# i2Nav-WHU/IC-GVINS

Measured on NVIDIA H100. Metric: frames/sec (KLT+BA) 1280x560 300-feat 10-KF window, higher is better.
Workload: dtype u8/int32 fixed point + f32 (KLT), f64 (BA)

## Files before the change

ic_gvins_b200/csrc/ba.cu:

```cuda
#include <cooperative_groups.h>
#include <dlfcn.h>
#include <unistd.h>
#include <math.h>
#include <nccl.h>
#include <stdlib.h>
#include <string.h>

#include <algorithm>
#include <string>
#include <thread>
#include <vector>

#include "ba_math.cuh"
#include "common.cuh"
#include "geom_core.cuh"

namespace icg {
using namespace bam;
namespace cg = cooperative_groups;

constexpr int BA_SPLIT_W = 4;
constexpr int BA_CHOL_NB = 8;
constexpr int BA_MARG_MAXB = 72;
constexpr int BA_MAX_NODES = 32;

struct BaCaps {
    int NW, K, L, F, G, R;
    int NCV, N, NS, NCA, RJ, LP, NVB;
    int GQ;
};

struct WinDims {
    int K, L, F, n_imu, n_gnss, marg_r, marg_nb;
    int ext_const, td_const, reproj_huber, gnss_huber, has_imu_error, has_pose_prior, has_mix_prior;
    double reproj_sinv;
};

struct LmState {
    double radius, decrease_factor, x_cost, x_norm, cand_cost, model_cost_change, step_norm, gmax, initial_cost, cost_cam;
    int iter, n_success, n_invalid, done, need_lin, last_success, first, step_valid, fresh_lin, max_iter, chol_ok;
};

struct ShardDev {
    int split;
    int PK, BS, RV;
    double *peer[8];
    size_t off_inbox, off_bcast, off_scal, off_flagA, off_flagB, off_flagC;
    double *redv;
    int *err;
    double *slm;
    int *slm_cnt;
};

struct BaDev {
    ShardDev S;
    WinDims *dims;
    LmState *st;
    double *pose, *mix, *ext, *rho;
    double *pose_c, *mix_c, *ext_c, *rho_c;
    double *pose_0, *mix_0, *ext_0, *rho_0;
    uint8_t *f_active_0;
    double *gnss_std_0;
    uint8_t *f_active;
    int *lm_off;
    int *lm_perm;
    int *vb_lm0;
    int *ref_nrun;
    int *f_meta_s;
    double *f_const_s;
    int *vis_ord;
    int *part_off, *pair_ro, *npairs;
    double *gpart;
    int *vis_cnt;
    double *Mp;
    double *AW;
    double *costf;
    double *hl, *gl, *scale_l, *scale_c;
    double *Hc, *gc;
    double *Hs;
    double *visv;
    double *imu_blob, *imu_U;
    int *gnss_node;
    double *gnss_blh, *gnss_std, *lever;
    double *pose_prior, *pose_prior_sinfo, *mix_prior, *mix_prior_std;
    int *marg_type, *marg_node;
    double *marg_x0, *marg_H0, *marg_b0, *marg_c0;
    double *cost_part;
    double *red;
    double *redmax;
    double *red2;
    int rank, world;
    double *step_c, *step_l;
    double *Sglobal;
    unsigned long long *clk;
};

__device__ __forceinline__ int col_pose(int k) { return 6 * k; }
__device__ __forceinline__ int col_ext(int K) { return 6 * K; }
__device__ __forceinline__ int col_td(int K) { return 6 * K + 6; }
__device__ __forceinline__ int col_mix(int K, int k) { return 6 * K + 7 + 9 * k; }

__device__ __forceinline__ int jc_off(int a) { return a < 18 ? (a / 6) * 12 + (a % 6) : 36 + 2 * (a - 18); }
__device__ __forceinline__ int jc_row1(int a) { return a < 18 ? 6 : 1; }
__device__ __forceinline__ int tri20(int la, int lb) {
    return la * 20 - la * (la - 1) / 2 + (lb - la);
}
__device__ __forceinline__ void dmma884(double &c0, double &c1, double a, double b) {
    asm volatile("mma.sync.aligned.m8n8k4.row.col.f64.f64.f64.f64 {%0,%1}, {%2}, {%3}, {%0,%1};" : "+d"(c0), "+d"(c1) : "d"(a), "d"(b));
}
constexpr int LV_LD = 45;
constexpr size_t LV_SMEM = sizeof(double) * (128 * LV_LD + (BA_MAX_NODES + 1) * NODE_FRAME_LD);
__global__ void __launch_bounds__(128, 4) ba_lin_vis(BaCaps C, BaDev D) {
    extern __shared__ double lv_sm[];
    __shared__ int s_ord[128], s_gbeg[BA_MAX_NODES], s_gend[BA_MAX_NODES], s_last, s_p0, s_np;
    double (*s_rec)[LV_LD] = (double (*)[LV_LD]) lv_sm;
    double (*s_frame)[NODE_FRAME_LD] = (double (*)[NODE_FRAME_LD]) (lv_sm + 128 * LV_LD);
    const int w = blockIdx.y;
    const LmState &st = D.st[w];
    if (st.done || !st.need_lin) return;
    const int *vb = D.vb_lm0 + (size_t) w * C.NVB;
    if ((int) blockIdx.x >= vb[C.NVB - 1]) return;
    const WinDims dm = D.dims[w];
    const int tid = threadIdx.x;
    const int *off = D.lm_off + (size_t) w * (C.L + 1);
    const int pA = vb[blockIdx.x], pB = vb[blockIdx.x + 1];
    const int s0 = off[pA], nslot = off[pB] - s0;
    if (tid <= dm.K) node_frame(tid < dm.K ? D.pose + ((size_t) w * C.K + tid) * 7 : D.ext + (size_t) w * 8, s_frame[tid]);
    if (tid < BA_MAX_NODES) s_gbeg[tid] = s_gend[tid] = 0;
    if (tid == 0) s_np = 0;
    __syncthreads();
    if (tid < nslot) {
        const int q = s0 + tid;
        double r[2], Ji[12], Jj[12], Je[12], Jr[2], Jt[2], cost = 0;
        const int4 meta = ((const int4 *) D.f_meta_s)[(size_t) w * C.F + q];
        const int i = meta.y, j = meta.z, f = meta.w;
        if (D.f_active[(size_t) w * C.F + f] != 0) {
            const double *ext = D.ext + (size_t) w * 8;
            reproj_eval_frames(s_frame[i], s_frame[j], s_frame[dm.K], D.rho[(size_t) w * C.L + meta.x], ext[7],
                               D.f_const_s + ((size_t) w * C.F + q) * 14, dm.reproj_sinv, true, r, Ji, Jj, Je, Jr, Jt);
            if (dm.ext_const)
                for (int k = 0; k < 12; k++) Je[k] = 0;
            if (dm.td_const) Jt[0] = Jt[1] = 0;
            double sq = r[0] * r[0] + r[1] * r[1], sc = 1.0;
            if (dm.reproj_huber)
                huber(sq, cost, sc);
            else
                cost = 0.5 * sq;
            if (sc != 1.0) {
                for (int k = 0; k < 12; k++) Ji[k] *= sc, Jj[k] *= sc, Je[k] *= sc;
                Jr[0] *= sc, Jr[1] *= sc, Jt[0] *= sc, Jt[1] *= sc, r[0] *= sc, r[1] *= sc;
            }
        } else {
            for (int k = 0; k < 12; k++) Ji[k] = Jj[k] = Je[k] = 0;
            Jr[0] = Jr[1] = Jt[0] = Jt[1] = r[0] = r[1] = 0;
        }
        D.costf[(size_t) w * C.F + f] = cost;
        double *sr = s_rec[tid];
#pragma unroll
        for (int k = 0; k < 12; k++) sr[k] = Ji[k], sr[12 + k] = Jj[k], sr[24 + k] = Je[k];
        sr[36] = Jt[0], sr[37] = Jt[1], sr[38] = r[0], sr[39] = r[1];
        sr[40] = Jr[0], sr[41] = Jr[1], sr[42] = (double) j, sr[43] = (double) i;
    }
    __syncthreads();
    const int lane = tid & 31, warp = tid >> 5;
    if (nslot > 0) {
        if (tid < nslot) {
            const int *ord = D.vis_ord + (size_t) w * C.F + s0;
            const int v = ord[tid], ob = (int) s_rec[v & 255][42];
            s_ord[tid] = v;
            if (tid == 0 || (int) s_rec[ord[tid - 1] & 255][42] != ob) s_gbeg[ob] = tid;
            if (tid == nslot - 1 || (int) s_rec[ord[tid + 1] & 255][42] != ob) s_gend[ob] = tid + 1;
        }
        __syncthreads();
        const int kk = lane & 3, g = lane >> 2;
        int o[3];
#pragma unroll
        for (int t = 0; t < 3; t++) {
            const int a = 8 * t + g;
            o[t] = a < 20 ? jc_off(a) + (kk & 1) * jc_row1(a) : -1;
        }
        for (int ob = warp; ob < dm.K; ob += 4) {
            const int beg = s_gbeg[ob], end = s_gend[ob];
            if (beg == end) continue;
            double c00[2] = {0, 0}, c01[2] = {0, 0}, c02[2] = {0, 0}, c11[2] = {0, 0}, c12[2] = {0, 0}, c22[2] = {0, 0};
            constexpr int UNR = 2;
            for (int base = beg; base < end; base += 2 * UNR) {
                double x[UNR][3];
#pragma unroll
                for (int u = 0; u < UNR; u++) {
                    const int q = base + 2 * u + (kk >> 1);
                    const bool ok = q < end;
                    const double *rec = s_rec[ok ? s_ord[q] & 255 : 0];
#pragma unroll
                    for (int t = 0; t < 3; t++) x[u][t] = (ok && o[t] >= 0) ? rec[o[t]] : 0.0;
                }
#pragma unroll
                for (int u = 0; u < UNR; u++) {
                    dmma884(c00[0], c00[1], x[u][0], x[u][0]);
                    dmma884(c01[0], c01[1], x[u][0], x[u][1]);
                    dmma884(c02[0], c02[1], x[u][0], x[u][2]);
                    dmma884(c11[0], c11[1], x[u][1], x[u][1]);
                    dmma884(c12[0], c12[1], x[u][1], x[u][2]);
                    dmma884(c22[0], c22[1], x[u][2], x[u][2]);
                }
            }
            double *pp = D.gpart + ((size_t) w * C.GQ + (s_ord[beg] >> 8)) * 210;
            auto put = [&](int ti, int tj, const double *c) {
#pragma unroll
                for (int e = 0; e < 2; e++) {
                    const int la = 8 * ti + g, lb = 8 * tj + 2 * kk + e;
                    if (la <= lb && lb < 20) pp[tri20(la, lb)] = c[e];
                }
            };
            put(0, 0, c00), put(0, 1, c01), put(0, 2, c02), put(1, 1, c11), put(1, 2, c12), put(2, 2, c22);
        }
        __threadfence();
    }
    const int *perm = D.lm_perm + (size_t) w * C.L;
    const int K = dm.K, NCV = 6 * K + 7, NCA = 4 * ((NCV + 1 + 3) / 4);
    const int grp = tid >> 3, sl = tid & 7;
    int o0[3], o1[3];
#pragma unroll
    for (int t = 0; t < 3; t++) {
        const int c = sl + 8 * t;
        o0[t] = c < 19 ? jc_off(c) : 38, o1[t] = c < 19 ? o0[t] + jc_row1(c) : 39;
    }
    for (int pl = pA + grp; pl < pB; pl += 16) {
        const int l = perm[pl], f0 = off[pl] - s0, nf = off[pl + 1] - off[pl];
        double *row = D.AW + ((size_t) w * C.LP + l) * C.NCA;
        for (int c = sl; c < NCA; c += 8) row[c] = 0.0;
        __syncwarp(0xffu << (tid & 24));
        double acc[3] = {0, 0, 0};
        for (int q = 0; q < nf; q++) {
            const double *rec = s_rec[f0 + q];
            const double r0 = rec[40], r1 = rec[41];
            const int ob = (int) rec[42];
#pragma unroll
            for (int t = 0; t < 3; t++) {
                const int c = sl + 8 * t;
                if (c == 20) {
                    acc[t] += r0 * r0 + r1 * r1;
                } else if (c < 20) {
                    const double v = rec[o0[t]] * r0 + rec[o1[t]] * r1;
                    if (c >= 6 && c < 12)
                        row[col_pose(ob) + c - 6] = v;
                    else
                        acc[t] += v;
                }
            }
        }
        const int ref = nf > 0 ? (int) s_rec[f0][43] : 0;
#pragma unroll
        for (int t = 0; t < 3; t++) {
            const int c = sl + 8 * t;
            if (nf > 0) {
                if (c < 6) row[col_pose(ref) + c] = acc[t];
                else if (c >= 12 && c < 18) row[col_ext(K) + c - 12] = acc[t];
                else if (c == 18) row[col_td(K)] = acc[t];
            }
            if (c == 19) {
                row[NCV] = acc[t];
                D.gl[(size_t) w * C.L + l] = acc[t];
            } else if (c == 20) {
                D.hl[(size_t) w * C.L + l] = acc[t];
                if (st.first) D.scale_l[(size_t) w * C.L + l] = 1.0 / (1.0 + sqrt(acc[t]));
            }
        }
    }
    if (nslot == 0) return;
    const int rn = (int) s_rec[0][43];
    __syncthreads();
    if (tid == 0) s_last = atomicAdd(D.vis_cnt + (size_t) w * C.K + rn, 1) == D.ref_nrun[(size_t) w * C.K + rn] - 1;
    __syncthreads();
    if (!s_last) return;
    __threadfence();
    if (tid == 0) D.vis_cnt[(size_t) w * C.K + rn] = 0;
    const int PM = C.K * (C.K - 1), P = D.npairs[w];
    const int *pro = D.pair_ro + (size_t) w * PM, *poff = D.part_off + (size_t) w * (PM + 1);
    for (int p = tid; p < P; p += 128)
        if ((pro[p] >> 8) == rn) {
            atomicAdd(&s_np, 1);
            if (p == 0 || (pro[p - 1] >> 8) != rn) s_p0 = p;
        }
    __syncthreads();
    const double *part = D.gpart + (size_t) w * C.GQ * 210;
    double *Mp = D.Mp + (size_t) w * PM * 210;
    for (int p = s_p0 + warp; p < s_p0 + s_np; p += 4) {
        const int k0 = poff[p], k1 = poff[p + 1];
        double acc[7];
#pragma unroll
        for (int j = 0; j < 7; j++) acc[j] = lane + 32 * j < 210 ? __ldcg(part + (size_t) k0 * 210 + lane + 32 * j) : 0.0;
        for (int k = k0 + 1; k < k1; k++) {
            double v[7];
#pragma unroll
            for (int j = 0; j < 7; j++) v[j] = lane + 32 * j < 210 ? __ldcg(part + (size_t) k * 210 + lane + 32 * j) : 0.0;
#pragma unroll
            for (int j = 0; j < 7; j++) acc[j] += v[j];
        }
#pragma unroll
        for (int j = 0; j < 7; j++)
            if (lane + 32 * j < 210) Mp[(size_t) p * 210 + lane + 32 * j] = acc[j];
    }
}


__device__ __forceinline__ void gram2_slots(const BaCaps &C, const BaDev &D, int w, int K, short *s_slot) {
    const int PM = C.K * (C.K - 1), P = D.npairs[w];
    const int *pro = D.pair_ro + (size_t) w * PM;
    for (int e = threadIdx.x; e < K * K; e += blockDim.x) s_slot[e] = -1;
    __syncthreads();
    for (int p = threadIdx.x; p < P; p += blockDim.x) s_slot[(pro[p] >> 8) * K + (pro[p] & 255)] = (short) p;
    __syncthreads();
}
__device__ __forceinline__ double gram2_entry(const BaCaps &C, const BaDev &D, int w, int K, const short *s_slot, int A, int B) {
    const int PM = C.K * (C.K - 1), P = D.npairs[w];
    const double *Mp = D.Mp + (size_t) w * PM * 210;
    const int bA = A < 6 * K ? A / 6 : K, bB = B < 6 * K ? B / 6 : K;
    const int a = A - 6 * bA, b = B - 6 * bB;
    const int ga = 12 + a, gb = 12 + b;
    double sum = 0;
    if (bA == K) {
        const int idx = tri20(ga, gb);
        double s4[4] = {0, 0, 0, 0};
        int p = 0;
        for (; p + 16 <= P; p += 16) {
            double v[16];
#pragma unroll
            for (int u = 0; u < 16; u++) v[u] = Mp[(size_t) (p + u) * 210 + idx];
#pragma unroll
            for (int u = 0; u < 16; u++) s4[u & 3] += v[u];
        }
        for (; p < P; p++) s4[p & 3] += Mp[(size_t) p * 210 + idx];
        sum = (s4[0] + s4[1]) + (s4[2] + s4[3]);
    } else if (bB == K || bB == bA) {
        const int i1 = tri20(a, bB == K ? gb : b), i2 = tri20(6 + a, bB == K ? gb : 6 + b);
        for (int o0 = 0; o0 < K; o0 += 8) {
            double v1[8], v2[8];
#pragma unroll
            for (int u = 0; u < 8; u++) {
                const int o = o0 + u;
                const int p1 = o < K ? s_slot[bA * K + o] : -1, p2 = o < K ? s_slot[o * K + bA] : -1;
                v1[u] = p1 >= 0 ? Mp[(size_t) p1 * 210 + i1] : 0.0;
                v2[u] = p2 >= 0 ? Mp[(size_t) p2 * 210 + i2] : 0.0;
            }
#pragma unroll
            for (int u = 0; u < 8; u++) sum += v1[u], sum += v2[u];
        }
    } else {
        const int p1 = s_slot[bA * K + bB], p2 = s_slot[bB * K + bA];
        if (p1 >= 0) sum += Mp[(size_t) p1 * 210 + tri20(a, 6 + b)];
        if (p2 >= 0) sum += Mp[(size_t) p2 * 210 + tri20(b, 6 + a)];
    }
    return sum;
}

__device__ __forceinline__ double block_sum(double v, double *s_red);
__device__ __forceinline__ double block_max(double v, double *s_red);
__device__ __forceinline__ double *x_inbox(const BaDev &D, int peer, int w, int from);
__device__ __forceinline__ int tri_idx(int A, int B, int ncv);

__device__ __forceinline__ void schur_store(const BaCaps &C, const BaDev &D, int w, int K, const short *s_slot, int A, int B, double cw) {
    const int NCV = 6 * K + 7;
    const bool nccl = !D.S.split && D.world > 1;
    if (A == NCV && !nccl) return;
    const size_t e = (size_t) w * C.NS * C.NS + (size_t) B * C.NS + A;
    const double hc = !D.S.split && !nccl && B < NCV ? D.Hc[e] : 0.0;
    const double cj = gram2_entry(C, D, w, K, s_slot, A, B);
    if (D.S.split) {
        double *P = x_inbox(D, w % D.world, w, D.rank);
        const int TRI = NCV * (NCV + 1) / 2;
        if (B < NCV) {
            P[tri_idx(A, B, NCV)] = cj - cw;
            if (A == B) P[TRI + A] = cj;
        } else {
            P[TRI + NCV + A] = cj;
            P[TRI + 2 * NCV + A] = cw;
        }
    } else if (nccl) {
        const size_t NN = (size_t) C.NCA * C.NCA;
        double *R = D.red + (size_t) w * (2 * NN + 8);
        R[(size_t) A * C.NCA + B] = R[(size_t) B * C.NCA + A] = cj;
        R[NN + (size_t) A * C.NCA + B] = R[NN + (size_t) B * C.NCA + A] = cw;
    } else {
        double *V = D.visv + (size_t) w * 3 * C.NCV;
        if (B < NCV) {
            D.Hs[e] = hc + (cj - cw);
            if (A == B) V[A] = cj;
        } else {
            V[NCV + A] = cj, V[2 * NCV + A] = cw;
        }
    }
}

__device__ __forceinline__ void schur_scalars(const BaCaps &C, const BaDev &D, int w, const WinDims &dm, double *s_red) {
    const int tid = threadIdx.x;
    double c = 0, q = 0, gm = 0;
    for (int f = tid; f < dm.F; f += 256) c += D.costf[(size_t) w * C.F + f];
    for (int l = tid; l < dm.L; l += 256) {
        const double r = D.rho[(size_t) w * C.L + l];
        q += r * r;
        gm = fmax(gm, fabs(D.gl[(size_t) w * C.L + l]));
    }
    c = block_sum(c, s_red);
    q = block_sum(q, s_red);
    gm = block_max(gm, s_red);
    if (tid != 0) return;
    if (D.S.split) {
        const int NCV = 6 * dm.K + 7, TRI = NCV * (NCV + 1) / 2;
        double *P = x_inbox(D, w % D.world, w, D.rank);
        P[TRI + 3 * NCV] = c, P[TRI + 3 * NCV + 1] = q, P[TRI + 3 * NCV + 2] = gm;
    } else {
        const size_t NN = (size_t) C.NCA * C.NCA;
        double *R = D.red + (size_t) w * (2 * NN + 8);
        R[2 * NN] = c, R[2 * NN + 1] = q;
        for (int k = 2; k < 8; k++) R[2 * NN + k] = 0;
        D.redmax[w] = gm;
    }
}

constexpr int SCHUR_RCH = 80;
constexpr int SCHUR_PASS = 16;
__global__ void __cluster_dims__(BA_SPLIT_W, 1, 1) __launch_bounds__(256) ba_schur_dmma(BaCaps C, BaDev D, int ld) {
    extern __shared__ double sA[];
    __shared__ short s_slot[32 * 32];
    __shared__ double s_red[40];
    cg::cluster_group cluster = cg::this_cluster();
    const int w = blockIdx.y, split = blockIdx.x;
    const LmState &st = D.st[w];
    if (st.done) return;
    const WinDims dm = D.dims[w];
    const int NCV = 6 * dm.K + 7, NCA = 4 * ((NCV + 1 + 3) / 4);
    const int T2 = (NCA + 15) / 16, nsuper = T2 * (T2 + 1) / 2;
    const int tid = threadIdx.x, lane = tid & 31, warp = tid >> 5, g = lane >> 2, kk = lane & 3;
    double *sphi = sA + (size_t) SCHUR_RCH * ld;
    const double *A = D.AW + (size_t) w * C.LP * C.NCA;
    const double radius = st.radius;
    const int nsteps = (dm.L + 3) / 4;
    const int r_beg = 4 * (int) ((long long) nsteps * split / BA_SPLIT_W), r_end = min(dm.L, 4 * (int) ((long long) nsteps * (split + 1) / BA_SPLIT_W));
    const int npass = (nsuper + SCHUR_PASS - 1) / SCHUR_PASS;
    gram2_slots(C, D, w, dm.K, s_slot);
    for (int pass = 0; pass < npass; pass++) {
        if (pass > 0) cluster.barrier_wait();
        int si[2], sj[2];
        bool on[2];
#pragma unroll
        for (int h2 = 0; h2 < 2; h2++) {
            const int su = (2 * pass + h2) * 8 + warp;
            on[h2] = su < nsuper;
            int a = 0, e = on[h2] ? su : 0;
            while (e >= T2 - a) e -= T2 - a, a++;
            si[h2] = a, sj[h2] = a + e;
        }
        double acc[2][4][2];
#pragma unroll
        for (int h2 = 0; h2 < 2; h2++)
#pragma unroll
            for (int q = 0; q < 4; q++) acc[h2][q][0] = acc[h2][q][1] = 0;
        for (int r0 = r_beg; r0 < r_end; r0 += SCHUR_RCH) {
            const int nr = min(SCHUR_RCH, r_end - r0), nr4 = (nr + 3) & ~3;
            __syncthreads();
            for (int rb = warp; rb < nr4; rb += 8 * 4) {
                double v[4][3];
#pragma unroll
                for (int u = 0; u < 4; u++) {
                    const int rr = rb + 8 * u;
#pragma unroll
                    for (int cchunk = 0; cchunk < 3; cchunk++) {
                        const int c = lane + 32 * cchunk;
                        v[u][cchunk] = (rr < nr && c < NCA) ? A[(size_t) (r0 + rr) * C.NCA + c] : 0.0;
                    }
                }
#pragma unroll
                for (int u = 0; u < 4; u++) {
                    const int rr = rb + 8 * u;
#pragma unroll
                    for (int cchunk = 0; cchunk < 3; cchunk++) {
                        const int c = lane + 32 * cchunk;
                        if (rr < nr4 && c < ld) sA[(size_t) rr * ld + c] = v[u][cchunk];
                    }
                }
                for (int c = lane + 96; c < ld; c += 32)
                    for (int u = 0; u < 4; u++) {
                        const int rr = rb + 8 * u;
                        if (rr < nr4) sA[(size_t) rr * ld + c] = (rr < nr && c < NCA) ? A[(size_t) (r0 + rr) * C.NCA + c] : 0.0;
                    }
            }
            for (int rr = tid; rr < nr4; rr += 256) {
                double ph = 0;
                if (rr < nr) {
                    const int l = r0 + rr;
                    const double sl = D.scale_l[(size_t) w * C.L + l], hs = sl * sl * D.hl[(size_t) w * C.L + l];
                    ph = sl * sl / (hs + fmin(fmax(hs, 1e-6), 1e32) / radius);
                }
                sphi[rr] = ph;
            }
            __syncthreads();
            for (int ks = 0; ks < nr4 / 4; ks++) {
                const double *row = sA + (size_t) (4 * ks + kk) * ld;
                const double ph = sphi[4 * ks + kk];
#pragma unroll
                for (int h2 = 0; h2 < 2; h2++) {
                    if (!on[h2]) continue;
                    const double xb0 = row[16 * sj[h2] + g], xb1 = row[16 * sj[h2] + 8 + g];
                    const double a0 = row[16 * si[h2] + g] * ph, a1 = row[16 * si[h2] + 8 + g] * ph;
                    dmma884(acc[h2][0][0], acc[h2][0][1], a0, xb0);
                    dmma884(acc[h2][1][0], acc[h2][1][1], a0, xb1);
                    dmma884(acc[h2][2][0], acc[h2][2][1], a1, xb0);
                    dmma884(acc[h2][3][0], acc[h2][3][1], a1, xb1);
                }
            }
        }
        __syncthreads();
#pragma unroll
        for (int h2 = 0; h2 < 2; h2++) {
            if (!on[h2]) continue;
#pragma unroll
            for (int q = 0; q < 4; q++)
#pragma unroll
                for (int e = 0; e < 2; e++) sA[(h2 * 8 + warp) * 256 + 64 * q + 32 * e + lane] = acc[h2][q][e];
        }
        cluster.sync();
        const int nslot = min(SCHUR_PASS, nsuper - SCHUR_PASS * pass);
        double cw[SCHUR_PASS / BA_SPLIT_W];
#pragma unroll
        for (int j = 0; j < SCHUR_PASS / BA_SPLIT_W; j++) {
            const int sl = split + BA_SPLIT_W * j;
            double p[BA_SPLIT_W];
#pragma unroll
            for (int k = 0; k < BA_SPLIT_W; k++) p[k] = sl < nslot ? cluster.map_shared_rank(sA, k)[sl * 256 + tid] : 0.0;
            cw[j] = 0;
#pragma unroll
            for (int k = 0; k < BA_SPLIT_W; k++) cw[j] += p[k];
        }
        cluster.barrier_arrive();
        const int q = tid >> 6, r_in = 8 * (q >> 1) + ((tid & 31) >> 2), c_in = 8 * (q & 1) + 2 * (tid & 3) + ((tid >> 5) & 1);
#pragma unroll
        for (int j = 0; j < SCHUR_PASS / BA_SPLIT_W; j++) {
            const int sl = split + BA_SPLIT_W * j;
            if (sl >= nslot) break;
            int a = 0, e = SCHUR_PASS * pass + sl;
            while (e >= T2 - a) e -= T2 - a, a++;
            const int r = 16 * a + r_in, cc = 16 * (a + e) + c_in;
            if (r <= cc && cc <= NCV) schur_store(C, D, w, dm.K, s_slot, r, cc, cw[j]);
        }
    }
    if (split == 0 && (D.S.split || D.world > 1)) schur_scalars(C, D, w, dm, s_red);
    cluster.barrier_wait();
}

constexpr double IMU_GB_STD = 7200 / 3600.0 * 3.14159265358979323846 / 180.0;
constexpr double IMU_AB_STD = 2.0e4 * 1.0e-5;

__device__ void imu_factor_warp(const double *blob, const double *U, const double *pose0, const double *mix0, const double *pose1,
                                const double *mix1, bool want_j, double *rw, double *Jw, int lane) {
    __shared__ ImuMid s_mid[16];
    double *raw_r = rw + 15;
    const int wslot = (threadIdx.x >> 5) & 15;
    if (want_j)
        for (int e = lane; e < 450; e += 32) Jw[e] = 0;
    __syncwarp();
    if (lane == 0) {
        ImuMid M;
        imu_residual_raw(blob, pose0, mix0, pose1, mix1, raw_r, M);
        if (want_j) imu_jacobian_raw(blob, M, Jw);
        s_mid[wslot] = M;
    }
    __syncwarp();
    if (want_j && lane < 30) {
        for (int i = 0; i < 15; i++) {
            double s = 0;
            for (int k = i; k < 15; k++) s += U[i * 15 + k] * Jw[k * 30 + lane];
            Jw[i * 30 + lane] = s;
        }
    }
    if (lane < 15) {
        double s = 0;
        for (int k = lane; k < 15; k++) s += U[lane * 15 + k] * raw_r[k];
        rw[lane] = s;
    }
    __syncwarp();
}

__device__ void marg_dx(const BaCaps &C, const BaDev &D, int w, const WinDims &dm, const double *pose, const double *mix, const double *ext, double *dx,
                        int *colmap, int tid, int nthreads) {
    const int *type = D.marg_type + (size_t) w * BA_MARG_MAXB, *node = D.marg_node + (size_t) w * BA_MARG_MAXB;
    const double *x0 = D.marg_x0 + (size_t) w * BA_MARG_MAXB * 9;
    if (tid == 0) {
        int col = 0, xo = 0;
        for (int b = 0; b < dm.marg_nb; b++) {
            int t = type[b], nd = node[b];
            if (t == 0 || t == 2) {
                const double *x = t == 0 ? pose + nd * 7 : ext;
                const double *xl = x0 + xo;
                Q dq = qmul(qinv(pose_q(xl)), pose_q(x));
                V3 a = 2.0 * qv(dq);
                if (dq.w < 0) a = -a;
                for (int k = 0; k < 3; k++) dx[col + k] = x[k] - xl[k];
                dx[col + 3] = a.x, dx[col + 4] = a.y, dx[col + 5] = a.z;
                int base = t == 0 ? col_pose(nd) : col_ext(dm.K);
                for (int k = 0; k < 6; k++) colmap[col + k] = (t == 2 && dm.ext_const) ? -1 : base + k;
                col += 6, xo += 7;
            } else if (t == 1) {
                for (int k = 0; k < 9; k++) dx[col + k] = mix[nd * 9 + k] - x0[xo + k], colmap[col + k] = col_mix(dm.K, nd) + k;
                col += 9, xo += 9;
            } else {
                dx[col] = ext[7] - x0[xo];
                colmap[col] = dm.td_const ? -1 : col_td(dm.K);
                col += 1, xo += 1;
            }
        }
    }
}

__device__ __forceinline__ void red_add(double *p, double v) { asm volatile("red.global.add.f64 [%0], %1;" ::"l"(p), "d"(v) : "memory"); }

__device__ double cam_factors(const BaCaps &C, const BaDev &D, int w, const WinDims &dm, const double *pose, const double *mix, const double *ext,
                              bool lin, double *smem) {
    const int tid = threadIdx.x, lane = tid & 31, warp = tid >> 5, nwarps = blockDim.x >> 5;
    const int K = dm.K, N = 15 * K + 7;
    double *Hc = D.Hc + (size_t) w * C.NS * C.NS, *gc = D.gc + (size_t) w * C.NS;
    double *s_imu = smem;
    double *s_gnss = s_imu + (size_t) C.K * 480;
    double *s_misc = s_gnss + (size_t) C.G * 24;
    double *s_pp = s_misc, *s_mp = s_misc + 48, *s_dx = s_mp + 16, *s_y = s_dx + C.R, *s_cost = s_y + C.R;
    int *s_colmap = (int *) (s_cost + 8);
    __shared__ double s_total;
#ifdef ICG_BA_PHASE_CLOCKS
    unsigned long long cclk = D.clk ? clock64() : 0ull;
#define CAM_CLK(k)                                                 \
    if (D.clk && lin && w == 0 && tid == 0) {                      \
        const unsigned long long t_ = clock64();                   \
        atomicAdd(&D.clk[16 + (k)], t_ - cclk), atomicAdd(&D.clk[24 + (k)], 1ull); \
        cclk = t_;                                                 \
    }
#else
#define CAM_CLK(k)
#endif
    for (int k = warp; k < dm.n_imu; k += nwarps)
        imu_factor_warp(D.imu_blob + ((size_t) w * C.K + k) * ICG_IMU_BLOB_DOUBLES, D.imu_U + ((size_t) w * C.K + k) * 225, pose + k * 7, mix + k * 9,
                        pose + (k + 1) * 7, mix + (k + 1) * 9, lin, s_imu + (size_t) k * 480, s_imu + (size_t) k * 480 + 30, lane);
    if (tid < dm.n_gnss) {
        const int nd = D.gnss_node[(size_t) w * C.G + tid];
        double *o = s_gnss + tid * 24;
        gnss_eval(pose + nd * 7, D.gnss_blh + ((size_t) w * C.G + tid) * 3, D.gnss_std + ((size_t) w * C.G + tid) * 3, D.lever + (size_t) w * 3, lin, o, o + 3);
        double sq = o[0] * o[0] + o[1] * o[1] + o[2] * o[2], cost, sc = 1.0;
        if (dm.gnss_huber)
            huber(sq, cost, sc);
        else
            cost = 0.5 * sq;
        if (sc != 1.0) {
            for (int e = 0; e < 3; e++) o[e] *= sc;
            if (lin)
                for (int e = 0; e < 18; e++) o[3 + e] *= sc;
        }
        o[21] = cost;
    }
    if (tid == 64 && dm.has_pose_prior) pose_prior_eval(pose, D.pose_prior + (size_t) w * 7, D.pose_prior_sinfo + (size_t) w * 6, lin, s_pp, s_pp + 6);
    if (tid == 96 && dm.has_mix_prior)
        for (int k = 0; k < 9; k++) s_mp[k] = (mix[k] - D.mix_prior[(size_t) w * 9 + k]) / D.mix_prior_std[(size_t) w * 9 + k];
    if (dm.marg_r > 0) marg_dx(C, D, w, dm, pose, mix, ext, s_dx, s_colmap, tid, blockDim.x);
    __syncthreads();
    CAM_CLK(0)
    const double *H0 = D.marg_H0 + (size_t) w * C.R * C.R, *b0 = D.marg_b0 + (size_t) w * C.R;
    if (dm.marg_r > 0) {
        for (int i = tid; i < dm.marg_r; i += blockDim.x) {
            double s = 0;
            for (int k = 0; k < dm.marg_r; k++) s += H0[(size_t) i * dm.marg_r + k] * s_dx[k];
            s_y[i] = s;
        }
    }
    __syncthreads();
    if (tid == 0) {
        double c = 0;
        for (int k = 0; k < dm.n_imu; k++) {
            const double *r = s_imu + (size_t) k * 480;
            double sq = 0;
            for (int e = 0; e < 15; e++) sq += r[e] * r[e];
            c += 0.5 * sq;
        }
        for (int g = 0; g < dm.n_gnss; g++) c += s_gnss[g * 24 + 21];
        if (dm.has_imu_error) {
            const double *m = mix + dm.n_imu * 9;
            double sq = 0;
            for (int e = 0; e < 3; e++) sq += (m[3 + e] / IMU_GB_STD) * (m[3 + e] / IMU_GB_STD) + (m[6 + e] / IMU_AB_STD) * (m[6 + e] / IMU_AB_STD);
            c += 0.5 * sq;
        }
        if (dm.has_pose_prior) {
            double sq = 0;
            for (int e = 0; e < 6; e++) sq += s_pp[e] * s_pp[e];
            c += 0.5 * sq;
        }
        if (dm.has_mix_prior) {
            double sq = 0;
            for (int e = 0; e < 9; e++) sq += s_mp[e] * s_mp[e];
            c += 0.5 * sq;
        }
        if (dm.marg_r > 0) {
            double q = D.marg_c0[w];
            for (int i = 0; i < dm.marg_r; i++) q += (2.0 * b0[i] + s_y[i]) * s_dx[i];
            c += 0.5 * q;
        }
        s_total = c;
    }
// ... 5 lines not shown
    for (int e = tid; e < N * C.NS; e += blockDim.x) Hc[e] = 0;
    for (int e = tid; e < N; e += blockDim.x) gc[e] = 0;
    __syncthreads();
    CAM_CLK(2)
    if (dm.marg_r > 0) {
        const int r = dm.marg_r;
        for (int e = tid; e < r * r; e += blockDim.x) {
            int i = e / r, j = e - i * r;
            int ci = s_colmap[i], cj = s_colmap[j];
            if (ci >= 0 && cj >= 0) Hc[(size_t) ci * C.NS + cj] = H0[e];
        }
        for (int i = tid; i < r; i += blockDim.x)
            if (s_colmap[i] >= 0) gc[s_colmap[i]] = b0[i] + s_y[i];
    }
    __syncthreads();
    CAM_CLK(3)
    for (int parity = 0; parity < 2; parity++) {
        const int nf = (dm.n_imu - parity + 1) / 2;
        for (int e = tid; e < nf * 930; e += blockDim.x) {
            const int k = parity + 2 * (e / 930), q = e % 930;
            const double *rw = s_imu + (size_t) k * 480, *Jw = rw + 30;
            auto gcol = [&](int c) { return c < 6 ? col_pose(k) + c : c < 15 ? col_mix(K, k) + c - 6 : c < 21 ? col_pose(k + 1) + c - 15 : col_mix(K, k + 1) + c - 21; };
            if (q < 900) {
                int a = q / 30, b = q - a * 30;
                double s = 0;
                for (int m = 0; m < 15; m++) s += Jw[m * 30 + a] * Jw[m * 30 + b];
                red_add(&Hc[(size_t) gcol(a) * C.NS + gcol(b)], s);
            } else {
                int a = q - 900;
                double s = 0;
                for (int m = 0; m < 15; m++) s += Jw[m * 30 + a] * rw[m];
                red_add(&gc[gcol(a)], s);
            }
        }
        __syncthreads();
    }
    CAM_CLK(4)
    for (int e = tid; e < K * 42; e += blockDim.x) {
        const int k = e / 42, q = e % 42;
        double s = 0;
        if (q < 36) {
            const int a = q / 6, b = q % 6;
            for (int g = 0; g < dm.n_gnss; g++)
                if (D.gnss_node[(size_t) w * C.G + g] == k) {
                    const double *J = s_gnss + g * 24 + 3;
                    s += J[a] * J[b] + J[6 + a] * J[6 + b] + J[12 + a] * J[12 + b];
                }
            if (k == 0 && dm.has_pose_prior)
                for (int m = 0; m < 6; m++) s += s_pp[6 + m * 6 + a] * s_pp[6 + m * 6 + b];
            red_add(&Hc[(size_t) (col_pose(k) + a) * C.NS + col_pose(k) + b], s);
        } else {
            const int a = q - 36;
            for (int g = 0; g < dm.n_gnss; g++)
                if (D.gnss_node[(size_t) w * C.G + g] == k) {
                    const double *o = s_gnss + g * 24;
                    s += o[3 + a] * o[0] + o[9 + a] * o[1] + o[15 + a] * o[2];
                }
            if (k == 0 && dm.has_pose_prior)
                for (int m = 0; m < 6; m++) s += s_pp[6 + m * 6 + a] * s_pp[m];
            red_add(&gc[col_pose(k) + a], s);
        }
    }
    if (tid < 9) {
        if (dm.has_imu_error && tid >= 3) {
            const int k = dm.n_imu;
            const double sd = tid < 6 ? IMU_GB_STD : IMU_AB_STD;
            Hc[(size_t) (col_mix(K, k) + tid) * C.NS + col_mix(K, k) + tid] += 1.0 / (sd * sd);
            gc[col_mix(K, k) + tid] += mix[k * 9 + tid] / (sd * sd);
        }
    }
    __syncthreads();
    if (tid < 9 && dm.has_mix_prior) {
        const double sd = D.mix_prior_std[(size_t) w * 9 + tid];
        Hc[(size_t) (col_mix(K, 0) + tid) * C.NS + col_mix(K, 0) + tid] += 1.0 / (sd * sd);
        gc[col_mix(K, 0) + tid] += s_mp[tid] / sd;
    }
    __syncthreads();
    CAM_CLK(5)
#undef CAM_CLK
    return s_total;
}

constexpr int CAM_THREADS = 320;
__global__ void __launch_bounds__(CAM_THREADS) ba_lin_cam(BaCaps C, BaDev D) {
    extern __shared__ double smem[];
    const int w = blockIdx.x;
    LmState &st = D.st[w];
    if (st.done || !st.need_lin) return;
    if (D.S.split && (w % D.world) != D.rank) return;
    const WinDims dm = D.dims[w];
    double c = cam_factors(C, D, w, dm, D.pose + (size_t) w * C.K * 7, D.mix + (size_t) w * C.K * 9, D.ext + (size_t) w * 8, true, smem);
    if (threadIdx.x == 0) st.cost_cam = c;
}

__global__ void ba_pack2(BaCaps C, BaDev D, int n, int nblk_vis) {
    const int w = blockIdx.x * blockDim.x + threadIdx.x;
    if (w >= n) return;
    const LmState &st = D.st[w];
    if (st.done || !st.step_valid) return;
    const WinDims dm = D.dims[w];
    const double *part = D.cost_part + (size_t) w * (nblk_vis + 1);
    double cand = 0;
    const int nb = (dm.F + 255) / 256;
    for (int b = 0; b < nb; b++) cand += part[b];
    if (D.rank == 0) cand += part[nblk_vis];
    D.red2[(size_t) w * 4 + 3] = cand;
}

__global__ void __launch_bounds__(256) ba_hsum(BaCaps C, BaDev D) {
    const int w = blockIdx.y;
    if (D.st[w].done) return;
    const int K = D.dims[w].K, NCV = 6 * K + 7, nn = NCV + 1;
    const int NN = C.NCA * C.NCA;
    const int t = blockIdx.x * 256 + threadIdx.x;
    if (t >= nn * nn) return;
    const int A = t / nn, B = t - A * nn;
    if (B < A || B >= NCV) return;
    const double *RED = D.red + (size_t) w * (2 * NN + 8);
    const double cj = RED[(size_t) B * C.NCA + A], cw = RED[NN + (size_t) B * C.NCA + A];
    D.Hs[(size_t) w * C.NS * C.NS + (size_t) B * C.NS + A] = D.Hc[(size_t) w * C.NS * C.NS + (size_t) B * C.NS + A] + (cj - cw);
}

constexpr int SOLVE_THREADS = 256;

__device__ __forceinline__ double block_sum(double v, double *s_red) {
    const int tid = threadIdx.x, lane = tid & 31, warp = tid >> 5;
    for (int o = 16; o > 0; o >>= 1) v += __shfl_down_sync(0xffffffffu, v, o);
    __syncthreads();
    if (lane == 0) s_red[warp] = v;
    __syncthreads();
    double t = 0;
    if (tid == 0) {
        for (int k = 0; k < (int) (blockDim.x >> 5); k++) t += s_red[k];
        s_red[32] = t;
    }
    __syncthreads();
    return s_red[32];
}
__device__ __forceinline__ double block_max(double v, double *s_red) {
    const int tid = threadIdx.x, lane = tid & 31, warp = tid >> 5;
    for (int o = 16; o > 0; o >>= 1) v = fmax(v, __shfl_down_sync(0xffffffffu, v, o));
    __syncthreads();
    if (lane == 0) s_red[warp] = v;
    __syncthreads();
    if (tid == 0) {
        double t = 0;
        for (int k = 0; k < (int) (blockDim.x >> 5); k++) t = fmax(t, s_red[k]);
        s_red[32] = t;
    }
    __syncthreads();
    return s_red[32];
}

__global__ void __launch_bounds__(SOLVE_THREADS, 2) ba_solve(BaCaps C, BaDev D) {
    extern __shared__ double sm[];
    const int w = blockIdx.x, tid = threadIdx.x;
    LmState &st = D.st[w];
    if (st.done) return;
#ifdef ICG_BA_PHASE_CLOCKS
    unsigned long long clk_prev = D.clk ? clock64() : 0ull;
#define SOLVE_CLK(k)                                              \
    if (D.clk && w == 0 && tid == 0) {                            \
        const unsigned long long t_ = clock64();                  \
        atomicAdd(&D.clk[k], t_ - clk_prev), atomicAdd(&D.clk[8 + (k)], 1ull); \
        clk_prev = t_;                                            \
    }
#define SOLVE_CLK_NOW() (D.clk ? clock64() : 0ull)
#define SOLVE_CLK_ADD(k, t0)                                      \
    if (D.clk && w == 0 && tid == 0) atomicAdd(&D.clk[k], clock64() - (t0)), atomicAdd(&D.clk[8 + (k)], 1ull);
#else
#define SOLVE_CLK(k)
#define SOLVE_CLK_NOW() 0ull
#define SOLVE_CLK_ADD(k, t0)
#endif
    const WinDims dm = D.dims[w];
    const int K = dm.K, L = dm.L, NCV = 6 * K + 7, N = 15 * K + 7;
    const int f_first = st.first, f_fresh = st.fresh_lin, f_last = st.last_success, f_iter = st.iter;
    const double f_gmax_old = st.gmax;
    (void) f_gmax_old;
    double *s_red = sm;
    double *s_scale = s_red + 40;
    double *s_g = s_scale + C.NS;
    double *s_rhs = s_g + C.NS;
    double *s_d2 = s_rhs + C.NS;
    double *s_diag = s_d2 + C.NS;
    double *S = s_diag + C.NS;
    const double *Hc = D.Hc + (size_t) w * C.NS * C.NS, *gcam = D.gc + (size_t) w * C.NS, *Hs = D.Hs + (size_t) w * C.NS * C.NS;
    const bool sharded = D.world > 1;
    const int NN = C.NCA * C.NCA;
    const double *RED = D.red + (size_t) w * (2 * NN + 8), *V = D.visv + (size_t) w * 3 * C.NCV;
    auto hvis_diag = [&](int a) { return sharded ? RED[(size_t) a * C.NCA + a] : V[a]; };
    auto g_vis = [&](int a) { return sharded ? RED[(size_t) a * C.NCA + NCV] : V[NCV + a]; };
    auto wphig = [&](int a) { return sharded ? RED[NN + (size_t) a * C.NCA + NCV] : V[2 * NCV + a]; };
    const double camw = D.rank == 0 ? 1.0 : 0.0;
    if (tid == 0 && st.need_lin) st.need_lin = 0;
    double *scale_c = D.scale_c + (size_t) w * C.NS;
    const double *hl = D.hl + (size_t) w * C.L, *gl = D.gl + (size_t) w * C.L, *scale_l = D.scale_l + (size_t) w * C.L;

    for (int a = tid; a < N; a += SOLVE_THREADS) {
        double g = gcam[a];
        if (a < NCV) g += g_vis(a);
        s_g[a] = g;
        if (f_first) {
            double h = Hc[(size_t) a * C.NS + a] + (a < NCV ? hvis_diag(a) : 0.0);
            scale_c[a] = 1.0 / (1.0 + sqrt(h));
        }
    }
    __syncthreads();
    for (int a = tid; a < N; a += SOLVE_THREADS) s_scale[a] = scale_c[a];
    double gmax_now = st.gmax;
    if (f_fresh) {
        double c, gml;
        if (sharded) {
            c = RED[2 * NN];
            gml = D.redmax[w];
        } else {
            double cs = 0, gq = 0;
            for (int f = tid; f < dm.F; f += SOLVE_THREADS) cs += D.costf[(size_t) w * C.F + f];
            for (int l = tid; l < L; l += SOLVE_THREADS) gq = fmax(gq, fabs(gl[l]));
            c = block_sum(cs, s_red);
            gml = block_max(gq, s_red);
        }
        double gm = 0;
        for (int a = tid; a < N; a += SOLVE_THREADS) gm = fmax(gm, fabs(s_g[a]));
        gm = fmax(block_max(gm, s_red), gml);
        gmax_now = gm;
        if (tid == 0) {
            st.x_cost = c + st.cost_cam;
            st.gmax = gm;
            if (f_first) st.initial_cost = st.x_cost;
            st.fresh_lin = 0;
        }
        __syncthreads();
    }
    if (f_first) {
        __syncthreads();
        if (tid == 0) st.first = 0;
    }
    {
        int term = 0;
        if (f_iter >= st.max_iter) term = 1;
        else if (f_last && gmax_now <= 1e-10) term = 2;
        else if (f_last && st.radius <= 1e-32) term = 2;
        if (term) {
            __syncthreads();
            if (tid == 0) st.done = term, st.step_valid = 0;
            return;
        }
    }
    __syncthreads();
    if (tid == 0) st.iter++;
    const double radius = st.radius;
    SOLVE_CLK(0)

    constexpr bool async_fill = true;
    if (async_fill) {
        for (int i = tid >> 5; i < N; i += SOLVE_THREADS / 32) {
            const double *src = (i < NCV ? Hs : Hc) + (size_t) i * C.NS;
            const unsigned dst = (unsigned) __cvta_generic_to_shared(S + i * (i + 1) / 2);
            for (int j = tid & 31; j <= i; j += 32)
                asm volatile("cp.async.ca.shared.global [%0], [%1], 8;" ::"r"(dst + 8u * j), "l"(src + j) : "memory");
        }
        asm volatile("cp.async.commit_group;" ::: "memory");
    }
    for (int a = tid; a < N; a += SOLVE_THREADS) {
        double h = Hc[(size_t) a * C.NS + a] + (a < NCV ? hvis_diag(a) : 0.0);
        double hs = s_scale[a] * s_scale[a] * h;
        s_d2[a] = fmin(fmax(hs, 1e-6), 1e32) / radius;
        double gw = a < NCV ? wphig(a) : 0.0;
        s_rhs[a] = -s_scale[a] * (s_g[a] - gw);
    }
    if (async_fill) asm volatile("cp.async.wait_all;" ::: "memory");
    __syncthreads();
    if (async_fill) {
        for (int i = tid >> 5; i < N; i += SOLVE_THREADS / 32) {
            double *row = S + i * (i + 1) / 2;
            const double si = s_scale[i];
            for (int j = tid & 31; j <= i; j += 32) {
                double v = si * s_scale[j] * row[j];
                if (i == j) v += s_d2[i];
                row[j] = v;
            }
        }
    } else {
        for (int i = tid >> 5; i < N; i += SOLVE_THREADS / 32) {
            constexpr int MAXQ = 16;
            double hv[MAXQ];
            const int nq = i / 32 + 1;
#pragma unroll
            for (int q = 0; q < MAXQ; q++) {
                const int j = (tid & 31) + 32 * q;
                hv[q] = 0;
                if (q < nq && j <= i) hv[q] = (i < NCV ? Hs : Hc)[(size_t) i * C.NS + j];
            }
#pragma unroll
            for (int q = 0; q < MAXQ; q++) {
                const int j = (tid & 31) + 32 * q;
                if (q < nq && j <= i) {
                    double v = s_scale[i] * s_scale[j] * hv[q];
                    if (i == j) v += s_d2[i];
                    S[i * (i + 1) / 2 + j] = v;
                }
            }
        }
    }
    for (int a = tid; a < N; a += SOLVE_THREADS) S[N * (N + 1) / 2 + a] = s_rhs[a];
    __syncthreads();
    SOLVE_CLK(1)
    __shared__ int s_fail;
    if (tid == 0) s_fail = 0;
    __syncthreads();
// ... 89 lines not shown
#pragma unroll
                    for (int u = 0; u < TPW; u++) {
                        dmma884(acc[u][0], acc[u][1], a0[u], b0);
                        dmma884(acc[u][2], acc[u][3], a1[u], b1);
                    }
                }
#pragma unroll
                for (int u = 0; u < TPW; u++) {
                    const double c0 = acc[u][0] + acc[u][2], c1 = acc[u][1] + acc[u][3];
                    const int i = J0 + 8 * (t0 + u * NWARP) + g;
                    if (oka[u]) {
                        const int ca = J0 + 2 * kk;
                        if (ca < J0 + nb && ca <= i) S[i * (i + 1) / 2 + ca] -= c0;
                        if (ca + 1 < J0 + nb && ca + 1 <= i) S[i * (i + 1) / 2 + ca + 1] -= c1;
                    }
                }
            }
        }
        __syncthreads();
        const unsigned long long pc1 = SOLVE_CLK_NOW();
        (void) pc1;
        if (s_fail) break;
        for (int i = J0 + nb + tid; i < NR; i += SOLVE_THREADS) {
            double *ri = S + i * (i + 1) / 2 + J0;
            double x[BA_CHOL_NB];
#pragma unroll
            for (int c = 0; c < BA_CHOL_NB; c++) x[c] = c < nb ? ri[c] : 0.0;
#pragma unroll
            for (int c = 0; c < BA_CHOL_NB; c++) {
                if (c < nb) {
                    const double *lc = S + (J0 + c) * (J0 + c + 1) / 2 + J0;
                    double sum = x[c];
#pragma unroll
                    for (int k = 0; k < c; k++) sum -= x[k] * lc[k];
                    x[c] = sum * s_diag[J0 + c];
                }
            }
#pragma unroll
            for (int c = 0; c < BA_CHOL_NB; c++)
                if (c < nb) ri[c] = x[c];
        }
        __syncthreads();
        SOLVE_CLK_ADD(7, pc1)
    }
    __syncthreads();
    bool valid = !s_fail;
    SOLVE_CLK(2)
    if (valid) {
        double *y = S + N * (N + 1) / 2;
        const int lane = tid & 31;
        for (int J0 = ((N - 1) / BA_CHOL_NB) * BA_CHOL_NB; J0 >= 0; J0 -= BA_CHOL_NB) {
            const int nb = min(BA_CHOL_NB, N - J0);
            if (tid < 32) {
                double x[BA_CHOL_NB];
#pragma unroll
                for (int c = BA_CHOL_NB - 1; c >= 0; c--) {
                    x[c] = 0.0;
                    if (c < nb) {
                        double sum = y[J0 + c];
#pragma unroll
                        for (int k = BA_CHOL_NB - 1; k > c; k--)
                            if (k < nb) sum -= S[(J0 + k) * (J0 + k + 1) / 2 + J0 + c] * x[k];
                        x[c] = sum * s_diag[J0 + c];
                    }
                }
#pragma unroll
                for (int c = 0; c < BA_CHOL_NB; c++)
                    if (c == lane && c < nb) s_rhs[J0 + c] = x[c];
            }
            __syncthreads();
            for (int i = tid; i < J0; i += SOLVE_THREADS) {
                double acc = y[i];
#pragma unroll
                for (int c = BA_CHOL_NB - 1; c >= 0; c--)
                    if (c < nb) acc -= S[(J0 + c) * (J0 + c + 1) / 2 + i] * s_rhs[J0 + c];
                y[i] = acc;
            }
            __syncthreads();
        }
    }
    __syncthreads();
    SOLVE_CLK(3)
    double *step_l = D.step_l + (size_t) w * C.L;
    const double *AW = D.AW + (size_t) w * C.LP * C.NCA;
    double part = 0;
    bool finite = true;
    double *R2 = D.red2 + (size_t) w * 4;
    if (!valid) {
        if (tid == 0) {
            st.chol_ok = 0, st.step_valid = 0;
            R2[0] = 0, R2[1] = 0, R2[2] = 1, R2[3] = 0;
        }
        return;
    }
    for (int a = tid; a < N; a += SOLVE_THREADS) {
        double sp = s_rhs[a];
        finite = finite && isfinite(sp);
        part += camw * (-0.5 * sp * (s_scale[a] * s_g[a]) + 0.5 * s_d2[a] * sp * sp);
    }
    double *s_sx = s_diag;
    __syncthreads();
    for (int a = tid; a < NCV; a += SOLVE_THREADS) s_sx[a] = s_scale[a] * s_rhs[a];
    __syncthreads();
    {
        const int lane = tid & 31, warp = tid >> 5;
        constexpr int LB = 8;
        const int lu = ((lane >> 4) & 1) * 4 + ((lane >> 3) & 1) * 2 + ((lane >> 2) & 1);
        for (int l0 = LB * warp; l0 < L; l0 += LB * (SOLVE_THREADS / 32)) {
            const int l = l0 + lu;
            const bool lok = l < L;
            const double sl = lok ? scale_l[l] : 0.0, hh = lok ? hl[l] : 0.0, gg = lok ? gl[l] : 0.0;
            double d[LB];
#pragma unroll
            for (int u = 0; u < LB; u++) d[u] = 0;
            for (int c = lane; c < NCV; c += 32) {
                const double sx = s_sx[c];
#pragma unroll
                for (int u = 0; u < LB; u++) d[u] += (l0 + u < L ? AW[(size_t) (l0 + u) * C.NCA + c] : 0.0) * sx;
            }
            const double hs = sl * sl * hh, d2 = fmin(fmax(hs, 1e-6), 1e32) / radius, den = hs + d2, sg = sl * gg;
            double e4[4], e2[2];
            {
                const bool hi = lane & 16;
#pragma unroll
                for (int u = 0; u < 4; u++) {
                    const double keep = hi ? d[u + 4] : d[u], send = hi ? d[u] : d[u + 4];
                    e4[u] = keep + __shfl_xor_sync(0xffffffffu, send, 16);
                }
            }
            {
                const bool hi = lane & 8;
#pragma unroll
                for (int u = 0; u < 2; u++) {
                    const double keep = hi ? e4[u + 2] : e4[u], send = hi ? e4[u] : e4[u + 2];
                    e2[u] = keep + __shfl_xor_sync(0xffffffffu, send, 8);
                }
            }
            double mine;
            {
                const bool hi = lane & 4;
                const double keep = hi ? e2[1] : e2[0], send = hi ? e2[0] : e2[1];
                mine = keep + __shfl_xor_sync(0xffffffffu, send, 4);
            }
            mine += __shfl_xor_sync(0xffffffffu, mine, 2);
            mine += __shfl_xor_sync(0xffffffffu, mine, 1);
            if ((lane & 3) == 0 && lok) {
                double sp = (-sg - sl * mine) / den;
                finite = finite && isfinite(sp);
                step_l[l] = sp;
                part += -0.5 * sp * sg + 0.5 * d2 * sp * sp;
            }
        }
    }
    __syncthreads();
    SOLVE_CLK(4)
    const double mcc = block_sum(part, s_red);
    const double nfin = block_sum(finite ? 0.0 : 1.0, s_red);
    const double *pose = D.pose + (size_t) w * C.K * 7, *mix = D.mix + (size_t) w * C.K * 9, *ext = D.ext + (size_t) w * 8, *rho = D.rho + (size_t) w * C.L;
    double *pose_c = D.pose_c + (size_t) w * C.K * 7, *mix_c = D.mix_c + (size_t) w * C.K * 9, *ext_c = D.ext_c + (size_t) w * 8, *rho_c = D.rho_c + (size_t) w * C.L;
    double sn = 0;
    for (int k = tid; k <= K; k += SOLVE_THREADS) {
        const bool is_ext = (k == K);
        const double *x = is_ext ? ext : pose + k * 7;
        double *xc = is_ext ? ext_c : pose_c + k * 7;
        if (is_ext && dm.ext_const) {
            for (int e = 0; e < 7; e++) xc[e] = x[e];
        } else {
            const int c0 = is_ext ? col_ext(K) : col_pose(k);
            double d[6];
            for (int e = 0; e < 6; e++) d[e] = s_rhs[c0 + e] * s_scale[c0 + e];
            pose_plus(x, d, xc);
            for (int e = 0; e < 7; e++) sn += camw * (x[e] - xc[e]) * (x[e] - xc[e]);
        }
    }
    for (int e = tid; e < K * 9; e += SOLVE_THREADS) {
        int k = e / 9, q = e - 9 * k, c = col_mix(K, k) + q;
        double v = mix[e] + s_rhs[c] * s_scale[c];
        mix_c[e] = v;
        sn += camw * (mix[e] - v) * (mix[e] - v);
    }
    if (tid == 0) {
        if (dm.td_const) {
            ext_c[7] = ext[7];
        } else {
            double v = ext[7] + s_rhs[col_td(K)] * s_scale[col_td(K)];
            ext_c[7] = v;
            sn += camw * (ext[7] - v) * (ext[7] - v);
        }
    }
    for (int l = tid; l < L; l += SOLVE_THREADS) {
        double v = rho[l] + step_l[l] * scale_l[l];
        rho_c[l] = v;
        sn += (rho[l] - v) * (rho[l] - v);
    }
    sn = block_sum(sn, s_red);
    if (tid == 0) {
        st.chol_ok = 1, st.step_valid = 1;
        R2[0] = mcc, R2[1] = sn, R2[2] = nfin, R2[3] = 0;
    }
    SOLVE_CLK(5)
#undef SOLVE_CLK
#undef SOLVE_CLK_NOW
#undef SOLVE_CLK_ADD
}

__global__ void __launch_bounds__(CAM_THREADS) ba_cost_cam(BaCaps C, BaDev D, int nblk_vis) {
    extern __shared__ double smem[];
    const int w = blockIdx.x;
    const LmState &st = D.st[w];
    if (st.done || !st.step_valid) return;
    if (D.S.split && (w % D.world) != D.rank) return;
    const WinDims dm = D.dims[w];
    double c = cam_factors(C, D, w, dm, D.pose_c + (size_t) w * C.K * 7, D.mix_c + (size_t) w * C.K * 9, D.ext_c + (size_t) w * 8, false, smem);
    if (threadIdx.x == 0) D.cost_part[(size_t) w * (nblk_vis + 1) + nblk_vis] = c;
}
__global__ void __launch_bounds__(256) ba_cost(BaCaps C, BaDev D, int nblk_vis) {
    __shared__ double s_red[40];
    const int w = blockIdx.y;
    const LmState &st = D.st[w];
    if (st.done || !st.step_valid) return;
    const WinDims dm = D.dims[w];
    const double *pose = D.pose_c + (size_t) w * C.K * 7, *ext = D.ext_c + (size_t) w * 8, *rho = D.rho_c + (size_t) w * C.L;
    double *part = D.cost_part + (size_t) w * (nblk_vis + 1);
    const int q = blockIdx.x * 256 + threadIdx.x;
    __shared__ double s_frame[BA_MAX_NODES + 1][NODE_FRAME_LD];
    if ((int) threadIdx.x <= dm.K) node_frame((int) threadIdx.x < dm.K ? pose + threadIdx.x * 7 : ext, s_frame[threadIdx.x]);
    __syncthreads();
    double cost = 0;
    int4 meta = make_int4(0, 0, 0, 0);
    if (q < dm.F) meta = ((const int4 *) D.f_meta_s)[(size_t) w * C.F + q];
    if (q < dm.F && D.f_active[(size_t) w * C.F + meta.w]) {
        double r[2];
        reproj_eval_frames(s_frame[meta.y], s_frame[meta.z], s_frame[dm.K], rho[meta.x], ext[7], D.f_const_s + ((size_t) w * C.F + q) * 14, dm.reproj_sinv,
                           false, r, nullptr, nullptr, nullptr, nullptr, nullptr);
        double sq = r[0] * r[0] + r[1] * r[1], sc;
        if (dm.reproj_huber)
            huber(sq, cost, sc);
        else
            cost = 0.5 * sq;
    }
    cost = block_sum(cost, s_red);
    if (threadIdx.x == 0) part[blockIdx.x] = cost;
}

__global__ void __launch_bounds__(128) ba_accept(BaCaps C, BaDev D, int nblk_vis) {
    __shared__ int s_accept;
    __shared__ double s_camsq, s_rhosq;
    __shared__ double s_red[40];
    const int w = blockIdx.x, tid = threadIdx.x;
    LmState &st = D.st[w];
    if (st.done) return;
    const WinDims dm = D.dims[w];
    const int chol_ok = st.chol_ok;
    const double *R2 = D.red2 + (size_t) w * 4;
    {
        const double *pose = D.pose + (size_t) w * C.K * 7, *mix = D.mix + (size_t) w * C.K * 9, *ext = D.ext + (size_t) w * 8;
        double s = 0;
        for (int e = tid; e < dm.K * 7; e += 128) s += pose[e] * pose[e];
        for (int e = tid; e < dm.K * 9; e += 128) s += mix[e] * mix[e];
        if (tid < 7 && !dm.ext_const) s += ext[tid] * ext[tid];
        if (tid == 7 && !dm.td_const) s += ext[7] * ext[7];
        s = block_sum(s, s_red);
        double q = 0;
        if (D.world == 1) {
            for (int l = tid; l < dm.L; l += 128) q += D.rho[(size_t) w * C.L + l] * D.rho[(size_t) w * C.L + l];
            q = block_sum(q, s_red);
        } else {
            q = D.red[(size_t) w * (2 * C.NCA * C.NCA + 8) + 2 * C.NCA * C.NCA + 1];
        }
        if (tid == 0) s_camsq = s, s_rhosq = q;
    }
    __syncthreads();
    if (tid == 0) {
        s_accept = 0;
        const double mcc = R2[0], sn = R2[1], nfin = R2[2];
        double cand = R2[3];
        if (D.world == 1 && st.step_valid) {
            const double *part = D.cost_part + (size_t) w * (nblk_vis + 1);
            cand = 0;
            const int nb = (dm.F + 255) / 256;
            for (int b = 0; b < nb; b++) cand += part[b];
            cand += part[nblk_vis];
        }
        if (!chol_ok || nfin != 0.0 || !(mcc > 0.0)) {
            st.step_valid = 0;
            st.n_invalid++;
            if (st.n_invalid >= 5) st.done = 3;
            st.radius *= 0.5;
            st.last_success = 0;
        } else {
            st.n_invalid = 0;
            st.model_cost_change = mcc;
            st.step_norm = sqrt(sn);
            st.x_norm = sqrt(s_camsq + s_rhosq);
            st.cand_cost = cand;
            if (st.step_norm <= 1e-8 * (st.x_norm + 1e-8)) {
                st.done = 2;
            } else if (fabs(st.x_cost - cand) <= 1e-6 * st.x_cost) {
                st.done = 2;
            } else {
                const double rel = (st.x_cost - cand) / mcc;
                if (rel > 1e-3) {
                    s_accept = 1;
                    st.n_success++;
                    double t = 2.0 * rel - 1.0;
                    st.radius = fmin(1e16, st.radius / fmax(1.0 / 3.0, 1.0 - t * t * t));
                    st.decrease_factor = 2.0;
                    st.last_success = 1;
                    st.need_lin = 1;
                    st.fresh_lin = 1;
                } else {
                    st.radius = st.radius / st.decrease_factor;
                    st.decrease_factor *= 2.0;
                    st.last_success = 0;
                    st.need_lin = 0;
                }
            }
        }
    }
    __syncthreads();
    if (!s_accept) return;
    double *pose = D.pose + (size_t) w * C.K * 7, *mix = D.mix + (size_t) w * C.K * 9, *ext = D.ext + (size_t) w * 8, *rho = D.rho + (size_t) w * C.L;
    const double *pose_c = D.pose_c + (size_t) w * C.K * 7, *mix_c = D.mix_c + (size_t) w * C.K * 9, *ext_c = D.ext_c + (size_t) w * 8, *rho_c = D.rho_c + (size_t) w * C.L;
    for (int e = tid; e < dm.K * 7; e += 128) pose[e] = pose_c[e];
    for (int e = tid; e < dm.K * 9; e += 128) mix[e] = mix_c[e];
    if (tid < 8) ext[tid] = ext_c[tid];
    for (int e = tid; e < dm.L; e += 128) rho[e] = rho_c[e];
}

__global__ void ba_reset_state(BaDev D, LmState *save, int n, int max_iter) {
    int w = blockIdx.x * blockDim.x + threadIdx.x;
    if (w >= n) return;
    if (save) save[w] = D.st[w];
    LmState st;
    memset(&st, 0, sizeof(st));
    st.radius = 1e4, st.decrease_factor = 2.0;
    st.need_lin = 1, st.fresh_lin = 1, st.first = 1, st.last_success = 1, st.max_iter = max_iter;
    D.st[w] = st;
}

__global__ void __launch_bounds__(128) ba_chi2_cull(BaCaps C, BaDev D, int *counters) {
    const int w = blockIdx.y;
    WinDims &dm = D.dims[w];
    const int t = blockIdx.x * 128 + threadIdx.x;
    const double *pose = D.pose + (size_t) w * C.K * 7, *ext = D.ext + (size_t) w * 8, *rho = D.rho + (size_t) w * C.L;
    int4 meta = make_int4(0, 0, 0, 0);
    if (t < dm.F) meta = ((const int4 *) D.f_meta_s)[(size_t) w * C.F + t];
    if (t < dm.F && D.f_active[(size_t) w * C.F + meta.w]) {
        double r[2];
        reproj_eval(pose + meta.y * 7, pose + meta.z * 7, ext, rho[meta.x], ext[7], D.f_const_s + ((size_t) w * C.F + t) * 14, dm.reproj_sinv, false, r, nullptr,
                    nullptr, nullptr, nullptr, nullptr);
        if ((r[0] * r[0] + r[1] * r[1]) > 5.991) {
            D.f_active[(size_t) w * C.F + meta.w] = 0;
            atomicAdd(&counters[2 * w], 1);
        }
    }
    if (t < dm.n_gnss) {
        double r[3];
        double *sd = D.gnss_std + ((size_t) w * C.G + t) * 3;
        gnss_eval(pose + D.gnss_node[(size_t) w * C.G + t] * 7, D.gnss_blh + ((size_t) w * C.G + t) * 3, sd, D.lever + (size_t) w * 3, false, r, nullptr);
        double chi2 = r[0] * r[0] + r[1] * r[1] + r[2] * r[2];
        if (chi2 > 7.815) {
            double sc = sqrt(chi2 / 7.815);
            sd[0] *= sc, sd[1] *= sc, sd[2] *= sc;
            atomicAdd(&counters[2 * w + 1], 1);
        }
    }
}
__global__ void ba_set_gnss_huber(BaDev D, int n, int v) {
    int w = blockIdx.x * blockDim.x + threadIdx.x;
    if (w < n) D.dims[w].gnss_huber = v;
}

__global__ void ba_residual_costs_kernel(BaCaps C, BaDev D, double *reproj_cost, double *gnss_cost) {
    const int w = 0;
    const WinDims dm = D.dims[w];
    const int t = blockIdx.x * blockDim.x + threadIdx.x;
    const double *pose = D.pose, *ext = D.ext, *rho = D.rho;
    if (t < dm.F) {
        double r[2];
        const int4 meta = ((const int4 *) D.f_meta_s)[t];
        reproj_eval(pose + meta.y * 7, pose + meta.z * 7, ext, rho[meta.x], ext[7], D.f_const_s + (size_t) t * 14, dm.reproj_sinv, false, r, nullptr, nullptr,
                    nullptr, nullptr, nullptr);
        reproj_cost[meta.w] = 0.5 * (r[0] * r[0] + r[1] * r[1]);
    }
    if (t < dm.n_gnss) {
        double r[3];
        gnss_eval(pose + D.gnss_node[t] * 7, D.gnss_blh + t * 3, D.gnss_std + t * 3, D.lever, false, r, nullptr);
        gnss_cost[t] = 0.5 * (r[0] * r[0] + r[1] * r[1] + r[2] * r[2]);
    }
}

__global__ void ba_reproj_eval_kernel(const double *in , double *out ) {
// ... 266 lines not shown
        return ICG_ENODEVICE;
    }
    if (device < 0 || device >= ndev) {
        set_error("icg_ba_create: device %d out of range", device);
        return ICG_EINVAL;
    }
    ICG_CUDA(cudaSetDevice(device));
    cudaDeviceProp prop;
    ICG_CUDA(cudaGetDeviceProperties(&prop, device));
    if (prop.major != 9 || prop.minor != 0) {
        set_error("icg_ba_create: device is sm_%d%d; this library is built for sm_90a only", prop.major, prop.minor);
        return ICG_ENODEVICE;
    }
    icg_ba *h = new icg_ba();
    h->device = device;
    const int rc_init = ba_create_body(h, max_windows, max_K, max_L, max_F, max_gnss, max_marg_r, stream);
    if (rc_init != ICG_OK) {
        icg_ba_destroy(h);
        return rc_init;
    }
    *out = h;
    return ICG_OK;
}

static int ba_create_body(icg_ba *h, int max_windows, int max_K, int max_L, int max_F, int max_gnss, int max_marg_r, void *stream) {
    if (stream) {
        h->stream = (cudaStream_t) stream;
    } else {
        ICG_CUDA(cudaStreamCreateWithFlags(&h->stream, cudaStreamNonBlocking));
        h->own_stream = true;
    }
    {
        int prio_lo = 0, prio_hi = 0;
        ICG_CUDA(cudaDeviceGetStreamPriorityRange(&prio_lo, &prio_hi));
        ICG_CUDA(cudaStreamCreateWithPriority(&h->stream_cam, cudaStreamNonBlocking, prio_hi));
    }
    ICG_CUDA(cudaEventCreateWithFlags(&h->ev_fork, cudaEventDisableTiming));
    ICG_CUDA(cudaEventCreateWithFlags(&h->ev_join, cudaEventDisableTiming));
    h->prof = getenv("ICG_BA_PROFILE") != nullptr;
    if (getenv("ICG_BA_CAM_THREADS")) h->cam_threads = std::min(CAM_THREADS, std::max(128, atoi(getenv("ICG_BA_CAM_THREADS")) & ~31));
    if (h->prof) {
        double *ck = nullptr;
        if (dmalloc(h, &ck, 48) != ICG_OK) return ICG_ENOMEM;
        h->D.clk = (unsigned long long *) ck;
    }
    if (getenv("ICG_BA_PROFILE_SKIP")) h->prof_skip = atoi(getenv("ICG_BA_PROFILE_SKIP"));
    BaCaps &C = h->C;
    max_L = std::max(1, max_L), max_F = std::max(1, max_F);
    C.NW = max_windows, C.K = max_K, C.L = max_L, C.F = max_F, C.G = std::max(1, max_gnss), C.R = std::max(1, max_marg_r);
    C.NCV = 6 * max_K + 7, C.N = 15 * max_K + 7, C.NS = (C.N + 3) & ~3, C.NCA = 4 * ((C.NCV + 1 + 3) / 4);
    C.RJ = (2 * max_F + 31) & ~31, C.LP = (max_L + 31) & ~31;
    C.NVB = (max_F + 127 - max_K) / (128 - max_K) + max_L / 128 + 4 + max_K;
    C.GQ = std::max(1, std::min(max_F, (C.NVB - 2) * (max_K - 1)));
    h->nblk_vis = (max_F + 255) / 256;
    const size_t NW = max_windows;
#define HD(field, count)                                                       \
    if (h->field.alloc(count) != ICG_OK) {                                     \
        set_error("icg_ba_create: allocation of " #field " failed");           \
        return ICG_ENOMEM;                                                     \
    }
    HD(dims, NW) HD(st, NW) HD(pose, NW * C.K * 7) HD(mix, NW * C.K * 9) HD(ext, NW * 8) HD(rho, NW * C.L)
    HD(imu_blob, NW * C.K * ICG_IMU_BLOB_DOUBLES) HD(imu_U, NW * C.K * 225) HD(gnss_blh, NW * C.G * 3) HD(gnss_std, NW * C.G * 3) HD(lever, NW * 3)
    HD(pose_prior, NW * 7) HD(pose_prior_sinfo, NW * 6) HD(mix_prior, NW * 9) HD(mix_prior_std, NW * 9) HD(marg_x0, NW * BA_MARG_MAXB * 9)
    HD(marg_H0, NW * C.R * C.R) HD(marg_b0, NW * C.R) HD(marg_c0, NW)
    HD(lm_off, NW * (C.L + 1)) HD(lm_perm, NW * C.L) HD(lm_fidx, NW * C.F) HD(gnss_node, NW * C.G) HD(marg_type, NW * BA_MARG_MAXB) HD(marg_node, NW * BA_MARG_MAXB) HD(f_active, NW * C.F)
    HD(scratch, 1024) HD(st_save, NW) HD(cull_counters, 2 * NW) HD(f_meta_s, NW * C.F * 4) HD(vb_lm0, NW * C.NVB) HD(ref_nrun, NW * C.K) HD(f_const_s, NW * C.F * 14)
    HD(part_off, NW * ((size_t) C.K * (C.K - 1) + 1)) HD(pair_ro, NW * (size_t) C.K * (C.K - 1)) HD(vis_ord, NW * C.F) HD(npairs, NW)
#undef HD
    BaDev &D = h->D;
    D.rank = 0, D.world = 1;
    D.dims = h->dims.d, D.st = h->st.d, D.pose = h->pose.d, D.mix = h->mix.d, D.ext = h->ext.d, D.rho = h->rho.d;
    D.f_active = h->f_active.d;
    D.part_off = h->part_off.d, D.pair_ro = h->pair_ro.d, D.vis_ord = h->vis_ord.d, D.npairs = h->npairs.d;
    D.f_meta_s = h->f_meta_s.d, D.vb_lm0 = h->vb_lm0.d, D.ref_nrun = h->ref_nrun.d, D.f_const_s = h->f_const_s.d;
    D.lm_off = h->lm_off.d, D.lm_perm = h->lm_perm.d, D.imu_blob = h->imu_blob.d, D.imu_U = h->imu_U.d;
    D.gnss_node = h->gnss_node.d, D.gnss_blh = h->gnss_blh.d, D.gnss_std = h->gnss_std.d, D.lever = h->lever.d;
    D.pose_prior = h->pose_prior.d, D.pose_prior_sinfo = h->pose_prior_sinfo.d, D.mix_prior = h->mix_prior.d, D.mix_prior_std = h->mix_prior_std.d;
    D.marg_type = h->marg_type.d, D.marg_node = h->marg_node.d, D.marg_x0 = h->marg_x0.d, D.marg_H0 = h->marg_H0.d, D.marg_b0 = h->marg_b0.d, D.marg_c0 = h->marg_c0.d;
    int rc = ICG_OK;
#define DM(field, count) \
    if (rc == ICG_OK) rc = dmalloc(h, &D.field, count);
    DM(pose_c, NW * C.K * 7) DM(mix_c, NW * C.K * 9) DM(ext_c, NW * 8) DM(rho_c, NW * C.L)
    DM(pose_0, NW * C.K * 7) DM(mix_0, NW * C.K * 9) DM(ext_0, NW * 8) DM(rho_0, NW * C.L)
    DM(AW, NW * C.NCA * C.LP) DM(Mp, NW * (size_t) C.K * (C.K - 1) * 210) DM(visv, NW * 3 * C.NCV)
    DM(gpart, NW * (size_t) C.GQ * 210) DM(costf, NW * C.F) DM(hl, NW * C.L) DM(gl, NW * C.L) DM(scale_l, NW * C.L) DM(scale_c, NW * C.NS)
    DM(Hc, NW * C.NS * C.NS) DM(gc, NW * C.NS) DM(Hs, NW * C.NS * C.NS) DM(cost_part, NW * (h->nblk_vis + 1)) DM(red, NW * (2 * (size_t) C.NCA * C.NCA + 8)) DM(redmax, NW) DM(red2, NW * 4) DM(step_c, NW * C.NS) DM(step_l, NW * C.L)
#undef DM
    if (rc == ICG_OK) rc = dmalloc(h, &D.gnss_std_0, NW * C.G * 3);
    if (rc == ICG_OK) {
        double *cnt = nullptr;
        rc = dmalloc(h, &cnt, (NW * C.K + 1) / 2);
        D.vis_cnt = (int *) cnt;
    }
    if (rc == ICG_OK) {
        double *fa0 = nullptr;
        rc = dmalloc(h, &fa0, (NW * C.F + 7) / 8 + 1);
        D.f_active_0 = (uint8_t *) fa0;
    }
    if (rc != ICG_OK) return rc;
    h->smem_cam = sizeof(double) * ((size_t) C.K * 480 + (size_t) C.G * 24 + 48 + 16 + 2 * (size_t) C.R + 8) + sizeof(int) * (size_t) C.R + 64;
    size_t vec = sizeof(double) * (40 + 5 * (size_t) C.NS);
    size_t packed = sizeof(double) * ((size_t) (C.N + 1) * (C.N + 2) / 2);
    h->use_global_S = (vec + packed > 220 * 1024) ? 1 : 0;
    h->smem_solve = vec + (h->use_global_S ? 0 : packed);
    D.Sglobal = nullptr;
    memset(&D.S, 0, sizeof(D.S));
    if (h->use_global_S) {
        rc = split_setup(h, 0, 1);
        if (rc != ICG_OK) return rc;
    } else {
        ICG_CUDA(raise_dynamic_smem((const void *) ba_solve, (size_t) (h->smem_solve)));
    }
    h->ld_schur = 16 * ((C.NCA + 15) / 16) + 8;
    h->smem_schur = sizeof(double) * std::max((size_t) SCHUR_RCH * h->ld_schur + SCHUR_RCH, (size_t) SCHUR_PASS * 256);
    ICG_CUDA(raise_dynamic_smem((const void *) ba_schur_dmma, (size_t) (h->smem_schur)));
    ICG_CUDA(cudaFuncSetAttribute(ba_schur_dmma, cudaFuncAttributePreferredSharedMemoryCarveout, cudaSharedmemCarveoutMaxShared));
    ICG_CUDA(raise_dynamic_smem((const void *) ba_lin_cam, (size_t) (h->smem_cam)));
    ICG_CUDA(raise_dynamic_smem((const void *) ba_cost_cam, (size_t) (h->smem_cam)));
    ICG_CUDA(raise_dynamic_smem((const void *) ba_lin_vis, LV_SMEM));
    ICG_CUDA(cudaStreamSynchronize(h->stream));
    h->cur_windows = 0;
    return ICG_OK;
}

void icg_ba_destroy(icg_ba *h) {
    if (!h) return;
    cudaSetDevice(h->device);
    if (h->stream) cudaStreamSynchronize(h->stream);
    prof_collect(h);
    prof_print(h);
    for (cudaEvent_t e : h->prof_ev) cudaEventDestroy(e);
    h->dims.release(), h->st.release(), h->pose.release(), h->mix.release(), h->ext.release(), h->rho.release();
    h->imu_blob.release(), h->imu_U.release(), h->gnss_blh.release(), h->gnss_std.release(), h->lever.release(), h->pose_prior.release();
    h->pose_prior_sinfo.release(), h->mix_prior.release(), h->mix_prior_std.release(), h->marg_x0.release(), h->marg_H0.release(), h->marg_b0.release();
    h->marg_c0.release(), h->lm_off.release(), h->lm_perm.release(), h->lm_fidx.release(), h->gnss_node.release();
    h->f_meta_s.release(), h->vb_lm0.release(), h->ref_nrun.release(), h->f_const_s.release(), h->marg_type.release(), h->marg_node.release(), h->f_active.release(), h->scratch.release(), h->st_save.release(), h->cull_counters.release(), h->part_off.release(), h->pair_ro.release(), h->vis_ord.release(), h->npairs.release();
    if (h->comm) nccl_api().CommDestroy((ncclComm_t) h->comm);
    split_release(h);
    if (h->marg_ready) h->marg_map.release(), h->marg_oJ0.release(), h->marg_oe0.release(), h->marg_oHp.release(), h->marg_obp.release();
    for (void *p : h->dev_only) cudaFree(p);
    if (h->stream_cam) cudaStreamSynchronize(h->stream_cam), cudaStreamDestroy(h->stream_cam);
    if (h->ev_fork) cudaEventDestroy(h->ev_fork);
    if (h->ev_join) cudaEventDestroy(h->ev_join);
    if (h->own_stream && h->stream) cudaStreamDestroy(h->stream);
    delete h;
}

int icg_ba_upload(icg_ba *h, int n, const icg_ba_problem *P) {
    if (!h || !P || n < 1 || n > h->C.NW) {
        set_error("icg_ba_upload: bad arguments (n=%d, capacity %d)", n, h ? h->C.NW : 0);
        return ICG_EINVAL;
    }
    ICG_CUDA(cudaSetDevice(h->device));
    const BaCaps &C = h->C;
#define PK_FAIL(code, ...)                          \
    do {                                            \
        char eb_[512];                              \
        snprintf(eb_, sizeof(eb_), __VA_ARGS__);    \
        err = eb_;                                  \
        return code;                                \
    } while (0)
    auto pack_one = [&](int w, std::string &err) -> int {
        const icg_ba_problem &p = P[w];
        if (p.K < 2 || p.K > C.K || p.L < 0 || p.L > C.L || p.F < 0 || p.F > C.F || p.n_imu < 0 || p.n_imu > p.K - 1 || p.n_gnss < 0 || p.n_gnss > C.G ||
            p.marg_r < 0 || p.marg_r > C.R || p.marg_nblocks < 0 || p.marg_nblocks > 2 * C.K + 2 || !p.pose || !p.mix || !p.ext || (p.L > 0 && !p.invdepth) ||
            (p.F > 0 && (!p.f_lm || !p.f_ref || !p.f_obs || !p.f_const))) {
            PK_FAIL(ICG_EINVAL, "icg_ba_upload: window %d exceeds the handle's capacity or has null parameter arrays (K=%d L=%d F=%d gnss=%d marg_r=%d)", w, p.K, p.L, p.F,
                      p.n_gnss, p.marg_r);
        }
// ... 129 lines not shown
        }
        if (p.marg_r > 0) {
            const int r = p.marg_r;
            int tot = 0, cols = 0;
            for (int b = 0; b < p.marg_nblocks; b++) {
                int t = p.marg_block_type[b];
                if (t < 0 || t > 3 || ((t == 0 || t == 1) && (p.marg_block_node[b] < 0 || p.marg_block_node[b] >= p.K))) {
                    PK_FAIL(ICG_EINVAL, "icg_ba_upload: window %d marginalization block %d invalid", w, b);
                }
                tot += (t == 0 || t == 2) ? 7 : t == 1 ? 9 : 1;
                cols += (t == 0 || t == 2) ? 6 : t == 1 ? 9 : 1;
                h->marg_type.h[(size_t) w * BA_MARG_MAXB + b] = t;
                h->marg_node.h[(size_t) w * BA_MARG_MAXB + b] = p.marg_block_node[b];
            }
            if (cols != r || tot > BA_MARG_MAXB * 9) {
                PK_FAIL(ICG_EINVAL, "icg_ba_upload: window %d marginalization prior size mismatch (blocks give %d columns, marg_r=%d)", w, cols, r);
            }
            memcpy(h->marg_x0.h + (size_t) w * BA_MARG_MAXB * 9, p.marg_x0, sizeof(double) * tot);
            double *H0 = h->marg_H0.h + (size_t) w * C.R * C.R, *b0 = h->marg_b0.h + (size_t) w * C.R;
            for (int i = 0; i < r; i++) {
                for (int j = i; j < r; j++) {
                    double s = 0;
                    for (int k = 0; k < r; k++) s += p.marg_J0[(size_t) k * r + i] * p.marg_J0[(size_t) k * r + j];
                    H0[(size_t) i * r + j] = H0[(size_t) j * r + i] = s;
                }
                double s = 0;
                for (int k = 0; k < r; k++) s += p.marg_J0[(size_t) k * r + i] * p.marg_e0[k];
                b0[i] = s;
            }
            double c0 = 0;
            for (int k = 0; k < r; k++) c0 += p.marg_e0[k] * p.marg_e0[k];
            h->marg_c0.h[w] = c0;
        }
            return ICG_OK;
    };
#undef PK_FAIL
    {
        const int nthreads = std::max(1, std::min({n / 4, 16, (int) std::thread::hardware_concurrency()}));
        std::vector<int> rcs(nthreads, ICG_OK);
        std::vector<std::string> errs(nthreads);
        auto worker = [&](int t) {
            for (int w = t; w < n; w += nthreads) {
                const int rc = pack_one(w, errs[t]);
                if (rc != ICG_OK) {
                    rcs[t] = rc;
                    return;
                }
            }
        };
        std::vector<std::thread> th;
        for (int t = 1; t < nthreads; t++) th.emplace_back(worker, t);
        worker(0);
        for (auto &x : th) x.join();
        for (int t = 0; t < nthreads; t++)
            if (rcs[t] != ICG_OK) {
                set_error("%s", errs[t].c_str());
                return rcs[t];
            }
    }
    cudaStream_t s = h->stream;
    {
        const size_t nn = (size_t) n, PM = (size_t) C.K * (C.K - 1);
#define UP(field, stride) ICG_CUDA(h->field.up(s, nn * (size_t) (stride)))
        UP(dims, 1); UP(pose, C.K * 7); UP(mix, C.K * 9); UP(ext, 8); UP(rho, C.L);
        UP(f_active, C.F);
        UP(f_meta_s, C.F * 4); UP(vb_lm0, C.NVB); UP(f_const_s, C.F * 14); UP(lm_off, C.L + 1); UP(lm_perm, C.L); UP(ref_nrun, C.K); UP(part_off, PM + 1); UP(pair_ro, PM); UP(vis_ord, C.F);
        UP(npairs, 1); UP(imu_blob, C.K * ICG_IMU_BLOB_DOUBLES); UP(imu_U, C.K * 225);
        UP(gnss_node, C.G); UP(gnss_blh, C.G * 3); UP(gnss_std, C.G * 3); UP(lever, 3);
        UP(pose_prior, 7); UP(pose_prior_sinfo, 6); UP(mix_prior, 9); UP(mix_prior_std, 9);
        UP(marg_type, BA_MARG_MAXB); UP(marg_node, BA_MARG_MAXB); UP(marg_x0, BA_MARG_MAXB * 9); UP(marg_H0, (size_t) C.R * C.R); UP(marg_b0, C.R); UP(marg_c0, 1);
#undef UP
    }
    const BaDev &D = h->D;
    ICG_CUDA(cudaMemcpyAsync(D.pose_0, D.pose, sizeof(double) * (size_t) n * C.K * 7, cudaMemcpyDeviceToDevice, s));
    ICG_CUDA(cudaMemcpyAsync(D.mix_0, D.mix, sizeof(double) * (size_t) n * C.K * 9, cudaMemcpyDeviceToDevice, s));
    ICG_CUDA(cudaMemcpyAsync(D.ext_0, D.ext, sizeof(double) * (size_t) n * 8, cudaMemcpyDeviceToDevice, s));
    ICG_CUDA(cudaMemcpyAsync(D.rho_0, D.rho, sizeof(double) * (size_t) n * C.L, cudaMemcpyDeviceToDevice, s));
    ICG_CUDA(cudaMemcpyAsync(D.f_active_0, D.f_active, (size_t) n * C.F, cudaMemcpyDeviceToDevice, s));
    ICG_CUDA(cudaMemcpyAsync(D.gnss_std_0, D.gnss_std, sizeof(double) * (size_t) n * C.G * 3, cudaMemcpyDeviceToDevice, s));
    h->cur_windows = n;
    return ICG_OK;
}

static const char *PROF_NAMES[16] = {"(gap/other)", "lin_vis", "lin_lm", "", "", "schur_dmma (+ epilogue)", "join lin_cam + lin_done",
                                     "signal", "solve", "cost (+cost_cam)", "pack2 / exchange", "accept", "hsum / reduce", "join gram chain", "step_lm", ""};
static void prof_mark(icg_ba *h, int tag) {
    if (!h->prof) return;
    if (h->prof_used == h->prof_ev.size()) {
        cudaEvent_t e;
        cudaEventCreate(&e);
        h->prof_ev.push_back(e);
        h->prof_tag.push_back(0);
    }
    h->prof_tag[h->prof_used] = tag;
    cudaEventRecord(h->prof_ev[h->prof_used++], h->stream);
}
static void prof_collect(icg_ba *h) {
    if (!h->prof) return;
    if (h->prof_used && h->prof_skip > 0) {
        h->prof_skip--;
        h->prof_used = 0;
        return;
    }
    for (size_t i = 1; i < h->prof_used; i++) {
        float ms = 0;
        if (cudaEventElapsedTime(&ms, h->prof_ev[i - 1], h->prof_ev[i]) == cudaSuccess) {
            h->prof_ms[h->prof_tag[i]] += ms;
            h->prof_cnt[h->prof_tag[i]]++;
        }
    }
    h->prof_used = 0;
}
static void prof_print(icg_ba *h) {
    if (!h->prof) return;
    double tot = 0;
    for (int t = 0; t < 16; t++) tot += h->prof_ms[t];
    fprintf(stderr, "[icg_ba profile] handle %p, %d windows: stage totals over all recorded LM sequences (ms, mean us, share)\n", (void *) h, h->cur_windows);
    for (int t = 0; t < 16; t++)
        if (h->prof_cnt[t])
            fprintf(stderr, "  %-28s %9.3f ms  %8.1f us  %5.1f %%\n", PROF_NAMES[t], h->prof_ms[t], 1e3 * h->prof_ms[t] / h->prof_cnt[t], 100.0 * h->prof_ms[t] / tot);
    if (h->D.clk) {
        unsigned long long ck[48];
        if (cudaMemcpy(ck, h->D.clk, sizeof(ck), cudaMemcpyDeviceToHost) == cudaSuccess) {
            static const char *cn[6] = {"factor evaluation", "prior product + cost", "zero H_c", "prior blocks", "IMU J^T J", "GNSS / prior diagonals"};
            fprintf(stderr, "[icg_ba profile] ba_lin_cam phases of window 0 (SM cycles per call, mean):\n");
            for (int k = 0; k < 6; k++)
                if (ck[24 + k]) fprintf(stderr, "  %-28s %9.0f cycles\n", cn[k], (double) ck[16 + k] / (double) ck[24 + k]);
            if (h->D.S.split) {
                static const char *sn_l2[6] = {"per panel: stage B operand", "per panel: warp 0 tile + factor", "per panel: tiles + barrier 1", "per panel: row solve + barrier 2", "whole factorisation", ""};
                static const char *sn_dsm[6] = {"assembly", "per panel: warp 0 tile + factor", "per panel: until block barrier", "per panel: row solve + cl. barrier", "whole factorisation", "backward substitution"};
                const char **sn = h->solve_cam_dsm ? sn_dsm : sn_l2;
                fprintf(stderr, "[icg_ba profile] %s phases of window 0 (SM cycles, mean):\n", h->solve_cam_dsm ? "ba_solve_cam_dsm" : "ba_solve_cam");
                for (int k = 0; k < 6; k++)
                    if (ck[8 + k]) fprintf(stderr, "  %-34s %9.0f cycles\n", sn[k], (double) ck[k] / (double) ck[8 + k]);
                static const char *sn2[5] = {"per panel: wait for the panel column", "(unused)", "per panel: warp 0 diagonal-tile update", "per panel: warp 0 loads + 8x8 factorisation", "per panel: warp 0 write-back"};
                for (int k = 0; k < 5 && h->solve_cam_dsm; k++)
                    if (ck[40 + k]) fprintf(stderr, "  %-50s %9.0f cycles\n", sn2[k], (double) ck[32 + k] / (double) ck[40 + k]);
            }
            static const char *nm[8] = {"gradient / cost / tests", "assembly", "Cholesky", "camera back-substitution", "landmark back-substitution", "candidate + reductions",
                                        "  per panel: warp 0 tile+factor", "  per panel: row solve phase"};
            if (!h->D.S.split) fprintf(stderr, "[icg_ba profile] ba_solve phases of window 0 (SM cycles per call, mean):\n");
            for (int k = 0; k < 8 && !h->D.S.split; k++)
                if (ck[8 + k]) fprintf(stderr, "  %-28s %9.0f cycles\n", nm[k], (double) ck[k] / (double) ck[8 + k]);
        }
    }
}

static int enqueue_lm_split(icg_ba *h, int max_num_iterations);

static int enqueue_lm(icg_ba *h, int max_num_iterations) {
    if (h->D.S.split) return enqueue_lm_split(h, max_num_iterations);
    const BaCaps &C = h->C;
    const BaDev &D = h->D;
    const int n = h->cur_windows;
    cudaStream_t s = h->stream;
    const dim3 g_vis(C.NVB - 2, n), g_cost(h->nblk_vis, n);
    static const int cam_fork = getenv("ICG_BA_CAM_FORK") ? atoi(getenv("ICG_BA_CAM_FORK")) : 0;
    for (int it = 0; it <= max_num_iterations; it++) {
        if (cam_fork == 0) {
            ICG_CUDA(cudaEventRecord(h->ev_fork, s));
            ICG_CUDA(cudaStreamWaitEvent(h->stream_cam, h->ev_fork, 0));
            ba_lin_cam<<<n, h->cam_threads, h->smem_cam, h->stream_cam>>>(C, D);
            ICG_CUDA(cudaEventRecord(h->ev_join, h->stream_cam));
        }
        prof_mark(h, 0);
        ba_lin_vis<<<g_vis, 128, LV_SMEM, s>>>(C, D);
        prof_mark(h, 1);
        if (cam_fork != 0) {
            ICG_CUDA(cudaEventRecord(h->ev_fork, s));
            ICG_CUDA(cudaStreamWaitEvent(h->stream_cam, h->ev_fork, 0));
            ba_lin_cam<<<n, h->cam_threads, h->smem_cam, h->stream_cam>>>(C, D);
            ICG_CUDA(cudaEventRecord(h->ev_join, h->stream_cam));
        }
        if (!h->comm) {
            ICG_CUDA(cudaStreamWaitEvent(s, h->ev_join, 0));
            prof_mark(h, 6);
        }
        ba_schur_dmma<<<dim3(BA_SPLIT_W, n), 256, h->smem_schur, s>>>(C, D, h->ld_schur);
        prof_mark(h, 5);
        if (h->comm) {
            ICG_CUDA(cudaStreamWaitEvent(s, h->ev_join, 0));
            prof_mark(h, 6);
            int rc = nccl_allreduce(h, D.red, (size_t) n * (2 * (size_t) C.NCA * C.NCA + 8), 0);
            if (rc != ICG_OK) return rc;
            rc = nccl_allreduce(h, D.redmax, (size_t) n, 1);
            if (rc != ICG_OK) return rc;
            ba_hsum<<<dim3(((C.NCV + 1) * (C.NCV + 1) + 255) / 256, n), 256, 0, s>>>(C, D);
            prof_mark(h, 12);
        }
        ba_solve<<<n, SOLVE_THREADS, h->smem_solve, s>>>(C, D);
        prof_mark(h, 8);
        count_launch(h->comm ? 5 : 4);
        if (it == max_num_iterations) break;
        ICG_CUDA(cudaEventRecord(h->ev_fork, s));
        ICG_CUDA(cudaStreamWaitEvent(h->stream_cam, h->ev_fork, 0));
        ba_cost_cam<<<n, h->cam_threads, h->smem_cam, h->stream_cam>>>(C, D, h->nblk_vis);
        ICG_CUDA(cudaEventRecord(h->ev_join, h->stream_cam));
        ba_cost<<<g_cost, 256, 0, s>>>(C, D, h->nblk_vis);
        ICG_CUDA(cudaStreamWaitEvent(s, h->ev_join, 0));
        prof_mark(h, 9);
        if (h->comm) {
            ba_pack2<<<(n + 127) / 128, 128, 0, s>>>(C, D, n, h->nblk_vis);
            prof_mark(h, 10);
            int rc = nccl_allreduce(h, D.red2, (size_t) n * 4, 0);
            if (rc != ICG_OK) return rc;
        }
        ba_accept<<<n, 128, 0, s>>>(C, D, h->nblk_vis);
        prof_mark(h, 11);
        count_launch(h->comm ? 4 : 3);
    }
    ICG_CHECK_LAUNCH();
    return ICG_OK;
}

static void split_release(icg_ba *h) {
    for (int r = 0; r < 8; r++)
        if (h->ipc_opened[r]) cudaIpcCloseMemHandle(h->ipc_opened[r]), h->ipc_opened[r] = nullptr;
    if (h->xbuf) cudaFree(h->xbuf), h->xbuf = nullptr;
    if (h->D.S.redv) cudaFree(h->D.S.redv), h->D.S.redv = nullptr;
    if (h->D.S.err) cudaFree(h->D.S.err), h->D.S.err = nullptr;
    if (h->D.S.slm) cudaFree(h->D.S.slm), h->D.S.slm = nullptr;
    if (h->D.S.slm_cnt) cudaFree(h->D.S.slm_cnt), h->D.S.slm_cnt = nullptr;
    if (h->D.Sglobal) cudaFree(h->D.Sglobal), h->D.Sglobal = nullptr;
    h->D.S.split = 0;
}

static int split_setup(icg_ba *h, int rank, int world) {
    if (world < 1 || world > 8 || rank < 0 || rank >= world) {
        set_error("split pipeline: rank %d / world %d out of range (<= 8 GPUs of one box)", rank, world);
        return ICG_EINVAL;
    }
    ICG_CUDA(cudaSetDevice(h->device));
    ICG_CUDA(cudaStreamSynchronize(h->stream));
    split_release(h);
    const BaCaps &C = h->C;
    ShardDev &S = h->D.S;
    const size_t NW = C.NW, G = world;
    const size_t TRI = (size_t) C.NCV * (C.NCV + 1) / 2;
    S.PK = (int) ((TRI + 3 * (size_t) C.NCV + 4 + 3) & ~(size_t) 3);
    S.BS = (SPLIT_HDR + C.NS + 3) & ~3;
    S.RV = (3 * C.NCV + 4 + 3) & ~3;
    const size_t NWo = (NW + G - 1) / G;
    size_t off = 0;
    S.off_inbox = off, off += NWo * G * S.PK;
    S.off_bcast = off, off += NW * S.BS;
    S.off_scal = off, off += NW * G * SPLIT_SCAL;
    S.off_flagA = off, off += 8;
    S.off_flagB = off, off += (NW + 3) & ~(size_t) 3;
    S.off_flagC = off, off += (NW * G + 3) & ~(size_t) 3;
    h->xbuf_doubles = off;
    if (cudaMalloc(&h->xbuf, sizeof(double) * off) != cudaSuccess || cudaMalloc(&S.redv, sizeof(double) * NW * S.RV) != cudaSuccess ||
        cudaMalloc(&S.err, sizeof(int) * 4) != cudaSuccess || cudaMalloc(&S.slm, sizeof(double) * NW * STEP_SLICES * 8) != cudaSuccess ||
        cudaMalloc(&S.slm_cnt, sizeof(int) * NW) != cudaSuccess ||
        cudaMalloc(&h->D.Sglobal, sizeof(double) * NWo * split_S_stride(C)) != cudaSuccess) {
        set_error("split pipeline: allocation of the exchange buffers failed (%zu doubles)", off);
        return ICG_ENOMEM;
    }
    ICG_CUDA(cudaMemset(h->xbuf, 0, sizeof(double) * off));
    ICG_CUDA(cudaMemset(S.redv, 0, sizeof(double) * NW * S.RV));
    ICG_CUDA(cudaMemset(S.err, 0, sizeof(int) * 4));
    ICG_CUDA(cudaMemset(S.slm, 0, sizeof(double) * NW * STEP_SLICES * 8));
    ICG_CUDA(cudaMemset(S.slm_cnt, 0, sizeof(int) * NW));
    for (int r = 0; r < 8; r++) S.peer[r] = nullptr;
    S.peer[rank] = h->xbuf;
    S.split = 1;
    h->D.rank = rank, h->D.world = world;
    h->x_world = world;
    if (!getenv("ICG_BA_CAM_THREADS")) h->cam_threads = world >= 4 ? CAM_THREADS : 160;
    h->epoch = 0;
    {
        const size_t ldbp = ((size_t) (C.N + 15) / 16) * 16 + 8;
        const size_t bs = (size_t) SPLIT_BS_ROWS * (C.NS + 1), base = 8 * ldbp + 64, strips = (size_t) (SOLVE_THREADS / 32) * 8 * ldbp;
        h->solve_cam_stage_a = sizeof(double) * (40 + 4 * (size_t) C.NS + std::max(bs, base + strips)) <= 220 * 1024;
        h->smem_solve_cam = sizeof(double) * (40 + 4 * (size_t) C.NS + std::max(bs, base + (h->solve_cam_stage_a ? strips : 0)));
    }
    h->smem_step_lm = sizeof(double) * (40 + (size_t) C.NS);
    h->smem_solve_cam_dsm = sizeof(double) * dsm_smem_doubles(C);
    h->solve_cam_dsm = h->smem_solve_cam_dsm <= 227 * 1024 && C.N <= 32 * 11 && !getenv("ICG_BA_SOLVE_CAM_L2");
    if (h->solve_cam_dsm) ICG_CUDA(raise_dynamic_smem((const void *) ba_solve_cam_dsm, h->smem_solve_cam_dsm));
    h->dsm_variant = getenv("ICG_BA_DSM_VARIANT") ? atoi(getenv("ICG_BA_DSM_VARIANT")) : DSM_V_MBAR_BSUB;
    ICG_CUDA(raise_dynamic_smem((const void *) ba_solve_cam, (size_t) (h->smem_solve_cam)));
    ICG_CUDA(cudaFuncSetAttribute(ba_solve_cam, cudaFuncAttributeNonPortableClusterSizeAllowed, 0));
    ICG_CUDA(raise_dynamic_smem((const void *) ba_step_lm, (size_t) (h->smem_step_lm)));
    return ICG_OK;
}

static int launch_solve_cam(icg_ba *h, int n, unsigned long long epoch) {
    cudaLaunchConfig_t cfg;
    memset(&cfg, 0, sizeof(cfg));
    cfg.gridDim = dim3((unsigned) (n * SPLIT_CLUSTER)), cfg.blockDim = dim3(SOLVE_THREADS);
    cfg.dynamicSmemBytes = h->solve_cam_dsm ? h->smem_solve_cam_dsm : h->smem_solve_cam, cfg.stream = h->stream;
    cudaLaunchAttribute at[1];
    at[0].id = cudaLaunchAttributeClusterDimension;
    at[0].val.clusterDim.x = SPLIT_CLUSTER, at[0].val.clusterDim.y = 1, at[0].val.clusterDim.z = 1;
    cfg.attrs = at, cfg.numAttrs = 1;
    if (h->solve_cam_dsm) ICG_CUDA(cudaLaunchKernelEx(&cfg, ba_solve_cam_dsm, h->C, h->D, epoch, h->dsm_variant));
    else ICG_CUDA(cudaLaunchKernelEx(&cfg, ba_solve_cam, h->C, h->D, epoch, (int) h->solve_cam_stage_a));
    return ICG_OK;
}

static int enqueue_lm_split(icg_ba *h, int max_num_iterations) {
    const BaCaps &C = h->C;
    const BaDev &D = h->D;
    const int n = h->cur_windows;
    cudaStream_t s = h->stream;
    for (int r = 0; r < D.world; r++)
        if (!D.S.peer[r]) {
            set_error("landmark-sharded solve: peer %d is not connected (icg_ba_shard_connect)", r);
            return ICG_EINVAL;
        }
    const dim3 g_vis(C.NVB - 2, n), g_cost(h->nblk_vis, n), g_nn(((C.NCV + 1) * (C.NCV + 1) + 255) / 256, n);
    for (int it = 0; it <= max_num_iterations; it++) {
        const unsigned long long epoch = ++h->epoch;
        ICG_CUDA(cudaEventRecord(h->ev_fork, s));
        ICG_CUDA(cudaStreamWaitEvent(h->stream_cam, h->ev_fork, 0));
        ba_lin_cam<<<n, h->cam_threads, h->smem_cam, h->stream_cam>>>(C, D);
        ICG_CUDA(cudaEventRecord(h->ev_join, h->stream_cam));
        prof_mark(h, 0);
        ba_lin_vis<<<g_vis, 128, LV_SMEM, s>>>(C, D);
        prof_mark(h, 1);
        ba_schur_dmma<<<dim3(BA_SPLIT_W, n), 256, h->smem_schur, s>>>(C, D, h->ld_schur);
        prof_mark(h, 5);
        ba_signal<<<1, 32, 0, s>>>(D, epoch);
        prof_mark(h, 7);
        ICG_CUDA(cudaStreamWaitEvent(s, h->ev_join, 0));
        prof_mark(h, 6);
        ba_reduce<<<g_nn, 256, 0, s>>>(C, D, epoch);
        prof_mark(h, 12);
        int rc = launch_solve_cam(h, n, epoch);
        if (rc != ICG_OK) return rc;
        prof_mark(h, 8);
        ba_step_lm<<<dim3(n, STEP_SLICES), SOLVE_THREADS, h->smem_step_lm, s>>>(C, D, epoch);
        prof_mark(h, 14);
        count_launch(7);
        if (it == max_num_iterations) break;
        ICG_CUDA(cudaEventRecord(h->ev_fork, s));
        ICG_CUDA(cudaStreamWaitEvent(h->stream_cam, h->ev_fork, 0));
        ba_cost_cam<<<n, h->cam_threads, h->smem_cam, h->stream_cam>>>(C, D, h->nblk_vis);
        ICG_CUDA(cudaEventRecord(h->ev_join, h->stream_cam));
        ba_cost<<<g_cost, 256, 0, s>>>(C, D, h->nblk_vis);
        ICG_CUDA(cudaStreamWaitEvent(s, h->ev_join, 0));
        prof_mark(h, 9);
        ba_exchange<<<(n + 63) / 64, 64, 0, s>>>(C, D, n, h->nblk_vis, epoch);
        prof_mark(h, 10);
        ba_accept_split<<<n, 128, 0, s>>>(C, D, epoch);
        prof_mark(h, 11);
        count_launch(4);
    }
    ICG_CHECK_LAUNCH();
    return ICG_OK;
}

static int restore_params(icg_ba *h) {
    const BaCaps &C = h->C;
    const BaDev &D = h->D;
    const int n = h->cur_windows;
    cudaStream_t s = h->stream;
    ICG_CUDA(cudaMemcpyAsync(D.pose, D.pose_0, sizeof(double) * (size_t) n * C.K * 7, cudaMemcpyDeviceToDevice, s));
    ICG_CUDA(cudaMemcpyAsync(D.mix, D.mix_0, sizeof(double) * (size_t) n * C.K * 9, cudaMemcpyDeviceToDevice, s));
    ICG_CUDA(cudaMemcpyAsync(D.ext, D.ext_0, sizeof(double) * (size_t) n * 8, cudaMemcpyDeviceToDevice, s));
    ICG_CUDA(cudaMemcpyAsync(D.rho, D.rho_0, sizeof(double) * (size_t) n * C.L, cudaMemcpyDeviceToDevice, s));
    ICG_CUDA(cudaMemcpyAsync(D.f_active, D.f_active_0, (size_t) n * C.F, cudaMemcpyDeviceToDevice, s));
    ICG_CUDA(cudaMemcpyAsync(D.gnss_std, D.gnss_std_0, sizeof(double) * (size_t) n * C.G * 3, cudaMemcpyDeviceToDevice, s));
    ICG_CUDA(h->dims.up(s, n));
    return ICG_OK;
}

int icg_ba_run(icg_ba *h, int max_num_iterations, int restart) {
    if (!h || h->cur_windows < 1 || max_num_iterations < 0) {
        set_error("icg_ba_run: no problems uploaded");
        return ICG_EINVAL;
    }
    ICG_CUDA(cudaSetDevice(h->device));
    const int n = h->cur_windows;
    if (restart) {
        int rc = restore_params(h);
        if (rc != ICG_OK) return rc;
    }
    ba_reset_state<<<(n + 127) / 128, 128, 0, h->stream>>>(h->D, nullptr, n, max_num_iterations);
    count_launch();
    return enqueue_lm(h, max_num_iterations);
}

int icg_ba_run_gvins(icg_ba *h, int num_iterations, int restart) {
    if (!h || h->cur_windows < 1 || num_iterations < 1) {
        set_error("icg_ba_run_gvins: no problems uploaded");
        return ICG_EINVAL;
    }
    ICG_CUDA(cudaSetDevice(h->device));
    const BaCaps &C = h->C;
    const int n = h->cur_windows;
    const int first = num_iterations / 4, second = num_iterations - first;
    if (restart) {
        int rc = restore_params(h);
        if (rc != ICG_OK) return rc;
    }
    cudaStream_t s = h->stream;
    ba_set_gnss_huber<<<(n + 127) / 128, 128, 0, s>>>(h->D, n, 1);
    ba_reset_state<<<(n + 127) / 128, 128, 0, s>>>(h->D, nullptr, n, first);
    count_launch(2);
    int rc = enqueue_lm(h, first);
    if (rc != ICG_OK) return rc;
// ... 134 lines not shown
    if (!h || !problems || !num_marg || !out || n_windows < 1 || n_windows > h->C.NW) {
        set_error("icg_ba_marginalize: bad arguments");
        return ICG_EINVAL;
    }
    if (h->comm || h->D.world > 1) {
        set_error("icg_ba_marginalize: not available on a landmark-sharded handle (icg_ba_set_shard(world = 1) first)");
        return ICG_EUNSUPPORTED;
    }
    int rc = ICG_OK;
    if (resident) {
        if (h->cur_windows != n_windows) {
            set_error("icg_ba_marginalize_resident: the handle holds %d uploaded windows, the call names %d", h->cur_windows, n_windows);
            return ICG_EINVAL;
        }
        ICG_CUDA(cudaSetDevice(h->device));
    } else {
        rc = icg_ba_upload(h, n_windows, problems);
        if (rc != ICG_OK) return rc;
    }
    rc = marg_alloc(h);
    if (rc != ICG_OK) return rc;
    const BaCaps &C = h->C;
    MargDev &M = h->M;
    const int n = n_windows;
    for (int w = 0; w < n; w++) {
        const icg_ba_problem &p = problems[w];
        const int nm = num_marg[w];
        icg_ba_prior &o = out[w];
        if (nm < 1 || nm >= p.K || !o.block_type || !o.block_node || !o.x0 || !o.J0 || !o.e0 || o.rcap < 15 * (p.K - nm) + 7) {
            set_error("icg_ba_marginalize: window %d: num_marg=%d out of range or output arrays missing / too small (rcap=%d)", w, nm, o.rcap);
            return ICG_EINVAL;
        }
        int *map = h->marg_map.h + (size_t) w * M.map_stride;
        int *pose_col = map + MARG_MAP_HDR, *mix_col = pose_col + C.K, *lm_col = mix_col + C.K;
        std::vector<char> tp(p.K, 0), tm(p.K, 0), tl(p.L, 0);
        bool any_vis = false;
        for (int f = 0; f < p.F; f++) {
            if ((p.f_active && !p.f_active[f]) || p.f_ref[f] >= nm) continue;
            tl[p.f_lm[f]] = 1, tp[p.f_obs[f]] = 1, any_vis = true;
        }
        bool has_ext = any_vis, has_td = any_vis;
        for (int f = 0; f < p.F; f++)
            if (!(p.f_active && !p.f_active[f]) && p.f_ref[f] < nm) tp[p.f_ref[f]] = 1;
        for (int k = 0; k < nm && k < p.n_imu; k++) tp[k] = tm[k] = tp[k + 1] = tm[k + 1] = 1;
        for (int g = 0; g < p.n_gnss; g++)
            if (p.gnss_node[g] < nm) tp[p.gnss_node[g]] = 1;
        if (p.has_pose_prior) tp[0] = 1;
        if (p.has_mix_prior) tm[0] = 1;
        for (int b = 0; b < p.marg_nblocks && p.marg_r > 0; b++) {
            const int t = p.marg_block_type[b], nd = p.marg_block_node[b];
            if (t == 0) tp[nd] = 1;
            else if (t == 1) tm[nd] = 1;
            else if (t == 2) has_ext = true;
            else has_td = true;
        }
        int idx = 0;
        for (int k = 0; k < C.K; k++) pose_col[k] = mix_col[k] = -1;
        for (int k = 0; k < nm; k++) {
            if (tp[k]) pose_col[k] = idx, idx += 6;
            if (tm[k]) mix_col[k] = idx, idx += 9;
        }
        for (int l = 0; l < C.L; l++) lm_col[l] = -1;
        for (int l = 0; l < p.L; l++)
            if (tl[l]) lm_col[l] = idx++;
        const int m = idx;
        int nb = 0, xo = 0;
        for (int k = nm; k < p.K; k++) {
            if (tp[k]) pose_col[k] = idx, idx += 6, o.block_type[nb] = 0, o.block_node[nb++] = k - nm, xo += 7;
            if (tm[k]) mix_col[k] = idx, idx += 9, o.block_type[nb] = 1, o.block_node[nb++] = k - nm, xo += 9;
        }
        int ext_col = -1, td_col = -1;
        if (has_ext) ext_col = idx, idx += 6, o.block_type[nb] = 2, o.block_node[nb++] = 0, xo += 7;
        if (has_td) td_col = idx, idx += 1, o.block_type[nb] = 3, o.block_node[nb++] = 0, xo += 1;
        if (ext_col < 0) ext_col = 0;
        if (td_col < 0) td_col = 0;
        map[0] = m, map[1] = idx - m, map[2] = idx, map[3] = nm, map[4] = ext_col, map[5] = td_col, map[6] = map[7] = 0;
        o.m = m, o.r = idx - m, o.nblocks = nb;
    }
    cudaStream_t s = h->stream;
    ICG_CUDA(h->marg_map.up(s, (size_t) n * M.map_stride));
    const BaDev &D = h->D;
    const size_t smem = sizeof(double) * (8 * 480 + 2 * (size_t) C.R) + sizeof(int) * (size_t) C.R + 64;
    marg_prepare<<<(n + 127) / 128, 128, 0, s>>>(D, M, n, 0);
    ba_lin_vis<<<dim3(C.NVB - 2, n), 128, LV_SMEM, s>>>(C, D);
    marg_assemble<<<n, 256, smem, s>>>(C, D, M);
    int max_m = 0, max_r = 0;
    for (int w = 0; w < n; w++) max_m = std::max(max_m, out[w].m), max_r = std::max(max_r, out[w].r);
    auto jacobi = [&](int which, int nmax) -> int {
        if (nmax <= MARG_CTA_MAXN && !getenv("ICG_MARG_GLOBAL_JACOBI") && !getenv("ICG_MARG_PAIR_JACOBI")) {
            const size_t smem = sizeof(double) * 2 * (size_t) nmax * nmax;
            ICG_CUDA(raise_dynamic_smem((const void *) marg_jacobi_cta, smem));
            marg_jacobi_cta<<<n, MARG_CTA_THREADS, smem, s>>>(M, which);
        } else if (nmax <= MARG_PAIR_MAXN && !getenv("ICG_MARG_GLOBAL_JACOBI")) {
            const size_t smem = sizeof(double) * ((size_t) nmax * nmax + 2 * (size_t) (nmax + 2));
            cudaLaunchConfig_t cfg;
            memset(&cfg, 0, sizeof(cfg));
            cfg.gridDim = dim3((unsigned) (2 * n)), cfg.blockDim = dim3(MARG_THREADS), cfg.dynamicSmemBytes = smem, cfg.stream = s;
            cudaLaunchAttribute at[1];
            at[0].id = cudaLaunchAttributeClusterDimension;
            at[0].val.clusterDim.x = 2, at[0].val.clusterDim.y = 1, at[0].val.clusterDim.z = 1;
            cfg.attrs = at, cfg.numAttrs = 1;
            ICG_CUDA(raise_dynamic_smem((const void *) marg_jacobi_pair, (size_t) (smem)));
            ICG_CUDA(cudaLaunchKernelEx(&cfg, marg_jacobi_pair, M, which));
        } else {
            marg_jacobi<<<n, MARG_THREADS, 0, s>>>(M, which);
        }
        return ICG_OK;
    };
    rc = jacobi(0, max_m);
    if (rc != ICG_OK) return rc;
    marg_schur<<<n, MARG_THREADS, 0, s>>>(M);
    rc = jacobi(1, max_r);
    if (rc != ICG_OK) return rc;
    marg_finish<<<n, MARG_THREADS, 0, s>>>(M);
    marg_prepare<<<(n + 127) / 128, 128, 0, s>>>(D, M, n, 1);
    ICG_CHECK_LAUNCH();
    count_launch(9);
    {
        const size_t pitch = sizeof(double) * (size_t) M.rcap * M.rcap, used = sizeof(double) * (size_t) max_r * max_r;
        bool want_Hp = false;
        for (int w = 0; w < n; w++) want_Hp = want_Hp || out[w].Hp != nullptr;
        if (used) ICG_CUDA(cudaMemcpy2DAsync(h->marg_oJ0.h, pitch, h->marg_oJ0.d, pitch, used, (size_t) n, cudaMemcpyDeviceToHost, s));
        ICG_CUDA(h->marg_oe0.down(s, (size_t) n * M.rcap));
        if (want_Hp && used) ICG_CUDA(cudaMemcpy2DAsync(h->marg_oHp.h, pitch, h->marg_oHp.d, pitch, used, (size_t) n, cudaMemcpyDeviceToHost, s));
        ICG_CUDA(h->marg_obp.down(s, (size_t) n * M.rcap));
    }
    ICG_CUDA(cudaStreamSynchronize(s));
    auto write_back = [&](int w) {
        const icg_ba_problem &p = problems[w];
        icg_ba_prior &o = out[w];
        const int nm = num_marg[w], r = o.r;
        int xo = 0;
        for (int b = 0; b < o.nblocks; b++) {
            const int t = o.block_type[b], nd = o.block_node[b] + nm;
            const double *src = t == 0 ? p.pose + 7 * nd : t == 1 ? p.mix + 9 * nd : t == 2 ? p.ext : p.ext + 7;
            const int gs = t == 1 ? 9 : t == 3 ? 1 : 7;
            memcpy(o.x0 + xo, src, sizeof(double) * gs);
            xo += gs;
        }
        if (o.m <= 0) return;
        memcpy(o.J0, h->marg_oJ0.h + (size_t) w * M.rcap * M.rcap, sizeof(double) * (size_t) r * r);
        memcpy(o.e0, h->marg_oe0.h + (size_t) w * M.rcap, sizeof(double) * r);
        if (o.Hp) memcpy(o.Hp, h->marg_oHp.h + (size_t) w * M.rcap * M.rcap, sizeof(double) * (size_t) r * r);
        if (o.bp) memcpy(o.bp, h->marg_obp.h + (size_t) w * M.rcap, sizeof(double) * r);
    };
    {
        const int nthreads = std::max(1, std::min({n / 8, 8, (int) std::thread::hardware_concurrency()}));
        auto worker = [&](int t) {
            for (int w = t; w < n; w += nthreads) write_back(w);
        };
        std::vector<std::thread> th;
        for (int t = 1; t < nthreads; t++) th.emplace_back(worker, t);
        worker(0);
        for (auto &x : th) x.join();
    }
    return ICG_OK;
}

int icg_ba_marginalize(icg_ba *h, int n_windows, const icg_ba_problem *problems, const int32_t *num_marg, icg_ba_prior *out) {
    return marginalize_body(h, n_windows, problems, num_marg, out, false);
}

int icg_ba_marginalize_resident(icg_ba *h, int n_windows, const icg_ba_problem *problems, const int32_t *num_marg, icg_ba_prior *out) {
    return marginalize_body(h, n_windows, problems, num_marg, out, true);
}

int icg_nccl_unique_id(uint8_t *id128) {
// ... 358 lines not shown
```

ic_gvins_b200/csrc/ba_marg.cuh:

```cuda
#pragma once

namespace icg {

constexpr double MARG_EPS = 1e-8;
constexpr int MARG_THREADS = 512;
constexpr int MARG_MAP_HDR = 8;

struct MargDev {
    int *map;
    int map_stride;
    double *H0, *b0;
    double *G1, *V1;
    double *G2, *V2;
    double *lam1, *lam2;
    double *Z;
    double *Hp, *bp;
    double *J0, *e0;
    int *flags;
    int n0cap, mcap, rcap;
};

__global__ void marg_prepare(BaDev D, MargDev M, int n, int restore) {
    const int w = blockIdx.x * blockDim.x + threadIdx.x;
    if (w >= n) return;
// ... 46 lines not shown
                    s_dx[col + 3] = a.x, s_dx[col + 4] = a.y, s_dx[col + 5] = a.z;
                    const int base = t == 0 ? pose_col[nd] : ext_col;
                    for (int k = 0; k < 6; k++) s_cm[col + k] = base + k;
                    col += 6, xo += 7;
                } else if (t == 1) {
                    for (int k = 0; k < 9; k++) s_dx[col + k] = mix[nd * 9 + k] - x0[xo + k], s_cm[col + k] = mix_col[nd] + k;
                    col += 9, xo += 9;
                } else {
                    s_dx[col] = ext[7] - x0[xo], s_cm[col] = td_col;
                    col += 1, xo += 1;
                }
            }
        }
        __syncthreads();
        const double *Hq = D.marg_H0 + (size_t) w * C.R * C.R, *bq = D.marg_b0 + (size_t) w * C.R;
        for (int i = tid; i < r; i += blockDim.x) {
            double s = 0;
            for (int k = 0; k < r; k++) s += Hq[(size_t) i * r + k] * s_dx[k];
            s_y[i] = s;
        }
        __syncthreads();
        for (int e = tid; e < r * r; e += blockDim.x) {
            const int i = e / r, j = e - i * r;
            H0[(size_t) s_cm[i] * n0 + s_cm[j]] = Hq[e];
        }
        for (int i = tid; i < r; i += blockDim.x) b0[s_cm[i]] = -(bq[i] + s_y[i]);
        __syncthreads();
    }
    for (int k = 0; k < nm && k < dm.n_imu; k++) {
        double *rw = s_imu, *Jw = s_imu + 30;
        if (warp == 0)
            imu_factor_warp(D.imu_blob + ((size_t) w * C.K + k) * ICG_IMU_BLOB_DOUBLES, D.imu_U + ((size_t) w * C.K + k) * 225, pose + k * 7, mix + k * 9,
                            pose + (k + 1) * 7, mix + (k + 1) * 9, true, rw, Jw, lane);
        __syncthreads();
        auto gcol = [&](int c) { return c < 6 ? pose_col[k] + c : c < 15 ? mix_col[k] + c - 6 : c < 21 ? pose_col[k + 1] + c - 15 : mix_col[k + 1] + c - 21; };
        for (int e = tid; e < 930; e += blockDim.x) {
            if (e < 900) {
                const int a = e / 30, b = e - a * 30;
                double s = 0;
                for (int q = 0; q < 15; q++) s += Jw[q * 30 + a] * Jw[q * 30 + b];
                H0[(size_t) gcol(a) * n0 + gcol(b)] += s;
            } else {
                const int a = e - 900;
                double s = 0;
                for (int q = 0; q < 15; q++) s += Jw[q * 30 + a] * rw[q];
                b0[gcol(a)] -= s;
            }
        }
        __syncthreads();
    }
    for (int e = tid; e < nm * 42; e += blockDim.x) {
        const int k = e / 42, q = e % 42;
        if (k >= K || pose_col[k] < 0) continue;
        double s = 0;
        const int a = q < 36 ? q / 6 : q - 36, b = q % 6;
        for (int g = 0; g < dm.n_gnss; g++) {
            if (D.gnss_node[(size_t) w * C.G + g] != k) continue;
            double r3[3], J[18];
            gnss_eval(pose + k * 7, D.gnss_blh + ((size_t) w * C.G + g) * 3, D.gnss_std + ((size_t) w * C.G + g) * 3, D.lever + (size_t) w * 3, true, r3, J);
            if (q < 36)
                s += J[a] * J[b] + J[6 + a] * J[6 + b] + J[12 + a] * J[12 + b];
            else
                s += J[a] * r3[0] + J[6 + a] * r3[1] + J[12 + a] * r3[2];
        }
        if (k == 0 && dm.has_pose_prior) {
            double r6[6], J[36];
            pose_prior_eval(pose, D.pose_prior + (size_t) w * 7, D.pose_prior_sinfo + (size_t) w * 6, true, r6, J);
            for (int q6 = 0; q6 < 6; q6++) s += q < 36 ? J[q6 * 6 + a] * J[q6 * 6 + b] : J[q6 * 6 + a] * r6[q6];
        }
        if (q < 36)
            H0[(size_t) (pose_col[k] + a) * n0 + pose_col[k] + b] += s;
        else
            b0[pose_col[k] + a] -= s;
    }
    if (tid < 9 && dm.has_mix_prior) {
        const double sd = D.mix_prior_std[(size_t) w * 9 + tid];
        H0[(size_t) (mix_col[0] + tid) * n0 + mix_col[0] + tid] += 1.0 / (sd * sd);
        b0[mix_col[0] + tid] -= (mix[tid] - D.mix_prior[(size_t) w * 9 + tid]) / (sd * sd);
    }
    __syncthreads();
    {
        const int PM = C.K * (C.K - 1), P = D.npairs[w];
        const int *pro = D.pair_ro + (size_t) w * PM;
        const double *Mp = D.Mp + (size_t) w * PM * 210;
        int la = 0, lb = 0;
        if (tid < 210) {
            int e = tid;
            while (e >= 20 - la) e -= 20 - la, la++;
            lb = la + e;
        }
        for (int p = 0; p < P; p++) {
            const int ref = pro[p] >> 8, obs = pro[p] & 255;
            if (ref >= nm) continue;
            if (tid < 210) {
                auto gcol = [&](int c) { return c < 6 ? pose_col[ref] + c : c < 12 ? pose_col[obs] + c - 6 : c < 18 ? ext_col + c - 12 : td_col; };
                const double v = Mp[(size_t) p * 210 + tid];
                if (lb < 19) {
                    const int ca = gcol(la), cb = gcol(lb);
                    H0[(size_t) ca * n0 + cb] += v;
                    if (ca != cb) H0[(size_t) cb * n0 + ca] += v;
                } else if (la < 19) {
                    b0[gcol(la)] -= v;
                }
            }
            __syncthreads();
        }
    }
    for (int e = tid; e < dm.L * (NCV + 1); e += blockDim.x) {
        const int l = e / (NCV + 1), c = e - l * (NCV + 1);
        const int cl = lm_col[l];
        if (cl < 0) continue;
        const double v = D.AW[((size_t) w * C.LP + l) * C.NCA + c];
        if (c == NCV) {
            H0[(size_t) cl * n0 + cl] = D.hl[(size_t) w * C.L + l];
            b0[cl] = -v;
        } else {
            const int mc = c < 6 * K ? (pose_col[c / 6] < 0 ? -1 : pose_col[c / 6] + c % 6) : c < 6 * K + 6 ? ext_col + c - 6 * K : td_col;
            if (mc >= 0) H0[(size_t) cl * n0 + mc] = v, H0[(size_t) mc * n0 + cl] = v;
        }
    }
}

__device__ __forceinline__ bool jacobi_rotation(double al, double be, double ga, double &c, double &s) {
    if (ga == 0.0 || ga * ga <= 1e-30 * (al * be)) return false;
    const double zeta = (be - al) * (0.5 / ga);
    if (!(fabs(zeta) < 1e300)) return false;
    const double t = copysign(1.0, zeta) / (fabs(zeta) + sqrt(1.0 + zeta * zeta));
    c = rsqrt(1.0 + t * t), s = c * t;
    return true;
}

__global__ void __launch_bounds__(MARG_THREADS) marg_jacobi(MargDev M, int which) {
    __shared__ int s_rot[2];
    const int w = blockIdx.x, tid = threadIdx.x, lane = tid & 31, warp = tid >> 5, nwarps = MARG_THREADS / 32;
    const int *map = M.map + (size_t) w * M.map_stride;
    const int m = map[0], r = map[1], n0 = map[2];
    if (m <= 0) return;
    const int n = which == 0 ? m : r;
    const double *src = which == 0 ? M.H0 + (size_t) w * M.n0cap * M.n0cap : M.Hp + (size_t) w * M.rcap * M.rcap;
    const int lds = which == 0 ? n0 : r;
    double *G = which == 0 ? M.G1 + (size_t) w * M.mcap * M.mcap : M.G2 + (size_t) w * M.rcap * M.rcap;
    double *V = which == 0 ? M.V1 + (size_t) w * M.mcap * M.mcap : M.V2 + (size_t) w * M.rcap * M.rcap;
    double *lam = which == 0 ? M.lam1 + (size_t) w * M.mcap : M.lam2 + (size_t) w * M.rcap;
    for (int e = tid; e < n * n; e += MARG_THREADS) {
        const int j = e / n, i = e - j * n;
        G[e] = 0.5 * (src[(size_t) i * lds + j] + src[(size_t) j * lds + i]);
        V[e] = i == j ? 1.0 : 0.0;
    }
    if (tid < 2) s_rot[tid] = 0;
    __syncthreads();
    const int ne = (n + 1) & ~1, half = ne / 2;
    constexpr int RPL = 16;
    for (int sweep = 0; sweep < 40; sweep++) {
        for (int step = 0; step < ne - 1; step++) {
            for (int i = warp; i < half; i += nwarps) {
                int p = i == 0 ? ne - 1 : (step + i) % (ne - 1);
                int q = (step + ne - 1 - i) % (ne - 1);
                if (p >= n || q >= n) continue;
                if (p > q) {
                    const int t = p;
                    p = q, q = t;
                }
                double *gp = G + (size_t) p * n, *gq = G + (size_t) q * n, *vp = V + (size_t) p * n, *vq = V + (size_t) q * n;
                double a[RPL], b[RPL];
                double al = 0, be = 0, ga = 0, c, s;
#pragma unroll
                for (int k = 0; k < RPL; k++) {
                    const int row = lane + 32 * k;
                    a[k] = row < n ? gp[row] : 0.0;
                    b[k] = row < n ? gq[row] : 0.0;
                    al += a[k] * a[k], be += b[k] * b[k], ga += a[k] * b[k];
                }
#pragma unroll
                for (int o = 16; o > 0; o >>= 1) {
                    al += __shfl_xor_sync(0xffffffffu, al, o);
                    be += __shfl_xor_sync(0xffffffffu, be, o);
                    ga += __shfl_xor_sync(0xffffffffu, ga, o);
                }
                if (!jacobi_rotation(al, be, ga, c, s)) continue;
#pragma unroll
                for (int k = 0; k < RPL; k++) {
                    const int row = lane + 32 * k;
                    if (row < n) {
                        gp[row] = c * a[k] - s * b[k];
                        gq[row] = s * a[k] + c * b[k];
                        const double x = vp[row], y = vq[row];
                        vp[row] = c * x - s * y;
                        vq[row] = s * x + c * y;
                    }
                }
                if (lane == 0) s_rot[sweep & 1] = 1;
            }
            __syncthreads();
        }
        const int any = s_rot[sweep & 1];
        __syncthreads();
        if (tid == 0) s_rot[(sweep + 1) & 1] = 0;
// ... 301 lines not shown
```

ic_gvins_b200/csrc/ba_split.cuh:

```cuda
#pragma once
#include <cooperative_groups.h>

namespace icg {
namespace cg = cooperative_groups;

constexpr int SPLIT_CLUSTER = 4;
constexpr int SPLIT_HDR = 16;
constexpr int SPLIT_SCAL = 8;
constexpr int SPLIT_BS_ROWS = 32;

__device__ __forceinline__ unsigned long long ld_acquire_sys(const unsigned long long *p) {
    unsigned long long v;
    asm volatile("ld.acquire.sys.global.u64 %0, [%1];" : "=l"(v) : "l"(p) : "memory");
    return v;
}
__device__ __forceinline__ void st_release_sys(unsigned long long *p, unsigned long long v) {
    asm volatile("st.release.sys.global.u64 [%0], %1;" ::"l"(p), "l"(v) : "memory");
}
__device__ __forceinline__ void wait_flag(const unsigned long long *f, unsigned long long epoch, int *err) {
    const long long t0 = clock64();
    while (ld_acquire_sys(f) < epoch) {
        if (clock64() - t0 > 4000000000ll) {
            atomicExch(err, 1);
            break;
        }
        __nanosleep(64);
    }
}

__device__ __forceinline__ double *x_inbox(const BaDev &D, int peer, int w, int from) {
    const ShardDev &S = D.S;
    return S.peer[peer] + S.off_inbox + ((size_t) (w / D.world) * D.world + from) * S.PK;
}
__device__ __forceinline__ double *x_bcast(const BaDev &D, int peer, int w) { return D.S.peer[peer] + D.S.off_bcast + (size_t) w * D.S.BS; }
__device__ __forceinline__ double *x_scal(const BaDev &D, int peer, int w, int from) {
    return D.S.peer[peer] + D.S.off_scal + ((size_t) w * D.world + from) * SPLIT_SCAL;
}
__device__ __forceinline__ unsigned long long *x_flagA(const BaDev &D, int peer, int from) {
    return (unsigned long long *) (D.S.peer[peer] + D.S.off_flagA) + from;
}
__device__ __forceinline__ unsigned long long *x_flagB(const BaDev &D, int peer, int w) {
    return (unsigned long long *) (D.S.peer[peer] + D.S.off_flagB) + w;
}
__device__ __forceinline__ unsigned long long *x_flagC(const BaDev &D, int peer, int w, int from) {
    return (unsigned long long *) (D.S.peer[peer] + D.S.off_flagC) + (size_t) w * D.world + from;
}
__device__ __forceinline__ int tri_idx(int A, int B, int ncv) { return A * ncv - A * (A - 1) / 2 + (B - A); }

__global__ void ba_signal(BaDev D, unsigned long long epoch) {
    const int q = threadIdx.x;
    if (q >= D.world) return;
    __threadfence_system();
    st_release_sys(x_flagA(D, q, D.rank), epoch);
}

__global__ void __launch_bounds__(256) ba_reduce(BaCaps C, BaDev D, unsigned long long epoch) {
    const int w = blockIdx.y, tid = threadIdx.x;
    if (w % D.world != D.rank) return;
    if (D.st[w].done) return;
    const int K = D.dims[w].K, NCV = 6 * K + 7, nn = NCV + 1, TRI = NCV * (NCV + 1) / 2;
    if ((int) blockIdx.x * 256 >= nn * nn) return;
    if (tid < D.world) wait_flag(x_flagA(D, D.rank, tid), epoch, D.S.err);
    __syncthreads();
    const int t = blockIdx.x * 256 + tid;
    if (t >= nn * nn) return;
    const int A = t / nn, B = t - A * nn;
    if (B < A) return;
    const double *P0 = x_inbox(D, D.rank, w, 0);
    const size_t PK = D.S.PK;
    auto rsum = [&](int e) {
        double s = 0;
        for (int r = 0; r < D.world; r++) s += __ldcg(P0 + (size_t) r * PK + e);
        return s;
    };
    double *rv = D.S.redv + (size_t) w * D.S.RV;
    if (A < NCV && B < NCV) {
        D.Hs[(size_t) w * C.NS * C.NS + (size_t) B * C.NS + A] = D.Hc[(size_t) w * C.NS * C.NS + (size_t) B * C.NS + A] + rsum(tri_idx(A, B, NCV));
        if (A == B) rv[A] = rsum(TRI + A);
    } else if (A < NCV) {
        rv[NCV + A] = rsum(TRI + NCV + A);
        rv[2 * NCV + A] = rsum(TRI + 2 * NCV + A);
    } else {
        rv[3 * NCV] = rsum(TRI + 3 * NCV);
        rv[3 * NCV + 1] = rsum(TRI + 3 * NCV + 1);
        double m = 0;
        for (int r = 0; r < D.world; r++) m = fmax(m, __ldcg(P0 + (size_t) r * PK + TRI + 3 * NCV + 2));
        rv[3 * NCV + 2] = m;
    }
}

__host__ __device__ inline size_t split_S_stride(const BaCaps &C) { return (size_t) (C.N + 1) * (C.N + 2) / 2 + (size_t) C.NS; }

__global__ void __launch_bounds__(SOLVE_THREADS) ba_solve_cam(BaCaps C, BaDev D, unsigned long long epoch, int stage_a) {
    extern __shared__ double sm[];
    cg::cluster_group cluster = cg::this_cluster();
    const int CL = (int) cluster.num_blocks(), cr = (int) cluster.block_rank();
    const int w = blockIdx.x / CL, tid = threadIdx.x, lane = tid & 31, warp = tid >> 5;
    if (w % D.world != D.rank) return;
    LmState &st = D.st[w];
    if (st.done) return;
    const WinDims dm = D.dims[w];
    const int K = dm.K, NCV = 6 * K + 7, N = 15 * K + 7, NR = N + 1;
    const int CT = CL * SOLVE_THREADS, ctid = cr * SOLVE_THREADS + tid, cwarp = ctid >> 5, ncwarps = CT / 32;
    const int f_first = st.first, f_fresh = st.fresh_lin, f_last = st.last_success, f_iter = st.iter, f_maxit = st.max_iter;
    const double radius = st.radius, cost_cam = st.cost_cam, gmax_old = st.gmax, xcost_old = st.x_cost, init_old = st.initial_cost;
    double *s_red = sm;
    double *s_scale = s_red + 40;
    double *s_g = s_scale + C.NS;
    double *s_rhs = s_g + C.NS;
    double *s_d2 = s_rhs + C.NS;
    double *s_blk = s_d2 + C.NS;
    double *S = D.Sglobal + (size_t) (w / D.world) * split_S_stride(C);
    const double *Hc = D.Hc + (size_t) w * C.NS * C.NS, *gcam = D.gc + (size_t) w * C.NS, *Hs = D.Hs + (size_t) w * C.NS * C.NS;
    const double *rv = D.S.redv + (size_t) w * D.S.RV;
    double *scale_c = D.scale_c + (size_t) w * C.NS;
    for (int a = tid; a < N; a += SOLVE_THREADS) {
        const double g = gcam[a] + (a < NCV ? rv[NCV + a] : 0.0);
        s_g[a] = g;
        const double h = Hc[(size_t) a * C.NS + a] + (a < NCV ? rv[a] : 0.0);
        const double sc = f_first ? 1.0 / (1.0 + sqrt(h)) : scale_c[a];
        s_scale[a] = sc;
        const double hs = sc * sc * h;
        s_d2[a] = fmin(fmax(hs, 1e-6), 1e32) / radius;
        s_rhs[a] = -sc * (g - (a < NCV ? rv[2 * NCV + a] : 0.0));
    }
    __syncthreads();
    double gmax_now = gmax_old, x_cost = xcost_old;
    if (f_fresh) {
        double gm = 0;
        for (int a = tid; a < N; a += SOLVE_THREADS) gm = fmax(gm, fabs(s_g[a]));
        gm = fmax(block_max(gm, s_red), rv[3 * NCV + 2]);
        gmax_now = gm;
        x_cost = rv[3 * NCV] + cost_cam;
    }
    int term = 0;
    if (f_iter >= f_maxit) term = 1;
    else if (f_last && gmax_now <= 1e-10) term = 2;
    else if (f_last && radius <= 1e-32) term = 2;
    cluster.sync();
    if (cr == 0 && tid == 0) {
        st.x_cost = x_cost, st.gmax = gmax_now;
        if (f_first) st.initial_cost = x_cost;
        st.fresh_lin = 0, st.first = 0, st.need_lin = 0;
        if (term) st.done = term, st.step_valid = 0;
        else st.iter = f_iter + 1;
    }
    if (cr == 0 && f_first)
        for (int a = tid; a < N; a += SOLVE_THREADS) scale_c[a] = s_scale[a];
    double *BC = nullptr;
    if (term) {
        if (cr == 0) {
            __syncthreads();
            for (int q = tid; q < D.world; q += SOLVE_THREADS) {
                BC = x_bcast(D, q, w);
                BC[0] = (double) term, BC[1] = 0.0, BC[2] = x_cost, BC[3] = gmax_now, BC[4] = f_first ? x_cost : init_old, BC[5] = 0.0;
                __threadfence_system();
                st_release_sys(x_flagB(D, q, w), epoch);
            }
        }
        return;
    }
    for (int i = cwarp; i < N; i += ncwarps) {
        const double *src = (i < NCV ? Hs : Hc) + (size_t) i * C.NS;
        double *dst = S + (size_t) i * (i + 1) / 2;
        const double si = s_scale[i];
        for (int j = lane; j <= i; j += 32) {
            double v = si * s_scale[j] * src[j];
            if (i == j) v += s_d2[i];
            dst[j] = v;
        }
    }
    for (int a = ctid; a < N; a += CT) S[(size_t) N * (N + 1) / 2 + a] = s_rhs[a];
    cluster.sync();
    double *dinvg = S + (size_t) (C.N + 1) * (C.N + 2) / 2;
    double *s_b = s_blk;
    const int ldbp = ((C.N + 15) / 16) * 16 + 8;
    int fail = 0;
#ifdef ICG_BA_PHASE_CLOCKS
#define CAMS_CLK(k, t0)                                                                                             \
    if (D.clk && w == 0 && ctid == 0) atomicAdd(&D.clk[k], clock64() - (t0)), atomicAdd(&D.clk[8 + (k)], 1ull);
#define CAMS_NOW() clock64()
#else
#define CAMS_CLK(k, t0)
#define CAMS_NOW() 0ull
#endif
    const unsigned long long tc_all = CAMS_NOW();
    (void) tc_all;
    for (int J0 = 0; J0 < N; J0 += BA_CHOL_NB) {
        const int nb = min(BA_CHOL_NB, N - J0);
        const int g = lane >> 2, kk = lane & 3;
        const int ntile = (NR - J0 + 7) / 8;
        const unsigned long long tc0 = CAMS_NOW();
        (void) tc0;
        if (J0 > 0) {
            for (int e = tid; e < 8 * J0; e += SOLVE_THREADS) {
                const int r = e / J0, c = e - r * J0, row = J0 + r;
// ... 207 lines not shown
            part += -0.5 * sp * (s_scale[a] * s_g[a]) + 0.5 * s_d2[a] * sp * sp;
        }
    const double mcc = block_sum(part, s_red);
    const double nfin = block_sum(finite ? 0.0 : 1.0, s_red);
    for (int q = 0; q < D.world; q++) {
        BC = x_bcast(D, q, w);
        if (valid)
            for (int a = tid; a < N; a += SOLVE_THREADS) BC[SPLIT_HDR + a] = y[a] * s_scale[a];
        if (tid == 0) {
            BC[0] = 0.0, BC[1] = (valid && nfin == 0.0) ? 1.0 : 0.0, BC[2] = x_cost, BC[3] = gmax_now, BC[4] = f_first ? x_cost : init_old, BC[5] = mcc;
        }
    }
    __threadfence_system();
    __syncthreads();
    for (int q = tid; q < D.world; q += SOLVE_THREADS) st_release_sys(x_flagB(D, q, w), epoch);
}

constexpr int DSM_CL = 4;
static_assert(SOLVE_THREADS == 256 && DSM_CL == SPLIT_CLUSTER, "ba_solve_cam_dsm: warp r assembles row r of a tile row; one launch geometry for both forms");
__host__ __device__ inline int dsm_tile_off(int cr, int m) { return m * cr + 2 * m * (m - 1); }
__host__ __device__ constexpr int dsm_ntiles(int NR) { return (NR + 7) / 8; }
__host__ inline size_t dsm_smem_doubles(const BaCaps &C) {
    const int nt = dsm_ntiles(C.N + 1);
    int mx = 0;
    for (int cr = 0; cr < DSM_CL; cr++) {
        int s = 0;
        for (int T = cr; T < nt; T += DSM_CL) s += T;
        mx = s > mx ? s : mx;
    }
    return 40 + 8 * (size_t) nt * 8 + 64 + 8 + 8 * DSM_CL + 8 + 8 + (size_t) nt * 64 * 3 + (size_t) mx * 64;
}

__device__ __forceinline__ unsigned mapa_u32(unsigned addr, unsigned rank) {
    unsigned r;
    asm volatile("mapa.shared::cluster.u32 %0, %1, %2;" : "=r"(r) : "r"(addr), "r"(rank));
    return r;
}
__device__ __forceinline__ void dsm_mbar_init(unsigned bar, unsigned count) { asm volatile("mbarrier.init.shared::cta.b64 [%0], %1;" ::"r"(bar), "r"(count) : "memory"); }
__device__ __forceinline__ void dsm_mbar_arrive_local(unsigned bar) { asm volatile("mbarrier.arrive.release.cta.shared::cta.b64 _, [%0];" ::"r"(bar) : "memory"); }
__device__ __forceinline__ void dsm_mbar_arrive_expect_tx_remote(unsigned bar_cluster, unsigned tx) {
    asm volatile("mbarrier.arrive.expect_tx.release.cluster.shared::cluster.b64 _, [%0], %1;" ::"r"(bar_cluster), "r"(tx) : "memory");
}
__device__ __forceinline__ void st_async_v2(unsigned dst_cluster, double a, double b, unsigned bar_cluster) {
    asm volatile("st.async.weak.shared::cluster.mbarrier::complete_tx::bytes.v2.f64 [%0], {%1, %2}, [%3];" ::"r"(dst_cluster), "d"(a), "d"(b), "r"(bar_cluster) : "memory");
}
__device__ __forceinline__ void st_async_f64(unsigned dst_cluster, double a, unsigned bar_cluster) {
    asm volatile("st.async.weak.shared::cluster.mbarrier::complete_tx::bytes.f64 [%0], %1, [%2];" ::"r"(dst_cluster), "d"(a), "r"(bar_cluster) : "memory");
}
__device__ __forceinline__ bool dsm_mbar_try_wait(unsigned bar, unsigned parity) {
    unsigned ok;
    asm volatile("{\n\t.reg .pred p;\n\tmbarrier.try_wait.parity.acquire.cluster.shared::cta.b64 p, [%1], %2;\n\tselp.u32 %0, 1, 0, p;\n\t}" : "=r"(ok) : "r"(bar), "r"(parity) : "memory");
    return ok != 0;
}
__device__ __forceinline__ void dsm_mbar_wait(unsigned bar, unsigned parity, volatile int *s_dead, int *err) {
    if (dsm_mbar_try_wait(bar, parity)) return;
    const long long t0 = clock64();
    while (!dsm_mbar_try_wait(bar, parity)) {
        if (*s_dead) return;
        if (clock64() - t0 > 400000000ll) {
            *s_dead = 1;
            atomicExch(err, 1);
            return;
        }
    }
}

constexpr int DSM_V_MBAR_PANEL = 1, DSM_V_MBAR_BSUB = 2;
__global__ void __launch_bounds__(SOLVE_THREADS, 1) ba_solve_cam_dsm(BaCaps C, BaDev D, unsigned long long epoch, int variant) {
    extern __shared__ double sm[];
    cg::cluster_group cluster = cg::this_cluster();
    constexpr int CL = DSM_CL;
    const int cr = (int) cluster.block_rank();
    const int w = blockIdx.x / CL, tid = threadIdx.x, lane = tid & 31, warp = tid >> 5;
    if (w % D.world != D.rank) return;
    LmState &st = D.st[w];
    if (st.done) return;
    const bool use_mbar = variant & DSM_V_MBAR_PANEL, bsub_mbar = variant & DSM_V_MBAR_BSUB;
    const WinDims dm = D.dims[w];
    const int K = dm.K, NCV = 6 * K + 7, N = 15 * K + 7, NR = N + 1;
    const int ntc = dsm_ntiles(C.N + 1), VL = ntc * 8;
    const int nt = dsm_ntiles(NR), npan = (N + 7) / 8;
    const int Tn = N >> 3, rn = N & 7;
    const int f_first = st.first, f_fresh = st.fresh_lin, f_last = st.last_success, f_iter = st.iter, f_maxit = st.max_iter;
    const double radius = st.radius, cost_cam = st.cost_cam, gmax_old = st.gmax, xcost_old = st.x_cost, init_old = st.initial_cost;
    double *s_red = sm;
    double *s_scale = s_red + 40;
    double *s_g = s_scale + VL;
    double *s_rhs = s_g + VL;
    double *s_d2 = s_rhs + VL;
    double *s_y = s_d2 + VL;
    double *s_contrib = s_y + VL;
    double *s_x = s_contrib + VL;
    double *s_dinv = s_x + VL;
    double *s_Lf = s_dinv + VL;
    double *s_dv = s_Lf + 64;
    double *s_inbox = s_dv + 8;
    double *s_xT = s_inbox + 8 * CL;
    int *s_fail = (int *) (s_xT + 8);
    unsigned long long *s_bar = (unsigned long long *) (s_xT + 12);
    double *s_dg = s_xT + 16;
    double *s_P = s_dg + (size_t) ntc * 64;
    double *s_tiles = s_P + (size_t) 2 * ntc * 64;
    const double *Hc = D.Hc + (size_t) w * C.NS * C.NS, *gcam = D.gc + (size_t) w * C.NS, *Hs = D.Hs + (size_t) w * C.NS * C.NS;
    const double *rv = D.S.redv + (size_t) w * D.S.RV;
    double *scale_c = D.scale_c + (size_t) w * C.NS;
    for (int a = tid; a < VL; a += SOLVE_THREADS) {
        double g = 0, sc = 0, d2 = 0, rh = 0;
        if (a < N) {
            g = gcam[a] + (a < NCV ? rv[NCV + a] : 0.0);
            const double h = Hc[(size_t) a * C.NS + a] + (a < NCV ? rv[a] : 0.0);
            sc = f_first ? 1.0 / (1.0 + sqrt(h)) : scale_c[a];
            const double hs = sc * sc * h;
            d2 = fmin(fmax(hs, 1e-6), 1e32) / radius;
            rh = -sc * (g - (a < NCV ? rv[2 * NCV + a] : 0.0));
        }
        s_g[a] = g, s_scale[a] = sc, s_d2[a] = d2, s_rhs[a] = rh;
        s_y[a] = 0, s_contrib[a] = 0, s_x[a] = 0, s_dinv[a] = 0;
    }
    if (tid < 8 * CL) s_inbox[tid] = 0;
    if (tid == 0) {
        s_fail[0] = 0, s_fail[1] = 0;
        dsm_mbar_init(smem_u32(s_bar), CL), dsm_mbar_init(smem_u32(s_bar + 1), CL), dsm_mbar_init(smem_u32(s_bar + 2), CL - 1);
        asm volatile("fence.mbarrier_init.release.cluster;" ::: "memory");
    }
    __syncthreads();
    double gmax_now = gmax_old, x_cost = xcost_old;
    if (f_fresh) {
        double gm = 0;
        for (int a = tid; a < N; a += SOLVE_THREADS) gm = fmax(gm, fabs(s_g[a]));
        gm = fmax(block_max(gm, s_red), rv[3 * NCV + 2]);
        gmax_now = gm;
        x_cost = rv[3 * NCV] + cost_cam;
    }
    int term = 0;
    if (f_iter >= f_maxit) term = 1;
    else if (f_last && gmax_now <= 1e-10) term = 2;
    else if (f_last && radius <= 1e-32) term = 2;
    cluster.sync();
    if (cr == 0 && tid == 0) {
        st.x_cost = x_cost, st.gmax = gmax_now;
        if (f_first) st.initial_cost = x_cost;
        st.fresh_lin = 0, st.first = 0, st.need_lin = 0;
        if (term) st.done = term, st.step_valid = 0;
        else st.iter = f_iter + 1;
    }
    if (cr == 0 && f_first)
        for (int a = tid; a < N; a += SOLVE_THREADS) scale_c[a] = s_scale[a];
    double *BC = nullptr;
    if (term) {
        if (cr == 0) {
            __syncthreads();
            for (int q = tid; q < D.world; q += SOLVE_THREADS) {
                BC = x_bcast(D, q, w);
                BC[0] = (double) term, BC[1] = 0.0, BC[2] = x_cost, BC[3] = gmax_now, BC[4] = f_first ? x_cost : init_old, BC[5] = 0.0;
                __threadfence_system();
                st_release_sys(x_flagB(D, q, w), epoch);
            }
        }
        return;
    }
#ifdef ICG_BA_PHASE_CLOCKS
#define DSM_CLK(k, t0)                                                                                             \
    if (D.clk && w == 0 && cr == 0 && tid == 0) atomicAdd(&D.clk[k], clock64() - (t0)), atomicAdd(&D.clk[8 + (k)], 1ull);
#define DSM_CLK2(k, t0)                                                                                            \
    if (D.clk && w == 0 && cr == 0 && tid == 0) atomicAdd(&D.clk[32 + (k)], clock64() - (t0)), atomicAdd(&D.clk[40 + (k)], 1ull);
#define DSM_NOW() clock64()
#else
#define DSM_CLK(k, t0)
#define DSM_CLK2(k, t0)
#define DSM_NOW() 0ull
#endif
    const unsigned long long tq0 = DSM_NOW();
    (void) tq0;
    for (int m = 0, T = cr; T < nt; m += 2, T += 2 * CL) {
        constexpr int NCH = (15 * 22 + 7 + 31) / 32;
        double v[2][NCH];
#pragma unroll
        for (int h = 0; h < 2; h++) {
            const int Th = T + h * CL, i = 8 * Th + warp, ncol = 8 * Th;
            const double *src = (i < NCV ? Hs : Hc) + (size_t) (i < N ? i : 0) * C.NS;
#pragma unroll
            for (int u = 0; u < NCH; u++) {
                const int j = 32 * u + lane;
                v[h][u] = (Th < nt && j < ncol && i < N) ? __ldcg(src + j) : 0.0;
            }
        }
// ... 284 lines not shown
                        s_contrib[col] = acc;
                        const int q = (col >> 3) % CL;
                        if (bsub_mbar) {
                            const unsigned abar = mapa_u32(smem_u32(s_bar + 2), q);
                            st_async_f64(mapa_u32(smem_u32(s_inbox + cr * 8 + (col & 7)), q), acc, abar);
                            if ((col & 7) == 0) dsm_mbar_arrive_expect_tx_remote(abar, 64u);
                        } else {
                            cluster.map_shared_rank(s_inbox, q)[cr * 8 + (col & 7)] = acc;
                        }
                    }
                }
                __syncthreads();
                for (int col = tid; col < c0; col += SOLVE_THREADS) {
                    const double *tp = trow + (col >> 3) * 64 + (col & 7);
                    double acc = s_contrib[col];
#pragma unroll
                    for (int r = 0; r < 8; r++) acc += tp[r * 8] * s_xT[r];
                    s_contrib[col] = acc;
                }
                __syncthreads();
            }
            if (!bsub_mbar) cluster.sync();
        }
    }
    cluster.sync();
    DSM_CLK(5, tb0)
    if (cr != 0) return;
    double part = 0;
    bool finite = true;
    if (valid)
        for (int a = tid; a < N; a += SOLVE_THREADS) {
            const double sp = s_x[a];
            finite = finite && isfinite(sp);
            part += -0.5 * sp * (s_scale[a] * s_g[a]) + 0.5 * s_d2[a] * sp * sp;
        }
    const double mcc = block_sum(part, s_red);
    const double nfin = block_sum(finite ? 0.0 : 1.0, s_red);
    for (int q = 0; q < D.world; q++) {
        BC = x_bcast(D, q, w);
        if (valid)
            for (int a = tid; a < N; a += SOLVE_THREADS) BC[SPLIT_HDR + a] = s_x[a] * s_scale[a];
        if (tid == 0) {
            BC[0] = 0.0, BC[1] = (valid && nfin == 0.0) ? 1.0 : 0.0, BC[2] = x_cost, BC[3] = gmax_now, BC[4] = f_first ? x_cost : init_old, BC[5] = mcc;
        }
    }
    __threadfence_system();
    __syncthreads();
    for (int q = tid; q < D.world; q += SOLVE_THREADS) st_release_sys(x_flagB(D, q, w), epoch);
}

constexpr int STEP_SLICES = 4;
__global__ void __launch_bounds__(SOLVE_THREADS) ba_step_lm(BaCaps C, BaDev D, unsigned long long epoch) {
    extern __shared__ double sm[];
    __shared__ int s_last;
    const int w = blockIdx.x, sl_id = blockIdx.y, tid = threadIdx.x;
    LmState &st = D.st[w];
    const WinDims dm = D.dims[w];
    const int K = dm.K, L = dm.L, NCV = 6 * K + 7, N = 15 * K + 7;
    const bool owner = (w % D.world) == D.rank;
    double *s_red = sm, *s_dl = s_red + 40;
    if (st.done) return;
    const double *BC = x_bcast(D, D.rank, w);
    if (tid == 0) wait_flag(x_flagB(D, D.rank, w), epoch, D.S.err);
    __syncthreads();
    const int term = (int) __ldcg(BC + 0), valid = (int) __ldcg(BC + 1);
    double *R3 = D.red2 + (size_t) w * 4;
    if (!owner && tid == 0 && sl_id == 0) {
        st.x_cost = __ldcg(BC + 2), st.gmax = __ldcg(BC + 3), st.initial_cost = __ldcg(BC + 4);
        st.fresh_lin = 0, st.first = 0, st.need_lin = 0;
        if (term) st.done = term, st.step_valid = 0;
        else st.iter = st.iter + 1;
    }
    if (term) return;
    if (!valid) {
        if (tid == 0 && sl_id == 0) {
            st.chol_ok = 0, st.step_valid = 0;
            R3[0] = 0, R3[1] = 0, R3[2] = 1, R3[3] = 0;
        }
        return;
    }
    for (int a = tid; a < N; a += SOLVE_THREADS) s_dl[a] = __ldcg(BC + SPLIT_HDR + a);
    __syncthreads();
    const double radius = st.radius;
    const double *hl = D.hl + (size_t) w * C.L, *gl = D.gl + (size_t) w * C.L, *scale_l = D.scale_l + (size_t) w * C.L;
    double *step_l = D.step_l + (size_t) w * C.L;
    const double *AW = D.AW + (size_t) w * C.LP * C.NCA;
    const double *rho = D.rho + (size_t) w * C.L;
    double *rho_c = D.rho_c + (size_t) w * C.L;
    constexpr int LB = 4;
    const int per = ((L + STEP_SLICES - 1) / STEP_SLICES + LB - 1) / LB * LB;
    const int lbeg = min(L, sl_id * per), lend = min(L, lbeg + per);
    double part = 0, sn_l = 0, rho2 = 0;
    bool finite = true;
    {
        const int lane = tid & 31, warp = tid >> 5;
        for (int l0 = lbeg + LB * warp; l0 < lend; l0 += LB * (SOLVE_THREADS / 32)) {
            double d[LB];
#pragma unroll
            for (int u = 0; u < LB; u++) d[u] = 0;
            for (int c = lane; c < NCV; c += 32) {
                const double sx = s_dl[c];
#pragma unroll
                for (int u = 0; u < LB; u++) d[u] += (l0 + u < lend ? AW[(size_t) (l0 + u) * C.NCA + c] : 0.0) * sx;
            }
            double mine = 0;
#pragma unroll
            for (int u = 0; u < LB; u++) {
#pragma unroll
                for (int o = 16; o > 0; o >>= 1) d[u] += __shfl_xor_sync(0xffffffffu, d[u], o);
                if (lane == u) mine = d[u];
            }
            if (lane < LB && l0 + lane < lend) {
                const int l = l0 + lane;
                const double sl = scale_l[l], hs = sl * sl * hl[l], d2 = fmin(fmax(hs, 1e-6), 1e32) / radius;
                const double sp = (-sl * gl[l] - sl * mine) / (hs + d2);
                finite = finite && isfinite(sp);
                step_l[l] = sp;
                part += -0.5 * sp * (sl * gl[l]) + 0.5 * d2 * sp * sp;
                const double r0 = rho[l], v = r0 + sp * sl;
                rho_c[l] = v;
                sn_l += (r0 - v) * (r0 - v);
                rho2 += r0 * r0;
            }
        }
    }
    __syncthreads();
    const double mcc_l = block_sum(part, s_red);
    const double nfin = block_sum(finite ? 0.0 : 1.0, s_red);
    sn_l = block_sum(sn_l, s_red);
    rho2 = block_sum(rho2, s_red);
    double sn_cam = 0;
    if (sl_id == 0) {
        const double *pose = D.pose + (size_t) w * C.K * 7, *mix = D.mix + (size_t) w * C.K * 9, *ext = D.ext + (size_t) w * 8;
        double *pose_c = D.pose_c + (size_t) w * C.K * 7, *mix_c = D.mix_c + (size_t) w * C.K * 9, *ext_c = D.ext_c + (size_t) w * 8;
        for (int k = tid; k <= K; k += SOLVE_THREADS) {
            const bool is_ext = (k == K);
            const double *x = is_ext ? ext : pose + k * 7;
            double *xc = is_ext ? ext_c : pose_c + k * 7;
            if (is_ext && dm.ext_const) {
                for (int e = 0; e < 7; e++) xc[e] = x[e];
            } else {
                const int c0 = is_ext ? col_ext(K) : col_pose(k);
                double d[6];
                for (int e = 0; e < 6; e++) d[e] = s_dl[c0 + e];
                pose_plus(x, d, xc);
                for (int e = 0; e < 7; e++) sn_cam += (x[e] - xc[e]) * (x[e] - xc[e]);
            }
        }
        for (int e = tid; e < K * 9; e += SOLVE_THREADS) {
            const int k = e / 9, q = e - 9 * k;
            const double v = mix[e] + s_dl[col_mix(K, k) + q];
            mix_c[e] = v;
            sn_cam += (mix[e] - v) * (mix[e] - v);
        }
        if (tid == 0) {
            if (dm.td_const) {
                ext_c[7] = ext[7];
            } else {
                const double v = ext[7] + s_dl[col_td(K)];
                ext_c[7] = v;
                sn_cam += (ext[7] - v) * (ext[7] - v);
            }
        }
    }
    sn_cam = block_sum(sn_cam, s_red);
    double *slot = D.S.slm + ((size_t) w * STEP_SLICES + sl_id) * 8;
    if (tid == 0) {
        slot[0] = mcc_l, slot[1] = sn_l, slot[2] = nfin, slot[3] = rho2, slot[4] = sn_cam;
        __threadfence();
// ... 111 lines not shown
```

Baseline: 21950.

## Linearize at candidate into double buffer, replacing separate cost evaluation

Adds double-buffered linearization storage (Mp, AW, costf, hl, gl, Hc, gc) and lets the lin kernels run at the candidate state into the inactive buffer. In the single-device path, the separate cost kernels are replaced by this candidate linearization, and ba_accept sums candidate cost from costf. On acceptance the buffer index flips, so the next iteration reuses the already-computed Jacobians instead of relinearizing. This saves a cost pass and a relinearization per accepted step, but computes full Jacobians even for rejected steps and doubles the workspace memory.

```diff
diff --git a/ic_gvins_b200/csrc/ba.cu b/ic_gvins_b200/csrc/ba.cu
--- a/ic_gvins_b200/csrc/ba.cu
+++ b/ic_gvins_b200/csrc/ba.cu
@@ -37,8 +37,10 @@
 };
 
 struct LmState {
-    double radius, decrease_factor, x_cost, x_norm, cand_cost, model_cost_change, step_norm, gmax, initial_cost, cost_cam;
+    double radius, decrease_factor, x_cost, x_norm, cand_cost, model_cost_change, step_norm, gmax, initial_cost;
+    double cost_cam[2];
     int iter, n_success, n_invalid, done, need_lin, last_success, first, step_valid, fresh_lin, max_iter, chol_ok;
+    int lin_buf;
 };
 
 struct ShardDev {
@@ -72,11 +74,12 @@
     int *part_off, *pair_ro, *npairs;
     double *gpart;
     int *vis_cnt;
-    double *Mp;
-    double *AW;
-    double *costf;
-    double *hl, *gl, *scale_l, *scale_c;
-    double *Hc, *gc;
+    double *Mp[2];
+    double *AW[2];
+    double *costf[2];
+    double *hl[2], *gl[2];
+    double *Hc[2], *gc[2];
+    double *scale_l, *scale_c;
     double *Hs;
     double *visv;
     double *imu_blob, *imu_U;
@@ -95,6 +98,14 @@
     unsigned long long *clk;
 };
 
+__device__ __forceinline__ double *lin_Mp(const BaCaps &C, const BaDev &D, int b, int w) { return D.Mp[b] + (size_t) w * C.K * (C.K - 1) * 210; }
+__device__ __forceinline__ double *lin_AW(const BaCaps &C, const BaDev &D, int b, int w) { return D.AW[b] + (size_t) w * C.LP * C.NCA; }
+__device__ __forceinline__ double *lin_costf(const BaCaps &C, const BaDev &D, int b, int w) { return D.costf[b] + (size_t) w * C.F; }
+__device__ __forceinline__ double *lin_hl(const BaCaps &C, const BaDev &D, int b, int w) { return D.hl[b] + (size_t) w * C.L; }
+__device__ __forceinline__ double *lin_gl(const BaCaps &C, const BaDev &D, int b, int w) { return D.gl[b] + (size_t) w * C.L; }
+__device__ __forceinline__ double *lin_Hc(const BaCaps &C, const BaDev &D, int b, int w) { return D.Hc[b] + (size_t) w * C.NS * C.NS; }
+__device__ __forceinline__ double *lin_gc(const BaCaps &C, const BaDev &D, int b, int w) { return D.gc[b] + (size_t) w * C.NS; }
+
 __device__ __forceinline__ int col_pose(int k) { return 6 * k; }
 __device__ __forceinline__ int col_ext(int K) { return 6 * K; }
 __device__ __forceinline__ int col_td(int K) { return 6 * K + 6; }
@@ -110,14 +121,16 @@
 }
 constexpr int LV_LD = 45;
 constexpr size_t LV_SMEM = sizeof(double) * (128 * LV_LD + (BA_MAX_NODES + 1) * NODE_FRAME_LD);
-__global__ void __launch_bounds__(128, 4) ba_lin_vis(BaCaps C, BaDev D) {
+__global__ void __launch_bounds__(128, 4) ba_lin_vis(BaCaps C, BaDev D, int at_cand) {
     extern __shared__ double lv_sm[];
     __shared__ int s_ord[128], s_gbeg[BA_MAX_NODES], s_gend[BA_MAX_NODES], s_last, s_p0, s_np;
     double (*s_rec)[LV_LD] = (double (*)[LV_LD]) lv_sm;
     double (*s_frame)[NODE_FRAME_LD] = (double (*)[NODE_FRAME_LD]) (lv_sm + 128 * LV_LD);
     const int w = blockIdx.y;
     const LmState &st = D.st[w];
-    if (st.done || !st.need_lin) return;
+    if (st.done || !(at_cand ? st.step_valid : st.need_lin)) return;
+    const int b = at_cand ? 1 - st.lin_buf : st.lin_buf;
+    const double *pose = at_cand ? D.pose_c : D.pose, *xext = at_cand ? D.ext_c : D.ext, *rho = at_cand ? D.rho_c : D.rho;
     const int *vb = D.vb_lm0 + (size_t) w * C.NVB;
     if ((int) blockIdx.x >= vb[C.NVB - 1]) return;
     const WinDims dm = D.dims[w];
@@ -125,7 +138,7 @@
     const int *off = D.lm_off + (size_t) w * (C.L + 1);
     const int pA = vb[blockIdx.x], pB = vb[blockIdx.x + 1];
     const int s0 = off[pA], nslot = off[pB] - s0;
-    if (tid <= dm.K) node_frame(tid < dm.K ? D.pose + ((size_t) w * C.K + tid) * 7 : D.ext + (size_t) w * 8, s_frame[tid]);
+    if (tid <= dm.K) node_frame(tid < dm.K ? pose + ((size_t) w * C.K + tid) * 7 : xext + (size_t) w * 8, s_frame[tid]);
     if (tid < BA_MAX_NODES) s_gbeg[tid] = s_gend[tid] = 0;
     if (tid == 0) s_np = 0;
     __syncthreads();
@@ -135,8 +148,8 @@
         const int4 meta = ((const int4 *) D.f_meta_s)[(size_t) w * C.F + q];
         const int i = meta.y, j = meta.z, f = meta.w;
         if (D.f_active[(size_t) w * C.F + f] != 0) {
-            const double *ext = D.ext + (size_t) w * 8;
-            reproj_eval_frames(s_frame[i], s_frame[j], s_frame[dm.K], D.rho[(size_t) w * C.L + meta.x], ext[7],
+            const double *ext = xext + (size_t) w * 8;
+            reproj_eval_frames(s_frame[i], s_frame[j], s_frame[dm.K], rho[(size_t) w * C.L + meta.x], ext[7],
                                D.f_const_s + ((size_t) w * C.F + q) * 14, dm.reproj_sinv, true, r, Ji, Jj, Je, Jr, Jt);
             if (dm.ext_const)
                 for (int k = 0; k < 12; k++) Je[k] = 0;
@@ -154,7 +167,7 @@
             for (int k = 0; k < 12; k++) Ji[k] = Jj[k] = Je[k] = 0;
             Jr[0] = Jr[1] = Jt[0] = Jt[1] = r[0] = r[1] = 0;
         }
-        D.costf[(size_t) w * C.F + f] = cost;
+        lin_costf(C, D, b, w)[f] = cost;
         double *sr = s_rec[tid];
 #pragma unroll
         for (int k = 0; k < 12; k++) sr[k] = Ji[k], sr[12 + k] = Jj[k], sr[24 + k] = Je[k];
@@ -227,7 +240,7 @@
     }
     for (int pl = pA + grp; pl < pB; pl += 16) {
         const int l = perm[pl], f0 = off[pl] - s0, nf = off[pl + 1] - off[pl];
-        double *row = D.AW + ((size_t) w * C.LP + l) * C.NCA;
+        double *row = lin_AW(C, D, b, w) + (size_t) l * C.NCA;
         for (int c = sl; c < NCA; c += 8) row[c] = 0.0;
         __syncwarp(0xffu << (tid & 24));
         double acc[3] = {0, 0, 0};
@@ -260,9 +273,9 @@
             }
             if (c == 19) {
                 row[NCV] = acc[t];
-                D.gl[(size_t) w * C.L + l] = acc[t];
+                lin_gl(C, D, b, w)[l] = acc[t];
             } else if (c == 20) {
-                D.hl[(size_t) w * C.L + l] = acc[t];
+                lin_hl(C, D, b, w)[l] = acc[t];
                 if (st.first) D.scale_l[(size_t) w * C.L + l] = 1.0 / (1.0 + sqrt(acc[t]));
             }
         }
@@ -284,7 +297,7 @@
         }
     __syncthreads();
     const double *part = D.gpart + (size_t) w * C.GQ * 210;
-    double *Mp = D.Mp + (size_t) w * PM * 210;
+    double *Mp = lin_Mp(C, D, b, w);
     for (int p = s_p0 + warp; p < s_p0 + s_np; p += 4) {
         const int k0 = poff[p], k1 = poff[p + 1];
         double acc[7];
@@ -312,9 +325,9 @@
     for (int p = threadIdx.x; p < P; p += blockDim.x) s_slot[(pro[p] >> 8) * K + (pro[p] & 255)] = (short) p;
     __syncthreads();
 }
-__device__ __forceinline__ double gram2_entry(const BaCaps &C, const BaDev &D, int w, int K, const short *s_slot, int A, int B) {
-    const int PM = C.K * (C.K - 1), P = D.npairs[w];
-    const double *Mp = D.Mp + (size_t) w * PM * 210;
+__device__ __forceinline__ double gram2_entry(const BaCaps &C, const BaDev &D, int buf, int w, int K, const short *s_slot, int A, int B) {
+    const int P = D.npairs[w];
+    const double *Mp = lin_Mp(C, D, buf, w);
     const int bA = A < 6 * K ? A / 6 : K, bB = B < 6 * K ? B / 6 : K;
     const int a = A - 6 * bA, b = B - 6 * bB;
     const int ga = 12 + a, gb = 12 + b;
@@ -359,13 +372,13 @@
 __device__ __forceinline__ double *x_inbox(const BaDev &D, int peer, int w, int from);
 __device__ __forceinline__ int tri_idx(int A, int B, int ncv);
 
-__device__ __forceinline__ void schur_store(const BaCaps &C, const BaDev &D, int w, int K, const short *s_slot, int A, int B, double cw) {
+__device__ __forceinline__ void schur_store(const BaCaps &C, const BaDev &D, int buf, int w, int K, const short *s_slot, int A, int B, double cw) {
     const int NCV = 6 * K + 7;
     const bool nccl = !D.S.split && D.world > 1;
     if (A == NCV && !nccl) return;
     const size_t e = (size_t) w * C.NS * C.NS + (size_t) B * C.NS + A;
-    const double hc = !D.S.split && !nccl && B < NCV ? D.Hc[e] : 0.0;
-    const double cj = gram2_entry(C, D, w, K, s_slot, A, B);
+    const double hc = !D.S.split && !nccl && B < NCV ? lin_Hc(C, D, buf, w)[(size_t) B * C.NS + A] : 0.0;
+    const double cj = gram2_entry(C, D, buf, w, K, s_slot, A, B);
     if (D.S.split) {
         double *P = x_inbox(D, w % D.world, w, D.rank);
         const int TRI = NCV * (NCV + 1) / 2;
@@ -395,11 +408,12 @@
 __device__ __forceinline__ void schur_scalars(const BaCaps &C, const BaDev &D, int w, const WinDims &dm, double *s_red) {
     const int tid = threadIdx.x;
     double c = 0, q = 0, gm = 0;
-    for (int f = tid; f < dm.F; f += 256) c += D.costf[(size_t) w * C.F + f];
+    const double *costf = lin_costf(C, D, 0, w), *gl = lin_gl(C, D, 0, w);
+    for (int f = tid; f < dm.F; f += 256) c += costf[f];
     for (int l = tid; l < dm.L; l += 256) {
         const double r = D.rho[(size_t) w * C.L + l];
         q += r * r;
-        gm = fmax(gm, fabs(D.gl[(size_t) w * C.L + l]));
+        gm = fmax(gm, fabs(gl[l]));
     }
     c = block_sum(c, s_red);
     q = block_sum(q, s_red);
@@ -433,7 +447,8 @@
     const int T2 = (NCA + 15) / 16, nsuper = T2 * (T2 + 1) / 2;
     const int tid = threadIdx.x, lane = tid & 31, warp = tid >> 5, g = lane >> 2, kk = lane & 3;
     double *sphi = sA + (size_t) SCHUR_RCH * ld;
-    const double *A = D.AW + (size_t) w * C.LP * C.NCA;
+    const int b = st.lin_buf;
+    const double *A = lin_AW(C, D, b, w), *hl = lin_hl(C, D, b, w);
     const double radius = st.radius;
     const int nsteps = (dm.L + 3) / 4;
     const int r_beg = 4 * (int) ((long long) nsteps * split / BA_SPLIT_W), r_end = min(dm.L, 4 * (int) ((long long) nsteps * (split + 1) / BA_SPLIT_W));
@@ -489,7 +504,7 @@
                 double ph = 0;
                 if (rr < nr) {
                     const int l = r0 + rr;
-                    const double sl = D.scale_l[(size_t) w * C.L + l], hs = sl * sl * D.hl[(size_t) w * C.L + l];
+                    const double sl = D.scale_l[(size_t) w * C.L + l], hs = sl * sl * hl[l];
                     ph = sl * sl / (hs + fmin(fmax(hs, 1e-6), 1e32) / radius);
                 }
                 sphi[rr] = ph;
@@ -541,7 +556,7 @@
             int a = 0, e = SCHUR_PASS * pass + sl;
             while (e >= T2 - a) e -= T2 - a, a++;
             const int r = 16 * a + r_in, cc = 16 * (a + e) + c_in;
-            if (r <= cc && cc <= NCV) schur_store(C, D, w, dm.K, s_slot, r, cc, cw[j]);
+            if (r <= cc && cc <= NCV) schur_store(C, D, b, w, dm.K, s_slot, r, cc, cw[j]);
         }
     }
     if (split == 0 && (D.S.split || D.world > 1)) schur_scalars(C, D, w, dm, s_red);
@@ -615,10 +630,10 @@
 __device__ __forceinline__ void red_add(double *p, double v) { asm volatile("red.global.add.f64 [%0], %1;" ::"l"(p), "d"(v) : "memory"); }
 
 __device__ double cam_factors(const BaCaps &C, const BaDev &D, int w, const WinDims &dm, const double *pose, const double *mix, const double *ext,
-                              bool lin, double *smem) {
+                              bool lin, int b, double *smem) {
     const int tid = threadIdx.x, lane = tid & 31, warp = tid >> 5, nwarps = blockDim.x >> 5;
     const int K = dm.K, N = 15 * K + 7;
-    double *Hc = D.Hc + (size_t) w * C.NS * C.NS, *gc = D.gc + (size_t) w * C.NS;
+    double *Hc = lin_Hc(C, D, b, w), *gc = lin_gc(C, D, b, w);
     double *s_imu = smem;
     double *s_gnss = s_imu + (size_t) C.K * 480;
     double *s_misc = s_gnss + (size_t) C.G * 24;
@@ -790,15 +805,17 @@
 }
 
 constexpr int CAM_THREADS = 320;
-__global__ void __launch_bounds__(CAM_THREADS) ba_lin_cam(BaCaps C, BaDev D) {
+__global__ void __launch_bounds__(CAM_THREADS) ba_lin_cam(BaCaps C, BaDev D, int at_cand) {
     extern __shared__ double smem[];
     const int w = blockIdx.x;
     LmState &st = D.st[w];
-    if (st.done || !st.need_lin) return;
+    if (st.done || !(at_cand ? st.step_valid : st.need_lin)) return;
     if (D.S.split && (w % D.world) != D.rank) return;
     const WinDims dm = D.dims[w];
-    double c = cam_factors(C, D, w, dm, D.pose + (size_t) w * C.K * 7, D.mix + (size_t) w * C.K * 9, D.ext + (size_t) w * 8, true, smem);
-    if (threadIdx.x == 0) st.cost_cam = c;
+    const int b = at_cand ? 1 - st.lin_buf : st.lin_buf;
+    const double *pose = at_cand ? D.pose_c : D.pose, *mix = at_cand ? D.mix_c : D.mix, *ext = at_cand ? D.ext_c : D.ext;
+    double c = cam_factors(C, D, w, dm, pose + (size_t) w * C.K * 7, mix + (size_t) w * C.K * 9, ext + (size_t) w * 8, true, b, smem);
+    if (threadIdx.x == 0) st.cost_cam[b] = c;
 }
 
 __global__ void ba_pack2(BaCaps C, BaDev D, int n, int nblk_vis) {
@@ -826,7 +843,7 @@
     if (B < A || B >= NCV) return;
     const double *RED = D.red + (size_t) w * (2 * NN + 8);
     const double cj = RED[(size_t) B * C.NCA + A], cw = RED[NN + (size_t) B * C.NCA + A];
-    D.Hs[(size_t) w * C.NS * C.NS + (size_t) B * C.NS + A] = D.Hc[(size_t) w * C.NS * C.NS + (size_t) B * C.NS + A] + (cj - cw);
+    D.Hs[(size_t) w * C.NS * C.NS + (size_t) B * C.NS + A] = lin_Hc(C, D, 0, w)[(size_t) B * C.NS + A] + (cj - cw);
 }
 
 constexpr int SOLVE_THREADS = 256;
@@ -893,7 +910,8 @@
     double *s_d2 = s_rhs + C.NS;
     double *s_diag = s_d2 + C.NS;
     double *S = s_diag + C.NS;
-    const double *Hc = D.Hc + (size_t) w * C.NS * C.NS, *gcam = D.gc + (size_t) w * C.NS, *Hs = D.Hs + (size_t) w * C.NS * C.NS;
+    const int b = st.lin_buf;
+    const double *Hc = lin_Hc(C, D, b, w), *gcam = lin_gc(C, D, b, w), *Hs = D.Hs + (size_t) w * C.NS * C.NS;
     const bool sharded = D.world > 1;
     const int NN = C.NCA * C.NCA;
     const double *RED = D.red + (size_t) w * (2 * NN + 8), *V = D.visv + (size_t) w * 3 * C.NCV;
@@ -903,7 +921,7 @@
     const double camw = D.rank == 0 ? 1.0 : 0.0;
     if (tid == 0 && st.need_lin) st.need_lin = 0;
     double *scale_c = D.scale_c + (size_t) w * C.NS;
-    const double *hl = D.hl + (size_t) w * C.L, *gl = D.gl + (size_t) w * C.L, *scale_l = D.scale_l + (size_t) w * C.L;
+    const double *hl = lin_hl(C, D, b, w), *gl = lin_gl(C, D, b, w), *scale_l = D.scale_l + (size_t) w * C.L;
 
     for (int a = tid; a < N; a += SOLVE_THREADS) {
         double g = gcam[a];
@@ -924,7 +942,8 @@
             gml = D.redmax[w];
         } else {
             double cs = 0, gq = 0;
-            for (int f = tid; f < dm.F; f += SOLVE_THREADS) cs += D.costf[(size_t) w * C.F + f];
+            const double *costf = lin_costf(C, D, b, w);
+            for (int f = tid; f < dm.F; f += SOLVE_THREADS) cs += costf[f];
             for (int l = tid; l < L; l += SOLVE_THREADS) gq = fmax(gq, fabs(gl[l]));
             c = block_sum(cs, s_red);
             gml = block_max(gq, s_red);
@@ -934,7 +953,7 @@
         gm = fmax(block_max(gm, s_red), gml);
         gmax_now = gm;
         if (tid == 0) {
-            st.x_cost = c + st.cost_cam;
+            st.x_cost = c + st.cost_cam[b];
             st.gmax = gm;
             if (f_first) st.initial_cost = st.x_cost;
             st.fresh_lin = 0;
@@ -1190,7 +1209,7 @@
     __syncthreads();
     SOLVE_CLK(3)
     double *step_l = D.step_l + (size_t) w * C.L;
-    const double *AW = D.AW + (size_t) w * C.LP * C.NCA;
+    const double *AW = lin_AW(C, D, b, w);
     double part = 0;
     bool finite = true;
     double *R2 = D.red2 + (size_t) w * 4;
@@ -1319,7 +1338,7 @@
     if (st.done || !st.step_valid) return;
     if (D.S.split && (w % D.world) != D.rank) return;
     const WinDims dm = D.dims[w];
-    double c = cam_factors(C, D, w, dm, D.pose_c + (size_t) w * C.K * 7, D.mix_c + (size_t) w * C.K * 9, D.ext_c + (size_t) w * 8, false, smem);
+    double c = cam_factors(C, D, w, dm, D.pose_c + (size_t) w * C.K * 7, D.mix_c + (size_t) w * C.K * 9, D.ext_c + (size_t) w * 8, false, 0, smem);
     if (threadIdx.x == 0) D.cost_part[(size_t) w * (nblk_vis + 1) + nblk_vis] = c;
 }
 __global__ void __launch_bounds__(256) ba_cost(BaCaps C, BaDev D, int nblk_vis) {
@@ -1351,7 +1370,7 @@
     if (threadIdx.x == 0) part[blockIdx.x] = cost;
 }
 
-__global__ void __launch_bounds__(128) ba_accept(BaCaps C, BaDev D, int nblk_vis) {
+__global__ void __launch_bounds__(128) ba_accept(BaCaps C, BaDev D) {
     __shared__ int s_accept;
     __shared__ double s_camsq, s_rhosq;
     __shared__ double s_red[40];
@@ -1378,17 +1397,33 @@
         }
         if (tid == 0) s_camsq = s, s_rhosq = q;
     }
+    extern __shared__ double s_warp[];
+    const int lane = tid & 31, warp = tid >> 5, ngrp = (dm.F + 31) / 32;
+    const bool cand_here = D.world == 1 && st.step_valid;
+    if (cand_here) {
+        const double *costf = lin_costf(C, D, 1 - st.lin_buf, w);
+        const int4 *meta = (const int4 *) D.f_meta_s + (size_t) w * C.F;
+#pragma unroll 4
+        for (int g = warp; g < ngrp; g += 4) {
+            const int q = 32 * g + lane;
+            double v = q < dm.F ? costf[meta[q].w] : 0.0;
+            for (int o = 16; o > 0; o >>= 1) v += __shfl_down_sync(0xffffffffu, v, o);
+            if (lane == 0) s_warp[g] = v;
+        }
+    }
     __syncthreads();
     if (tid == 0) {
         s_accept = 0;
         const double mcc = R2[0], sn = R2[1], nfin = R2[2];
         double cand = R2[3];
-        if (D.world == 1 && st.step_valid) {
-            const double *part = D.cost_part + (size_t) w * (nblk_vis + 1);
+        if (cand_here) {
             cand = 0;
-            const int nb = (dm.F + 255) / 256;
-            for (int b = 0; b < nb; b++) cand += part[b];
-            cand += part[nblk_vis];
+            for (int g0 = 0; g0 < ngrp; g0 += 8) {
+                double t = 0;
+                for (int k = 0; k < 8; k++) t += g0 + k < ngrp ? s_warp[g0 + k] : 0.0;
+                cand += t;
+            }
+            cand += st.cost_cam[1 - st.lin_buf];
         }
         if (!chol_ok || nfin != 0.0 || !(mcc > 0.0)) {
             st.step_valid = 0;
@@ -1415,8 +1450,11 @@
                     st.radius = fmin(1e16, st.radius / fmax(1.0 / 3.0, 1.0 - t * t * t));
                     st.decrease_factor = 2.0;
                     st.last_success = 1;
-                    st.need_lin = 1;
                     st.fresh_lin = 1;
+                    if (D.world == 1)
+                        st.lin_buf ^= 1;
+                    else
+                        st.need_lin = 1;
                 } else {
                     st.radius = st.radius / st.decrease_factor;
                     st.decrease_factor *= 2.0;
@@ -1849,9 +1887,9 @@
     if (rc == ICG_OK) rc = dmalloc(h, &D.field, count);
     DM(pose_c, NW * C.K * 7) DM(mix_c, NW * C.K * 9) DM(ext_c, NW * 8) DM(rho_c, NW * C.L)
     DM(pose_0, NW * C.K * 7) DM(mix_0, NW * C.K * 9) DM(ext_0, NW * 8) DM(rho_0, NW * C.L)
-    DM(AW, NW * C.NCA * C.LP) DM(Mp, NW * (size_t) C.K * (C.K - 1) * 210) DM(visv, NW * 3 * C.NCV)
-    DM(gpart, NW * (size_t) C.GQ * 210) DM(costf, NW * C.F) DM(hl, NW * C.L) DM(gl, NW * C.L) DM(scale_l, NW * C.L) DM(scale_c, NW * C.NS)
-    DM(Hc, NW * C.NS * C.NS) DM(gc, NW * C.NS) DM(Hs, NW * C.NS * C.NS) DM(cost_part, NW * (h->nblk_vis + 1)) DM(red, NW * (2 * (size_t) C.NCA * C.NCA + 8)) DM(redmax, NW) DM(red2, NW * 4) DM(step_c, NW * C.NS) DM(step_l, NW * C.L)
+    DM(AW[0], NW * C.NCA * C.LP) DM(Mp[0], NW * (size_t) C.K * (C.K - 1) * 210) DM(visv, NW * 3 * C.NCV)
+    DM(gpart, NW * (size_t) C.GQ * 210) DM(costf[0], NW * C.F) DM(hl[0], NW * C.L) DM(gl[0], NW * C.L) DM(scale_l, NW * C.L) DM(scale_c, NW * C.NS)
+    DM(Hc[0], NW * C.NS * C.NS) DM(gc[0], NW * C.NS) DM(Hs, NW * C.NS * C.NS) DM(cost_part, NW * (h->nblk_vis + 1)) DM(red, NW * (2 * (size_t) C.NCA * C.NCA + 8)) DM(redmax, NW) DM(red2, NW * 4) DM(step_c, NW * C.NS) DM(step_l, NW * C.L)
 #undef DM
     if (rc == ICG_OK) rc = dmalloc(h, &D.gnss_std_0, NW * C.G * 3);
     if (rc == ICG_OK) {
@@ -2147,7 +2185,7 @@
     return ICG_OK;
 }
 
-static const char *PROF_NAMES[16] = {"(gap/other)", "lin_vis", "lin_lm", "", "", "schur_dmma (+ epilogue)", "join lin_cam + lin_done",
+static const char *PROF_NAMES[16] = {"(gap/other)", "lin_vis", "lin_lm", "lin at candidate", "","schur_dmma (+ epilogue)", "join lin_cam + lin_done",
                                      "signal", "solve", "cost (+cost_cam)", "pack2 / exchange", "accept", "hsum / reduce", "join gram chain", "step_lm", ""};
 static void prof_mark(icg_ba *h, int tag) {
     if (!h->prof) return;
@@ -2213,33 +2251,59 @@
 
 static int enqueue_lm_split(icg_ba *h, int max_num_iterations);
 
+static int alloc_lin_buf2(icg_ba *h) {
+    BaDev &D = h->D;
+    if (D.Mp[1]) return ICG_OK;
+    const BaCaps &C = h->C;
+    const size_t NW = C.NW;
+    int rc = ICG_OK;
+#define DM(field, count) \
+    if (rc == ICG_OK) rc = dmalloc(h, &D.field, count);
+    DM(AW[1], NW * C.NCA * C.LP) DM(Mp[1], NW * (size_t) C.K * (C.K - 1) * 210) DM(costf[1], NW * C.F) DM(hl[1], NW * C.L) DM(gl[1], NW * C.L)
+    DM(Hc[1], NW * C.NS * C.NS) DM(gc[1], NW * C.NS)
+#undef DM
+    return rc;
+}
+
 static int enqueue_lm(icg_ba *h, int max_num_iterations) {
     if (h->D.S.split) return enqueue_lm_split(h, max_num_iterations);
+    if (!h->comm) {
+        const int rc = alloc_lin_buf2(h);
+        if (rc != ICG_OK) return rc;
+    }
     const BaCaps &C = h->C;
     const BaDev &D = h->D;
     const int n = h->cur_windows;
     cudaStream_t s = h->stream;
     const dim3 g_vis(C.NVB - 2, n), g_cost(h->nblk_vis, n);
     static const int cam_fork = getenv("ICG_BA_CAM_FORK") ? atoi(getenv("ICG_BA_CAM_FORK")) : 0;
-    for (int it = 0; it <= max_num_iterations; it++) {
+    auto enqueue_lin = [&](int at_cand) -> int {
         if (cam_fork == 0) {
             ICG_CUDA(cudaEventRecord(h->ev_fork, s));
             ICG_CUDA(cudaStreamWaitEvent(h->stream_cam, h->ev_fork, 0));
-            ba_lin_cam<<<n, h->cam_threads, h->smem_cam, h->stream_cam>>>(C, D);
+            ba_lin_cam<<<n, h->cam_threads, h->smem_cam, h->stream_cam>>>(C, D, at_cand);
             ICG_CUDA(cudaEventRecord(h->ev_join, h->stream_cam));
         }
         prof_mark(h, 0);
-        ba_lin_vis<<<g_vis, 128, LV_SMEM, s>>>(C, D);
-        prof_mark(h, 1);
+        ba_lin_vis<<<g_vis, 128, LV_SMEM, s>>>(C, D, at_cand);
+        prof_mark(h, at_cand ? 3 : 1);
         if (cam_fork != 0) {
             ICG_CUDA(cudaEventRecord(h->ev_fork, s));
             ICG_CUDA(cudaStreamWaitEvent(h->stream_cam, h->ev_fork, 0));
-            ba_lin_cam<<<n, h->cam_threads, h->smem_cam, h->stream_cam>>>(C, D);
+            ba_lin_cam<<<n, h->cam_threads, h->smem_cam, h->stream_cam>>>(C, D, at_cand);
             ICG_CUDA(cudaEventRecord(h->ev_join, h->stream_cam));
         }
         if (!h->comm) {
             ICG_CUDA(cudaStreamWaitEvent(s, h->ev_join, 0));
-            prof_mark(h, 6);
+            prof_mark(h, at_cand ? 3 : 6);
+        }
+        count_launch(2);
+        return ICG_OK;
+    };
+    for (int it = 0; it <= max_num_iterations; it++) {
+        if (it == 0 || h->comm) {
+            const int rc = enqueue_lin(0);
+            if (rc != ICG_OK) return rc;
         }
         ba_schur_dmma<<<dim3(BA_SPLIT_W, n), 256, h->smem_schur, s>>>(C, D, h->ld_schur);
         prof_mark(h, 5);
@@ -2255,24 +2319,28 @@
         }
         ba_solve<<<n, SOLVE_THREADS, h->smem_solve, s>>>(C, D);
         prof_mark(h, 8);
-        count_launch(h->comm ? 5 : 4);
+        count_launch(h->comm ? 3 : 2);
         if (it == max_num_iterations) break;
-        ICG_CUDA(cudaEventRecord(h->ev_fork, s));
-        ICG_CUDA(cudaStreamWaitEvent(h->stream_cam, h->ev_fork, 0));
-        ba_cost_cam<<<n, h->cam_threads, h->smem_cam, h->stream_cam>>>(C, D, h->nblk_vis);
-        ICG_CUDA(cudaEventRecord(h->ev_join, h->stream_cam));
-        ba_cost<<<g_cost, 256, 0, s>>>(C, D, h->nblk_vis);
-        ICG_CUDA(cudaStreamWaitEvent(s, h->ev_join, 0));
-        prof_mark(h, 9);
         if (h->comm) {
+            ICG_CUDA(cudaEventRecord(h->ev_fork, s));
+            ICG_CUDA(cudaStreamWaitEvent(h->stream_cam, h->ev_fork, 0));
+            ba_cost_cam<<<n, h->cam_threads, h->smem_cam, h->stream_cam>>>(C, D, h->nblk_vis);
+            ICG_CUDA(cudaEventRecord(h->ev_join, h->stream_cam));
+            ba_cost<<<g_cost, 256, 0, s>>>(C, D, h->nblk_vis);
+            ICG_CUDA(cudaStreamWaitEvent(s, h->ev_join, 0));
+            prof_mark(h, 9);
             ba_pack2<<<(n + 127) / 128, 128, 0, s>>>(C, D, n, h->nblk_vis);
             prof_mark(h, 10);
             int rc = nccl_allreduce(h, D.red2, (size_t) n * 4, 0);
             if (rc != ICG_OK) return rc;
-        }
-        ba_accept<<<n, 128, 0, s>>>(C, D, h->nblk_vis);
+            count_launch(3);
+        } else {
+            const int rc = enqueue_lin(1);
+            if (rc != ICG_OK) return rc;
+        }
+        ba_accept<<<n, 128, sizeof(double) * 8 * h->nblk_vis, s>>>(C, D);
         prof_mark(h, 11);
-        count_launch(h->comm ? 4 : 3);
+        count_launch();
     }
     ICG_CHECK_LAUNCH();
     return ICG_OK;
@@ -2379,10 +2447,10 @@
         const unsigned long long epoch = ++h->epoch;
         ICG_CUDA(cudaEventRecord(h->ev_fork, s));
         ICG_CUDA(cudaStreamWaitEvent(h->stream_cam, h->ev_fork, 0));
-        ba_lin_cam<<<n, h->cam_threads, h->smem_cam, h->stream_cam>>>(C, D);
+        ba_lin_cam<<<n, h->cam_threads, h->smem_cam, h->stream_cam>>>(C, D, 0);
         ICG_CUDA(cudaEventRecord(h->ev_join, h->stream_cam));
         prof_mark(h, 0);
-        ba_lin_vis<<<g_vis, 128, LV_SMEM, s>>>(C, D);
+        ba_lin_vis<<<g_vis, 128, LV_SMEM, s>>>(C, D, 0);
         prof_mark(h, 1);
         ba_schur_dmma<<<dim3(BA_SPLIT_W, n), 256, h->smem_schur, s>>>(C, D, h->ld_schur);
         prof_mark(h, 5);
@@ -2683,7 +2751,7 @@
     const BaDev &D = h->D;
     const size_t smem = sizeof(double) * (8 * 480 + 2 * (size_t) C.R) + sizeof(int) * (size_t) C.R + 64;
     marg_prepare<<<(n + 127) / 128, 128, 0, s>>>(D, M, n, 0);
-    ba_lin_vis<<<dim3(C.NVB - 2, n), 128, LV_SMEM, s>>>(C, D);
+    ba_lin_vis<<<dim3(C.NVB - 2, n), 128, LV_SMEM, s>>>(C, D, 0);
     marg_assemble<<<n, 256, smem, s>>>(C, D, M);
     int max_m = 0, max_r = 0;
     for (int w = 0; w < n; w++) max_m = std::max(max_m, out[w].m), max_r = std::max(max_r, out[w].r);
diff --git a/ic_gvins_b200/csrc/ba_marg.cuh b/ic_gvins_b200/csrc/ba_marg.cuh
--- a/ic_gvins_b200/csrc/ba_marg.cuh
+++ b/ic_gvins_b200/csrc/ba_marg.cuh
@@ -152,7 +152,7 @@
     {
         const int PM = C.K * (C.K - 1), P = D.npairs[w];
         const int *pro = D.pair_ro + (size_t) w * PM;
-        const double *Mp = D.Mp + (size_t) w * PM * 210;
+        const double *Mp = lin_Mp(C, D, D.st[w].lin_buf, w);
         int la = 0, lb = 0;
         if (tid < 210) {
             int e = tid;
@@ -176,13 +176,15 @@
             __syncthreads();
         }
     }
+    const int buf = D.st[w].lin_buf;
+    const double *AW = lin_AW(C, D, buf, w), *hl = lin_hl(C, D, buf, w);
     for (int e = tid; e < dm.L * (NCV + 1); e += blockDim.x) {
         const int l = e / (NCV + 1), c = e - l * (NCV + 1);
         const int cl = lm_col[l];
         if (cl < 0) continue;
-        const double v = D.AW[((size_t) w * C.LP + l) * C.NCA + c];
+        const double v = AW[(size_t) l * C.NCA + c];
         if (c == NCV) {
-            H0[(size_t) cl * n0 + cl] = D.hl[(size_t) w * C.L + l];
+            H0[(size_t) cl * n0 + cl] = hl[l];
             b0[cl] = -v;
         } else {
             const int mc = c < 6 * K ? (pose_col[c / 6] < 0 ? -1 : pose_col[c / 6] + c % 6) : c < 6 * K + 6 ? ext_col + c - 6 * K : td_col;
diff --git a/ic_gvins_b200/csrc/ba_split.cuh b/ic_gvins_b200/csrc/ba_split.cuh
--- a/ic_gvins_b200/csrc/ba_split.cuh
+++ b/ic_gvins_b200/csrc/ba_split.cuh
@@ -75,7 +75,7 @@
     };
     double *rv = D.S.redv + (size_t) w * D.S.RV;
     if (A < NCV && B < NCV) {
-        D.Hs[(size_t) w * C.NS * C.NS + (size_t) B * C.NS + A] = D.Hc[(size_t) w * C.NS * C.NS + (size_t) B * C.NS + A] + rsum(tri_idx(A, B, NCV));
+        D.Hs[(size_t) w * C.NS * C.NS + (size_t) B * C.NS + A] = lin_Hc(C, D, 0, w)[(size_t) B * C.NS + A] + rsum(tri_idx(A, B, NCV));
         if (A == B) rv[A] = rsum(TRI + A);
     } else if (A < NCV) {
         rv[NCV + A] = rsum(TRI + NCV + A);
@@ -103,7 +103,7 @@
     const int K = dm.K, NCV = 6 * K + 7, N = 15 * K + 7, NR = N + 1;
     const int CT = CL * SOLVE_THREADS, ctid = cr * SOLVE_THREADS + tid, cwarp = ctid >> 5, ncwarps = CT / 32;
     const int f_first = st.first, f_fresh = st.fresh_lin, f_last = st.last_success, f_iter = st.iter, f_maxit = st.max_iter;
-    const double radius = st.radius, cost_cam = st.cost_cam, gmax_old = st.gmax, xcost_old = st.x_cost, init_old = st.initial_cost;
+    const double radius = st.radius, cost_cam = st.cost_cam[0], gmax_old = st.gmax, xcost_old = st.x_cost, init_old = st.initial_cost;
     double *s_red = sm;
     double *s_scale = s_red + 40;
     double *s_g = s_scale + C.NS;
@@ -111,7 +111,7 @@
     double *s_d2 = s_rhs + C.NS;
     double *s_blk = s_d2 + C.NS;
     double *S = D.Sglobal + (size_t) (w / D.world) * split_S_stride(C);
-    const double *Hc = D.Hc + (size_t) w * C.NS * C.NS, *gcam = D.gc + (size_t) w * C.NS, *Hs = D.Hs + (size_t) w * C.NS * C.NS;
+    const double *Hc = lin_Hc(C, D, 0, w), *gcam = lin_gc(C, D, 0, w), *Hs = D.Hs + (size_t) w * C.NS * C.NS;
     const double *rv = D.S.redv + (size_t) w * D.S.RV;
     double *scale_c = D.scale_c + (size_t) w * C.NS;
     for (int a = tid; a < N; a += SOLVE_THREADS) {
@@ -485,7 +485,7 @@
     const int nt = dsm_ntiles(NR), npan = (N + 7) / 8;
     const int Tn = N >> 3, rn = N & 7;
     const int f_first = st.first, f_fresh = st.fresh_lin, f_last = st.last_success, f_iter = st.iter, f_maxit = st.max_iter;
-    const double radius = st.radius, cost_cam = st.cost_cam, gmax_old = st.gmax, xcost_old = st.x_cost, init_old = st.initial_cost;
+    const double radius = st.radius, cost_cam = st.cost_cam[0], gmax_old = st.gmax, xcost_old = st.x_cost, init_old = st.initial_cost;
     double *s_red = sm;
     double *s_scale = s_red + 40;
     double *s_g = s_scale + VL;
@@ -504,7 +504,7 @@
     double *s_dg = s_xT + 16;
     double *s_P = s_dg + (size_t) ntc * 64;
     double *s_tiles = s_P + (size_t) 2 * ntc * 64;
-    const double *Hc = D.Hc + (size_t) w * C.NS * C.NS, *gcam = D.gc + (size_t) w * C.NS, *Hs = D.Hs + (size_t) w * C.NS * C.NS;
+    const double *Hc = lin_Hc(C, D, 0, w), *gcam = lin_gc(C, D, 0, w), *Hs = D.Hs + (size_t) w * C.NS * C.NS;
     const double *rv = D.S.redv + (size_t) w * D.S.RV;
     double *scale_c = D.scale_c + (size_t) w * C.NS;
     for (int a = tid; a < VL; a += SOLVE_THREADS) {
@@ -955,9 +955,9 @@
     for (int a = tid; a < N; a += SOLVE_THREADS) s_dl[a] = __ldcg(BC + SPLIT_HDR + a);
     __syncthreads();
     const double radius = st.radius;
-    const double *hl = D.hl + (size_t) w * C.L, *gl = D.gl + (size_t) w * C.L, *scale_l = D.scale_l + (size_t) w * C.L;
+    const double *hl = lin_hl(C, D, 0, w), *gl = lin_gl(C, D, 0, w), *scale_l = D.scale_l + (size_t) w * C.L;
     double *step_l = D.step_l + (size_t) w * C.L;
-    const double *AW = D.AW + (size_t) w * C.LP * C.NCA;
+    const double *AW = lin_AW(C, D, 0, w);
     const double *rho = D.rho + (size_t) w * C.L;
     double *rho_c = D.rho_c + (size_t) w * C.L;
     constexpr int LB = 4;
```

Measured after the change: 24190, median of 6. +10.2%, better.
